# gusanagy/Hybrid-Diffusion-Underwater-Atmopheric-Image-Enhancement

Measured on AMD Instinct MI355X. Metric: denoising-steps/sec (256x256, T=1000), higher is better.
Workload: dtype f32 (tensors and accumulation fp32; every operand of the attention contractions as 2xfp16 pieces -- scores: a balance per product term, four terms at d_head 16 / three at d_head 32; P.V: three terms -- and of the 3x3 convs behind GroupNorm likewise (other 3x3 convs: 3xbf16 pieces), on the 16-bit MFM

## Files before the change

### hybrid-diffusion-underwater-atmopheric-image-enhancement_amd/_capi.py

```python
from __future__ import annotations

import ctypes as C
import os
import subprocess

_HERE = os.path.dirname(os.path.abspath(__file__))
LIB_PATH = os.environ.get("HDIFF_LIB", os.path.join(_HERE, "libhdiff.so"))
CSRC = os.path.join(_HERE, "csrc")
MAX_TAPS = 25

_lib = None


class LinearJob(C.Structure):
    _fields_ = [("w0", C.c_void_p), ("b0", C.c_void_p), ("w1", C.c_void_p), ("b1", C.c_void_p), ("y", C.c_void_p),
                ("n", C.c_int), ("first", C.c_int)]


class DdpmLoopDesc(C.Structure):
    _fields_ = [
        ("x", C.c_void_p), ("eps_c", C.c_void_p), ("eps_u", C.c_void_p), ("noise", C.c_void_p), ("x_next", C.c_void_p),
        ("coeff1", C.c_void_p), ("coeff2", C.c_void_p), ("sigma", C.c_void_p), ("step_ptr", C.c_void_p), ("T", C.c_int),
        ("w", C.c_double), ("seed", C.c_uint64), ("nan_flag", C.c_void_p), ("n", C.c_int64),
        ("x_dup0", C.c_void_p), ("x_dup1", C.c_void_p), ("t_next", C.c_void_p), ("t_count", C.c_int),
        ("done_counter", C.c_void_p),
    ]


class CfgDdimLoopDesc(C.Structure):
    _fields_ = [
        ("x", C.c_void_p), ("eps_c", C.c_void_p), ("eps_u", C.c_void_p), ("noise", C.c_void_p), ("x_next", C.c_void_p),
        ("tab", C.c_void_p), ("t_tab", C.c_void_p), ("step_ptr", C.c_void_p), ("nsteps", C.c_int), ("clip_x0", C.c_int),
        ("w", C.c_double), ("seed", C.c_uint64), ("nan_flag", C.c_void_p), ("n", C.c_int64),
        ("x_dup0", C.c_void_p), ("x_dup1", C.c_void_p), ("t_next", C.c_void_p), ("t_count", C.c_int),
        ("done_counter", C.c_void_p),
    ]


class CfgDpmppLoopDesc(C.Structure):
    _fields_ = [
        ("x", C.c_void_p), ("eps_c", C.c_void_p), ("eps_u", C.c_void_p), ("x_next", C.c_void_p), ("x0_prev", C.c_void_p),
        ("tab", C.c_void_p), ("t_tab", C.c_void_p), ("step_ptr", C.c_void_p), ("nsteps", C.c_int), ("clip_x0", C.c_int),
        ("w", C.c_double), ("nan_flag", C.c_void_p), ("n", C.c_int64),
        ("x_dup0", C.c_void_p), ("x_dup1", C.c_void_p), ("t_next", C.c_void_p), ("t_count", C.c_int),
        ("done_counter", C.c_void_p),
    ]


class ConvDesc(C.Structure):
    _fields_ = [
        ("x0", C.c_void_p), ("x1", C.c_void_p), ("C0", C.c_int), ("C1", C.c_int),
        ("B", C.c_int), ("H", C.c_int), ("W", C.c_int),
        ("wp", C.c_void_p), ("bias", C.c_void_p), ("Cout", C.c_int), ("CinPad", C.c_int), ("CoutPad", C.c_int),
        ("gn_scale", C.c_void_p), ("gn_shift", C.c_void_p), ("addvec", C.c_void_p), ("residual", C.c_void_p),
        ("out", C.c_void_p), ("OH", C.c_int), ("OW", C.c_int),
        ("VH", C.c_int), ("VW", C.c_int), ("in_stride", C.c_int),
        ("out_sy", C.c_int), ("out_oy", C.c_int), ("out_sx", C.c_int), ("out_ox", C.c_int),
        ("ntaps", C.c_int), ("tap_dy", C.c_int * MAX_TAPS), ("tap_dx", C.c_int * MAX_TAPS),
        ("splitk_ws", C.c_void_p), ("splitk_floats", C.c_int64), ("wp_x3", C.c_void_p),
        ("wp_h2", C.c_void_p), ("act_scale", C.c_void_p),
    ]


class ConvRange(C.Structure):
    _fields_ = [("absmax_out", C.c_void_p), ("absmax_in", C.c_void_p), ("wp_h2_taps", C.c_void_p),
                ("wp_h2_s2", C.c_void_p)]


class MsssimDesc(C.Structure):
    MAX_PAIRS, MAX_SCALES, MAX_WINDOW = 15, 5, 33
    _fields_ = [
        ("B", C.c_int), ("C", C.c_int), ("H", C.c_int), ("W", C.c_int), ("nscales", C.c_int), ("window", C.c_int),
        ("weights", C.POINTER(C.c_float)), ("npairs", C.c_int),
        ("pair_chan", C.c_int * 15), ("pair_scale", C.c_int * 15), ("pair_cs_pow", C.c_int * 15), ("pair_l_pow", C.c_int * 15),
        ("l1_scale", C.c_int), ("C1", C.c_float), ("C2", C.c_float), ("alpha", C.c_float), ("compensation", C.c_float),
        ("data_range", C.c_float), ("mean", C.c_int),
    ]


class WgradDesc(C.Structure):
    _fields_ = [
        ("x0", C.c_void_p), ("x1", C.c_void_p), ("C0", C.c_int), ("C1", C.c_int),
        ("B", C.c_int), ("H", C.c_int), ("W", C.c_int),
        ("gn_scale", C.c_void_p), ("gn_shift", C.c_void_p), ("dy", C.c_void_p),
        ("Cout", C.c_int), ("CinPad", C.c_int), ("CoutPad", C.c_int), ("OH", C.c_int), ("OW", C.c_int),
        ("VH", C.c_int), ("VW", C.c_int), ("in_stride", C.c_int),
        ("out_sy", C.c_int), ("out_oy", C.c_int), ("out_sx", C.c_int), ("out_ox", C.c_int),
        ("ntaps", C.c_int), ("tap_dy", C.c_int * MAX_TAPS), ("tap_dx", C.c_int * MAX_TAPS),
    ]


_PROTOS = {
    "hdiff_abi_version": (C.c_int, []),
    "hdiff_last_error": (C.c_char_p, []),
    "hdiff_device_count": (C.c_int, []),
    "hdiff_pack_conv_weight_x3": (C.c_int, [C.c_void_p, C.c_void_p, C.c_int, C.c_int, C.c_int, C.c_int, C.c_void_p]),
    "hdiff_pack_conv_weight_x3_taps": (C.c_int, [C.c_void_p, C.c_void_p, C.c_int, C.c_int, C.c_int, C.c_int, C.c_int, C.c_int,
                                                 C.POINTER(C.c_int), C.POINTER(C.c_int), C.c_int, C.c_void_p]),
    "hdiff_pack_conv_weight_h2_words": (C.c_int, [C.c_int, C.c_int, C.c_int, C.POINTER(C.c_int64)]),
    "hdiff_pack_conv_weight_h2": (C.c_int, [C.c_void_p, C.c_void_p, C.c_int, C.c_int, C.c_int, C.c_void_p]),
    "hdiff_gn_act_scale": (C.c_int, [C.c_void_p, C.c_void_p, C.c_int, C.c_int64, C.c_float, C.c_void_p, C.c_void_p]),
    "hdiff_set_contraction_mode": (C.c_int, [C.c_int]),
    "hdiff_get_contraction_mode": (C.c_int, []),
    "hdiff_pack_conv_weight": (C.c_int, [C.c_void_p, C.c_void_p, C.c_int, C.c_int, C.c_int, C.c_int, C.c_int, C.c_int,
                                         C.POINTER(C.c_int), C.POINTER(C.c_int), C.c_int, C.c_int, C.c_int, C.c_void_p]),
    "hdiff_conv2d_fwd": (C.c_int, [C.POINTER(ConvDesc), C.c_void_p]),
    "hdiff_conv2d_fwd_dropout": (C.c_int, [C.POINTER(ConvDesc), C.c_void_p, C.c_float, C.c_void_p]),
    "hdiff_conv2d_fwd_range": (C.c_int, [C.POINTER(ConvDesc), C.POINTER(ConvRange), C.c_void_p]),
    "hdiff_range_words_zero": (C.c_int, [C.c_void_p, C.c_int, C.c_void_p]),
    "hdiff_conv2d_fwd_route": (C.c_int, [C.POINTER(ConvDesc), C.POINTER(ConvRange), C.c_int, C.POINTER(C.c_int), C.POINTER(C.c_int)]),
    "hdiff_pack_conv_weight_h2_taps_words": (C.c_int, [C.c_int, C.c_int, C.c_int, C.c_int, C.POINTER(C.c_int64)]),
    "hdiff_pack_conv_weight_h2_taps": (C.c_int, [C.c_void_p, C.c_void_p, C.c_int, C.c_int, C.c_int, C.c_int, C.c_int, C.c_int,
                                                 C.POINTER(C.c_int), C.POINTER(C.c_int), C.c_int, C.c_void_p]),
    "hdiff_pack_conv_weight_h2_s2_words": (C.c_int, [C.c_int, C.c_int, C.c_int, C.POINTER(C.c_int64)]),
    "hdiff_pack_conv_weight_h2_s2": (C.c_int, [C.c_void_p, C.c_void_p, C.c_int, C.c_int, C.c_int, C.c_int, C.c_void_p]),
    "hdiff_conv2d_fwd_workspace": (C.c_int, [C.POINTER(ConvDesc), C.POINTER(C.c_int64)]),
    "hdiff_gn_stats": (C.c_int, [C.c_void_p, C.c_void_p, C.c_int, C.c_int, C.c_int, C.c_int, C.c_int, C.c_int, C.c_void_p,
                                 C.c_void_p]),
    "hdiff_gn_finalize": (C.c_int, [C.c_void_p, C.c_int, C.c_int, C.c_int, C.c_int, C.c_void_p, C.c_void_p, C.c_float,
                                    C.c_void_p, C.c_void_p, C.c_void_p, C.c_void_p, C.c_void_p]),
    "hdiff_gn_scale_shift": (C.c_int, [C.c_void_p, C.c_void_p, C.c_int, C.c_int, C.c_int, C.c_int, C.c_int, C.c_int, C.c_void_p,
                                       C.c_void_p, C.c_void_p, C.c_float, C.c_void_p, C.c_void_p, C.c_void_p]),
    "hdiff_gn_swish_apply": (C.c_int, [C.c_void_p, C.c_void_p, C.c_void_p, C.c_void_p, C.c_int, C.c_int, C.c_int,
                                       C.c_void_p]),
    "hdiff_mha_flash_fwd": (C.c_int, [C.c_void_p, C.c_void_p, C.c_void_p, C.c_int, C.c_int, C.c_int, C.c_int, C.c_void_p]),
    "hdiff_mha_flash_fwd_workspace": (C.c_int, [C.c_int, C.c_int, C.c_int, C.c_int, C.POINTER(C.c_int64)]),
    "hdiff_mha_flash_fwd_ws": (C.c_int, [C.c_void_p, C.c_void_p, C.c_void_p, C.c_int, C.c_int, C.c_int, C.c_int, C.c_void_p,
                                         C.c_int64, C.c_void_p]),
    "hdiff_mha_flash_fwd_route": (C.c_int, [C.c_int, C.c_int, C.c_int, C.c_int, C.c_int, C.c_int64] + [C.POINTER(C.c_int)] * 3),
    "hdiff_mha_wide_fwd": (C.c_int, [C.c_void_p, C.c_void_p, C.c_int, C.c_int, C.c_int, C.c_void_p]),
    "hdiff_mha_wide_bwd": (C.c_int, [C.c_void_p, C.c_void_p, C.c_void_p, C.c_void_p, C.c_int, C.c_int, C.c_int, C.c_void_p]),
    "hdiff_gn_affine_bwd": (C.c_int, [C.c_void_p, C.c_int, C.c_int, C.c_int, C.c_int, C.c_void_p, C.c_void_p, C.c_void_p, C.c_void_p,
                                      C.c_void_p, C.c_void_p, C.c_void_p, C.c_void_p, C.c_void_p, C.c_void_p]),
    "hdiff_gn_affine_apply": (C.c_int, [C.c_void_p, C.c_void_p, C.c_void_p, C.c_void_p, C.c_int, C.c_int, C.c_int,
                                        C.c_void_p]),
    "hdiff_mha_flash_bwd_workspace": (C.c_int, [C.c_int, C.c_int, C.c_int, C.c_int, C.POINTER(C.c_int64)]),
    "hdiff_mha_flash_bwd": (C.c_int, [C.c_void_p, C.c_void_p, C.c_void_p, C.c_void_p, C.c_void_p, C.c_void_p, C.c_void_p,
                                      C.c_int, C.c_int, C.c_int, C.c_int, C.c_void_p]),
    "hdiff_mha_flash_bwd_route": (C.c_int, [C.c_int, C.c_int, C.c_int, C.c_int] + [C.POINTER(C.c_int)] * 4),
    "hdiff_conv2d_wgrad_workspace": (C.c_int, [C.POINTER(WgradDesc), C.POINTER(C.c_int), C.POINTER(C.c_int64)]),
    "hdiff_conv2d_wgrad": (C.c_int, [C.POINTER(WgradDesc), C.c_void_p, C.c_int, C.c_void_p]),
    "hdiff_conv2d_wgrad_dropout": (C.c_int, [C.POINTER(WgradDesc), C.c_void_p, C.c_float, C.c_void_p, C.c_int, C.c_void_p]),
    "hdiff_conv2d_wgrad_route": (C.c_int, [C.POINTER(WgradDesc), C.c_int, C.POINTER(C.c_int)]),
    "hdiff_conv_wgrad_unpack": (C.c_int, [C.c_void_p, C.c_int, C.c_void_p, C.c_int, C.c_int, C.c_int, C.c_int, C.c_int, C.c_int,
                                          C.POINTER(C.c_int), C.POINTER(C.c_int), C.c_int, C.c_int, C.c_int, C.c_void_p]),
    "hdiff_gn_swish_bwd": (C.c_int, [C.c_void_p, C.c_void_p, C.c_int, C.c_int, C.c_int, C.c_int, C.c_int, C.c_void_p, C.c_void_p,
                                     C.c_void_p, C.c_void_p, C.c_void_p, C.c_void_p, C.c_void_p, C.c_void_p, C.c_void_p,
                                     C.c_void_p, C.c_void_p]),
    "hdiff_gn_swish_dropout_bwd": (C.c_int, [C.c_void_p, C.c_int, C.c_int, C.c_int, C.c_int, C.c_void_p, C.c_void_p, C.c_float,
                                             C.c_void_p, C.c_void_p, C.c_void_p, C.c_void_p, C.c_void_p, C.c_void_p, C.c_void_p,
                                             C.c_void_p, C.c_void_p]),
    "hdiff_bias_addvec_grad": (C.c_int, [C.c_void_p, C.c_int, C.c_int, C.c_int, C.c_void_p, C.c_void_p, C.c_void_p]),
    "hdiff_linear_rows_bwd": (C.c_int, [C.c_void_p, C.c_void_p, C.c_int, C.c_void_p, C.c_void_p, C.c_void_p, C.c_void_p,
                                        C.c_void_p, C.c_int, C.c_int, C.c_int, C.c_int, C.c_int, C.c_int, C.c_void_p]),
    "hdiff_sq_err_bwd": (C.c_int, [C.c_void_p, C.c_void_p, C.c_void_p, C.c_void_p, C.c_int64, C.c_void_p]),
    "hdiff_dropout_mask": (C.c_int, [C.c_void_p, C.c_int64, C.c_float, C.c_uint64, C.c_uint64, C.c_void_p]),
    "hdiff_dropout_keep_bits": (C.c_int, [C.c_void_p, C.c_int64, C.c_float, C.c_uint64, C.c_uint64, C.c_void_p]),
    "hdiff_mul": (C.c_int, [C.c_void_p, C.c_void_p, C.c_void_p, C.c_int64, C.c_void_p]),
    "hdiff_linear_rows": (C.c_int, [C.c_void_p, C.c_void_p, C.c_int, C.c_void_p, C.c_void_p, C.c_void_p, C.c_int, C.c_int,
                                    C.c_int, C.c_int, C.c_int, C.c_void_p]),
    "hdiff_linear_rows_multi": (C.c_int, [C.c_void_p, C.c_void_p, C.c_void_p, C.c_int, C.c_int, C.c_int, C.c_int, C.c_void_p]),
    "hdiff_q_sample": (C.c_int, [C.c_void_p, C.c_void_p, C.c_void_p, C.c_void_p, C.c_void_p, C.c_void_p, C.c_int, C.c_int,
                                 C.c_int, C.c_void_p]),
    "hdiff_sq_err": (C.c_int, [C.c_void_p, C.c_void_p, C.c_void_p, C.c_int64, C.c_void_p]),
    "hdiff_ddpm_step": (C.c_int, [C.c_void_p, C.c_void_p, C.c_void_p, C.c_void_p, C.c_void_p, C.c_void_p, C.c_void_p,
                                  C.c_void_p, C.c_void_p, C.c_int, C.c_double, C.c_uint64, C.c_void_p, C.c_int64, C.c_void_p]),
    "hdiff_ddpm_step_loop": (C.c_int, [C.c_void_p, C.c_void_p]),
    "hdiff_cfg_ddim_step": (C.c_int, [C.c_void_p, C.c_void_p, C.c_void_p, C.c_void_p, C.c_void_p, C.c_void_p, C.c_void_p, C.c_int,
                                      C.c_double, C.c_int, C.c_uint64, C.c_void_p, C.c_int64, C.c_void_p]),
    "hdiff_cfg_ddim_step_loop": (C.c_int, [C.c_void_p, C.c_void_p]),
    "hdiff_cfg_dpmpp_step": (C.c_int, [C.c_void_p, C.c_void_p, C.c_void_p, C.c_void_p, C.c_void_p, C.c_void_p, C.c_void_p, C.c_int,
                                       C.c_double, C.c_int, C.c_void_p, C.c_int64, C.c_void_p]),
    "hdiff_cfg_dpmpp_step_loop": (C.c_int, [C.c_void_p, C.c_void_p]),
    "hdiff_fill_t": (C.c_int, [C.c_void_p, C.c_void_p, C.c_int, C.c_void_p]),
    "hdiff_step_decrement": (C.c_int, [C.c_void_p, C.c_void_p]),
    "hdiff_ddim_step": (C.c_int, [C.c_void_p, C.c_void_p, C.c_void_p, C.c_void_p, C.c_void_p, C.c_int, C.c_void_p, C.c_int64,
                                  C.c_void_p]),
    "hdiff_fill_from_table": (C.c_int, [C.c_void_p, C.c_void_p, C.c_void_p, C.c_int, C.c_int, C.c_void_p]),
    "hdiff_tile_gather": (C.c_int, [C.c_void_p] * 4 + [C.c_int] * 10 + [C.c_void_p]),
    "hdiff_tile_ddim_step": (C.c_int, [C.c_void_p] * 12 + [C.c_int, C.c_void_p] + [C.c_int] * 8 + [C.c_void_p]),
    "hdiff_dpmpp_step": (C.c_int, [C.c_void_p] * 6 + [C.c_int, C.c_int, C.c_void_p, C.c_int64, C.c_void_p]),
    "hdiff_tile_dpmpp_step": (C.c_int, [C.c_void_p] * 13 + [C.c_int, C.c_int, C.c_void_p] + [C.c_int] * 8 + [C.c_void_p]),
    "hdiff_resize_nearest": (C.c_int, [C.c_void_p, C.c_void_p, C.c_int, C.c_int, C.c_int, C.c_int, C.c_int, C.c_void_p]),
    "hdiff_avgpool_global": (C.c_int, [C.c_void_p, C.c_void_p, C.c_int, C.c_int, C.c_void_p]),
    "hdiff_train_b_loss_workspace": (C.c_int, [C.c_int64, C.POINTER(C.c_int64)]),
    "hdiff_train_b_loss_fwd": (C.c_int, [C.c_void_p] * 7 + [C.c_int, C.c_int, C.c_int] + [C.c_void_p] * 5),
    "hdiff_train_b_loss_bwd": (C.c_int, [C.c_void_p] * 7 + [C.c_int, C.c_int, C.c_int] + [C.c_void_p] * 5),
    "hdiff_msssim_l1_workspace": (C.c_int, [C.POINTER(MsssimDesc), C.POINTER(C.c_int64), C.POINTER(C.c_int64)]),
    "hdiff_msssim_l1_fwd": (C.c_int, [C.POINTER(MsssimDesc)] + [C.c_void_p] * 6),
    "hdiff_msssim_l1_bwd": (C.c_int, [C.POINTER(MsssimDesc)] + [C.c_void_p] * 7),
    "hdiff_quality_workspace": (C.c_int, [C.c_int, C.c_int, C.c_int, C.POINTER(C.c_int64)]),
    "hdiff_psnr_ssim": (C.c_int, [C.c_void_p, C.c_void_p, C.c_int, C.c_int, C.c_int, C.c_void_p, C.c_void_p, C.c_void_p]),
    "hdiff_uiqm": (C.c_int, [C.c_void_p, C.c_int, C.c_int, C.c_int, C.c_void_p, C.c_void_p, C.c_void_p]),
    "hdiff_avgpool_global_bwd": (C.c_int, [C.c_void_p, C.c_void_p, C.c_int, C.c_int, C.c_void_p]),
    "hdiff_resize_nearest_bwd": (C.c_int, [C.c_void_p, C.c_void_p, C.c_int, C.c_int, C.c_int, C.c_int, C.c_int, C.c_void_p]),
    "hdiff_concat2": (C.c_int, [C.c_void_p, C.c_void_p, C.c_void_p, C.c_int, C.c_int64, C.c_int64, C.c_void_p]),
    "hdiff_clip": (C.c_int, [C.c_void_p, C.c_void_p, C.c_float, C.c_float, C.c_int64, C.c_void_p]),
    "hdiff_axpby": (C.c_int, [C.c_float, C.c_void_p, C.c_float, C.c_void_p, C.c_void_p, C.c_int64, C.c_void_p]),
    "hdiff_opt_chunk": (C.c_int, []),
    "hdiff_grad_norm_clip_coef": (C.c_int, [C.c_void_p, C.c_void_p, C.c_int, C.c_void_p, C.c_float, C.c_void_p, C.c_void_p]),
    "hdiff_adamw_step": (C.c_int, [C.c_void_p, C.c_void_p, C.c_int, C.c_void_p, C.c_double, C.c_double, C.c_double, C.c_double, C.c_double,
                                   C.c_int64, C.c_void_p]),
    "hdiff_randn": (C.c_int, [C.c_void_p, C.c_int64, C.c_uint64, C.c_uint64, C.c_void_p]),
    "hdiff_graph_begin": (C.c_int, [C.c_void_p]),
    "hdiff_graph_end": (C.c_int, [C.c_void_p, C.POINTER(C.c_void_p)]),
    "hdiff_graph_launch": (C.c_int, [C.c_void_p, C.c_void_p]),
    "hdiff_graph_destroy": (C.c_int, [C.c_void_p]),
    "hdiff_event_create": (C.c_int, [C.POINTER(C.c_void_p)]),
    "hdiff_event_record": (C.c_int, [C.c_void_p, C.c_void_p]),
    "hdiff_event_elapsed_ms": (C.c_int, [C.c_void_p, C.c_void_p, C.POINTER(C.c_float)]),
    "hdiff_event_destroy": (C.c_int, [C.c_void_p]),
}

EXPORTED_SYMBOLS = tuple(_PROTOS.keys())


def build(verbose: bool = False, clean: bool = False) -> str:
    if clean:
        subprocess.run(["make", "-C", CSRC, "clean"], capture_output=True, text=True, check=True)
    res = subprocess.run(["make", "-C", CSRC, "-j8"], capture_output=True, text=True)
    if verbose or res.returncode != 0:
        print(res.stdout[-4000:])
        print(res.stderr[-4000:])
    if res.returncode != 0 or not os.path.isfile(LIB_PATH):
        raise RuntimeError("building libhdiff.so failed")
    return LIB_PATH


MUTANT_PATH = os.path.join(CSRC, "build", "libhdiff_mutant.so")
MUTANT2_PATH = os.path.join(CSRC, "build", "libhdiff_mutant2.so")


def build_mutant(verbose: bool = False) -> str:
    res = subprocess.run(["make", "-C", CSRC, "-j4", "mutant", "mutant2"], capture_output=True, text=True)
    if verbose or res.returncode != 0:
        print(res.stdout[-4000:])
        print(res.stderr[-4000:])
    if res.returncode != 0 or not os.path.isfile(MUTANT_PATH) or not os.path.isfile(MUTANT2_PATH):
        raise RuntimeError("building libhdiff_mutant.so / libhdiff_mutant2.so failed")
    return MUTANT_PATH


def lib() -> C.CDLL:
    global _lib
    if _lib is None:
        if not os.path.isfile(LIB_PATH):
            raise RuntimeError(f"{LIB_PATH} is missing: run `python -c 'import __graft_entry__ as g; g.build()'` "
                               "(the HIP extension is required; there is no CPU fallback)")
        import torch
        hip_rt = os.path.join(os.path.dirname(torch.__file__), "lib", "libamdhip64.so")
        if os.path.isfile(hip_rt):
            C.CDLL(hip_rt, mode=C.RTLD_GLOBAL)
        l = C.CDLL(LIB_PATH)
        for name, (res, args) in _PROTOS.items():
            fn = getattr(l, name)
            fn.restype, fn.argtypes = res, args
        _lib = l
    return _lib


def check(rc: int, what: str = "") -> None:
    if rc != 0:
        msg = lib().hdiff_last_error().decode(errors="replace")
        raise RuntimeError(f"hdiff {what} failed (status {rc}): {msg}")
```

### hybrid-diffusion-underwater-atmopheric-image-enhancement_amd/csrc/attention.hip

```cpp
#include <stdlib.h>

#include <type_traits>

#include "common.h"
#include "device.h"

using namespace hdiff;

namespace {

constexpr int KT = 64;
constexpr int KROW = KT + 4;
constexpr int ATT_THREADS = 256;
constexpr float RESCALE_LIMIT = 1.8446744e19f;

__device__ __forceinline__ f32x2 pk_add(f32x2 a, f32x2 b) {
  f32x2 r;
  asm("v_pk_add_f32 %0, %1, %2" : "=v"(r) : "v"(a), "v"(b));
  return r;
}

template <int D, int NQ>
__global__ __launch_bounds__(ATT_THREADS) void mha_flash_fwd_kernel(const float* __restrict__ qkv, float* __restrict__ out,
                                                                    float* __restrict__ lse2, int C, int L, float qscale, int check) {
// ... 300 lines not shown
  f32x2 l_run[NQ];
#pragma unroll
  for (int qt = 0; qt < NQ; ++qt) {
    l_run[qt] = f32x2{0.f, 0.f};
    negm4[qt] = f32x4{0.f, 0.f, 0.f, 0.f};
#pragma unroll
    for (int mt = 0; mt < MT; ++mt) O[mt][qt] = f32x4{0.f, 0.f, 0.f, 0.f};
  }

  f32x4 P[4];
  auto rowsum = [&](int qt) {
    const f32x2 a = pk_add(__builtin_shufflevector(P[0], P[0], 0, 1), __builtin_shufflevector(P[0], P[0], 2, 3));
    const f32x2 b = pk_add(__builtin_shufflevector(P[1], P[1], 0, 1), __builtin_shufflevector(P[1], P[1], 2, 3));
    const f32x2 c = pk_add(__builtin_shufflevector(P[2], P[2], 0, 1), __builtin_shufflevector(P[2], P[2], 2, 3));
    const f32x2 d = pk_add(__builtin_shufflevector(P[3], P[3], 0, 1), __builtin_shufflevector(P[3], P[3], 2, 3));
    const f32x2 ab = pk_add(a, b), cd = pk_add(c, d);
    l_run[qt] = pk_add(l_run[qt], pk_add(ab, cd));
  };
  auto do_tile = [&](auto first_tag, int buf) {
    constexpr bool FIRST = decltype(first_tag)::value;
    float kf[4][KS];
    float vf[4][MT][4];
#pragma unroll
    for (int ks = 0; ks < 4; ++ks) {
#pragma unroll
      for (int s = 0; s < KS; ++s) kf[ks][s] = sK[buf][(4 * s + g) * KROW + ks * 16 + i16];
#pragma unroll
      for (int mt = 0; mt < MT; ++mt) {
        const float4 v4 = *reinterpret_cast<const float4*>(&sV[buf][(mt * 16 + i16) * KROW + ks * 16 + 4 * g]);
        vf[ks][mt][0] = v4.x; vf[ks][mt][1] = v4.y; vf[ks][mt][2] = v4.z; vf[ks][mt][3] = v4.w;
      }
    }
    f32x4 S[2][4];
    auto qk_mfma = [&](int qt, int i) {
      const int s = i >> 2, ks = i & 3;
      S[qt & 1][ks] = __builtin_amdgcn_mfma_f32_16x16x4f32(kf[ks][s], qf[qt][s], s == 0 ? negm4[qt] : S[qt & 1][ks], 0, 0, 0);
    };
    auto pv_mfma = [&](int qt, int i) {
      const int mt = i % MT, j = i / MT, ks = j >> 2, r = j & 3;
      O[mt][qt] = __builtin_amdgcn_mfma_f32_16x16x4f32(vf[ks][mt][r], P[ks][r], O[mt][qt], 0, 0, 0);
    };
    auto softmax = [&](int qt) {
      f32x4(&Sq)[4] = S[qt & 1];
      if (FIRST) {
        float tm = fmaxf(fmaxf(Sq[0][0], Sq[0][1]), fmaxf(Sq[0][2], Sq[0][3]));
#pragma unroll
        for (int ks = 1; ks < 4; ++ks) tm = fmaxf(tm, fmaxf(fmaxf(Sq[ks][0], Sq[ks][1]), fmaxf(Sq[ks][2], Sq[ks][3])));
        tm = fmaxf(tm, __shfl_xor(tm, 16, 64));
        tm = fmaxf(tm, __shfl_xor(tm, 32, 64));
        const float nm = -tm;
        negm4[qt] = f32x4{nm, nm, nm, nm};
#pragma unroll
        for (int ks = 0; ks < 4; ++ks) Sq[ks] += negm4[qt];
      }
      if (!FIRST || qt > 0) {
        __builtin_amdgcn_sched_barrier(0);
        rowsum((qt + NQ - 1) % NQ);
      }
#pragma unroll
      for (int ks = 0; ks < 4; ++ks)
        P[ks] = f32x4{__builtin_amdgcn_exp2f(Sq[ks][0]), __builtin_amdgcn_exp2f(Sq[ks][1]), __builtin_amdgcn_exp2f(Sq[ks][2]),
                      __builtin_amdgcn_exp2f(Sq[ks][3])};
      __builtin_amdgcn_sched_barrier(0);
    };
#pragma unroll
    for (int i = 0; i < N_QK; ++i) qk_mfma(0, i);
#pragma unroll
    for (int qt = 0; qt < NQ; ++qt) {
      softmax(qt);
      constexpr int LEAD = 3;
      static_assert(N_QK <= N_PV, "the QK^T chain is folded into the P.V slots");
      if (qt + 1 < NQ) {
#pragma unroll
        for (int i = 0; i < LEAD; ++i) qk_mfma(qt + 1, i);
      }
#pragma unroll
      for (int i = 0; i < N_PV; ++i) {
        if (i == N_PV - LEAD) __builtin_amdgcn_sched_barrier(0);
        pv_mfma(qt, i);
        if (qt + 1 < NQ && i + LEAD < N_QK) qk_mfma(qt + 1, i + LEAD);
      }
    }
  };

  stage_load(0);
  stage_store(0);
  __syncthreads();
  stage_load(ntiles > 1 ? 1 : 0);
  do_tile(std::true_type{}, 0);
  stage_store(1);
  __syncthreads();
  auto step = [&](int t, auto buf_tag) {
    constexpr int buf = decltype(buf_tag)::value;
    stage_load((t + 1 < ntiles) ? t + 1 : t);
    do_tile(std::false_type{}, buf);
    stage_store(buf ^ 1);
    __syncthreads();
  };
  int t = 1;
  for (; t + 1 < ntiles; t += 2) {
    step(t, std::integral_constant<int, 1>{});
    step(t + 1, std::integral_constant<int, 0>{});
  }
  if (t < ntiles) step(t, std::integral_constant<int, 1>{});
  rowsum(NQ - 1);

  float* obase = out + ((size_t)b * C + (size_t)head * D) * L;
#pragma unroll
  for (int qt = 0; qt < NQ; ++qt) {
    float lt = l_run[qt].x + l_run[qt].y;
    lt += __shfl_xor(lt, 16, 64);
    lt += __shfl_xor(lt, 32, 64);
    const bool bad = !(lt < OVERFLOW_LIMIT);
    const float inv = bad ? __builtin_nanf("") : 1.0f / lt;
    const int q = qblk0 + qt * 16 + i16;
    if (lse2 != nullptr && q < L && g == 0)
      lse2[((size_t)b * gridDim.y + head) * L + q] = bad ? __builtin_nanf("") : __builtin_amdgcn_logf(lt) - negm4[qt][0];
    if (q < L) {
#pragma unroll
      for (int mt = 0; mt < MT; ++mt)
#pragma unroll
        for (int r = 0; r < 4; ++r) {
          const int d = mt * 16 + 4 * g + r;
          if (d < D) obase[(size_t)d * L + q] = O[mt][qt][r] * inv;
        }
    }
  }
}

template <int D, int NQ>
void launch_v(const float* qkv, float* o, float* lse2, int B, int C, int heads, int L, float qscale, int check,
              hipStream_t stream) {
  dim3 grid(cdiv(L, 64 * NQ), heads, B);
  hipLaunchKernelGGL((mha_flash_fwd_kernel<D, NQ>), grid, dim3(ATT_THREADS), 0, stream, qkv, o, lse2, C, L, qscale, check);
}

struct MhaFwdRoute { int route, nq, check; };
MhaFwdRoute mha_fwd_route(int B, int C, int heads, int L, bool want_lse, int64_t ws_bytes, int mode) {
  const int D = C / heads;
  if (D >= 48 || L < 512) return {HDIFF_MHA_FWD_ROUTE_RUNNING_MAX, 1, 0};
  if (mode != HDIFF_CONTRACT_F32) {
    const int64_t need = mha_fwd_x3p_workspace(B, C, heads, L);
    const bool ws_ok = need != 0 && ws_bytes >= need;
    if (mode == HDIFF_CONTRACT_F16 && !want_lse && ws_ok) return {HDIFF_MHA_FWD_ROUTE_F16_SINGLE, 4, 1};
    if (ws_ok && D == 16) return {HDIFF_MHA_FWD_ROUTE_H2_PAIRS, 4, 1};
    if (ws_ok && D == 32) return {HDIFF_MHA_FWD_ROUTE_X3P_PAIRS, 4, 1};
    if (L % KT == 0 && (D == 16 || D == 32)) return {HDIFF_MHA_FWD_ROUTE_X3_TRIPLES, 4, 1};
  }
  if (L % KT == 0) return {HDIFF_MHA_FWD_ROUTE_FAST_F32, 4, 1};
  return {HDIFF_MHA_FWD_ROUTE_RUNNING_MAX, 4, 0};
}

template <int D>
void launch_d(const float* qkv, float* o, float* lse2, int B, int C, int heads, int L, void* ws, const MhaFwdRoute& rt,
              hipStream_t stream) {
  const float qscale = 1.4426950408889634f / sqrtf((float)D);
  static const bool skip_check = getenv("HDIFF_NO_CHECK_PASS") != nullptr;
  const bool tail = !skip_check || rt.route == HDIFF_MHA_FWD_ROUTE_RUNNING_MAX || rt.route == HDIFF_MHA_FWD_ROUTE_FAST_F32;
  if constexpr (D < 48) {
    switch (rt.route) {
      case HDIFF_MHA_FWD_ROUTE_F16_SINGLE: launch_mha_fwd_f16(qkv, o, B, C, heads, L, qscale, ws, stream); break;
      case HDIFF_MHA_FWD_ROUTE_H2_PAIRS: launch_mha_fwd_h2(qkv, o, lse2, B, C, heads, L, qscale, ws, stream); break;
      case HDIFF_MHA_FWD_ROUTE_X3P_PAIRS: launch_mha_fwd_x3p(qkv, o, lse2, B, C, heads, L, qscale, ws, stream); break;
      case HDIFF_MHA_FWD_ROUTE_X3_TRIPLES: launch_mha_fwd_x3(qkv, o, lse2, B, C, heads, L, qscale, stream); break;
      case HDIFF_MHA_FWD_ROUTE_FAST_F32:
        hipLaunchKernelGGL((mha_flash_fwd_fast_kernel<D, 4>), dim3(cdiv(L, 256), heads, B), dim3(ATT_THREADS), 0, stream, qkv, o, lse2, C, L, qscale);
        break;
      default: break;
    }
    if (tail && rt.nq == 4) launch_v<D, 4>(qkv, o, lse2, B, C, heads, L, qscale, rt.check, stream);
  }
  if (tail && rt.nq == 1) launch_v<D, 1>(qkv, o, lse2, B, C, heads, L, qscale, rt.check, stream);
}

}

static int mha_fwd_check_shape(int B, int C, int heads, int L) {
  HDIFF_CHECK_ARG(B > 0 && L > 0 && heads > 0 && C % heads == 0, "mha_flash_fwd: bad sizes B=%d C=%d heads=%d L=%d", B, C,
                  heads, L);
  HDIFF_CHECK_ARG(mha_head_dim_ok(C / heads), "mha_flash_fwd: head dim %d not in {4, 8, 12, 16, 24, 32, 48, 64}", C / heads);
  return HDIFF_OK;
}

static int mha_flash_fwd_any(const float* qkv, float* o, float* lse2, int B, int C, int heads, int L, void* ws,
                             int64_t ws_bytes, hipStream_t s) {
  HDIFF_CHECK_ARG(qkv && o, "mha_flash_fwd: null pointer");
  const int rc = mha_fwd_check_shape(B, C, heads, L);
  if (rc != HDIFF_OK) return rc;
  const MhaFwdRoute rt = mha_fwd_route(B, C, heads, L, lse2 != nullptr, ws_bytes, contraction_mode());
  (void)hipGetLastError();
  with_head_dim(C / heads, [&](auto d) { launch_d<decltype(d)::value>(qkv, o, lse2, B, C, heads, L, ws, rt, s); });
  HDIFF_CHECK_LAUNCH("mha_flash_fwd_kernel");
  return HDIFF_OK;
}

extern "C" int hdiff_mha_flash_fwd(const float* qkv, float* o, float* lse2, int B, int C, int heads, int L,
                                   hdiff_stream_t stream) {
  return mha_flash_fwd_any(qkv, o, lse2, B, C, heads, L, nullptr, 0, (hipStream_t)stream);
}

extern "C" int hdiff_mha_flash_fwd_workspace(int B, int C, int heads, int L, int64_t* bytes_out) {
  HDIFF_CHECK_ARG(bytes_out, "mha_flash_fwd_workspace: null pointer");
  HDIFF_CHECK_ARG(B > 0 && L > 0 && heads > 0 && C % heads == 0, "mha_flash_fwd_workspace: bad sizes B=%d C=%d heads=%d L=%d", B,
                  C, heads, L);
  *bytes_out = mha_fwd_x3p_workspace(B, C, heads, L);
  return HDIFF_OK;
}

extern "C" int hdiff_mha_flash_fwd_ws(const float* qkv, float* o, float* lse2, int B, int C, int heads, int L, void* ws,
                                      int64_t ws_bytes, hdiff_stream_t stream) {
  HDIFF_CHECK_ARG(ws_bytes >= 0 && (ws != nullptr || ws_bytes == 0), "mha_flash_fwd_ws: workspace pointer / size mismatch");
  return mha_flash_fwd_any(qkv, o, lse2, B, C, heads, L, ws, ws_bytes, (hipStream_t)stream);
}

extern "C" int hdiff_mha_flash_fwd_route(int B, int C, int heads, int L, int want_lse, int64_t ws_bytes, int* route_out,
                                         int* nq_out, int* check_out) {
  HDIFF_CHECK_ARG(route_out && nq_out && check_out, "mha_flash_fwd_route: null pointer");
  HDIFF_CHECK_ARG(ws_bytes >= 0, "mha_flash_fwd_ws: workspace pointer / size mismatch");
  const int rc = mha_fwd_check_shape(B, C, heads, L);
  if (rc != HDIFF_OK) return rc;
  const MhaFwdRoute rt = mha_fwd_route(B, C, heads, L, want_lse != 0, ws_bytes, contraction_mode());
  *route_out = rt.route;
  *nq_out = rt.nq;
  *check_out = rt.check;
  return HDIFF_OK;
}
```

### hybrid-diffusion-underwater-atmopheric-image-enhancement_amd/csrc/attention_h2.hip

```cpp
#include <stdlib.h>

#include <type_traits>

#include "common.h"
#include "device.h"

using namespace hdiff;

namespace {

constexpr int KT = 64;
constexpr int THREADS = 256;
#define H2_RARE_BEGIN "s_cmp_lg_u64 %[cond], 0\n\ts_cbranch_scc1 .Lh2r_%=\n.Lh2b_%=:\n\t.subsection 1\n.Lh2r_%=:\n\t"
#define H2_RARE_END "s_branch .Lh2b_%=\n\t.subsection 0"

__device__ __forceinline__ float h2_rare_delta(unsigned long long cond, const f32x4 (&S)[4], int bp16, int bp32) {
  float delta, t, u;
  asm volatile(H2_RARE_BEGIN
               "v_max3_f32 %[t], %[s0], %[s1], %[s2]\n\t"
               "v_max3_f32 %[u], %[s3], %[s4], %[s5]\n\t"
               "v_max3_f32 %[t], %[t], %[s6], %[s7]\n\t"
               "v_max3_f32 %[u], %[u], %[s8], %[s9]\n\t"
               "v_max3_f32 %[t], %[t], %[s10], %[s11]\n\t"
               "v_max3_f32 %[u], %[u], %[s12], %[s13]\n\t"
               "v_max3_f32 %[t], %[t], %[s14], %[s15]\n\t"
               "v_max_f32 %[t], %[t], %[u]\n\t"
               "s_nop 1\n\t"
               "ds_bpermute_b32 %[u], %[bp16], %[t]\n\t"
               "s_waitcnt lgkmcnt(0)\n\t"
               "v_max_f32 %[t], %[t], %[u]\n\t"
               "s_nop 1\n\t"
               "ds_bpermute_b32 %[u], %[bp32], %[t]\n\t"
               "s_waitcnt lgkmcnt(0)\n\t"
               "v_max_f32 %[t], %[t], %[u]\n\t"
               "v_subrev_f32 %[u], 8.0, %[t]\n\t"
               "v_ceil_f32 %[u], %[u]\n\t"
               "v_cmp_lt_f32 vcc, 0x41100000, %[t]\n\t"
               "v_cndmask_b32 %[d], 0, %[u], vcc\n\t"
               H2_RARE_END
               : [d] "=&v"(delta), [t] "=&v"(t), [u] "=&v"(u)
               : [cond] "s"(cond), [bp16] "v"(bp16), [bp32] "v"(bp32), [s0] "v"(S[0][0]), [s1] "v"(S[0][1]), [s2] "v"(S[0][2]),
                 [s3] "v"(S[0][3]), [s4] "v"(S[1][0]), [s5] "v"(S[1][1]), [s6] "v"(S[1][2]), [s7] "v"(S[1][3]), [s8] "v"(S[2][0]),
                 [s9] "v"(S[2][1]), [s10] "v"(S[2][2]), [s11] "v"(S[2][3]), [s12] "v"(S[3][0]), [s13] "v"(S[3][1]),
                 [s14] "v"(S[3][2]), [s15] "v"(S[3][3])
               : "vcc", "scc");
  return delta;
}

__device__ __forceinline__ void h2_rare_rescale(unsigned long long cond, float delta, f32x4& O, f32x4& negm, float& l, float& sum0,
                                                float& sum1) {
  float o0 = O[0], o1 = O[1], o2 = O[2], o3 = O[3], n0 = negm[0], n1 = negm[1], n2 = negm[2], n3 = negm[3], w;
  asm volatile(H2_RARE_BEGIN
               "v_cvt_i32_f32 %[w], %[d]\n\t"
               "v_sub_u32 %[w], 0, %[w]\n\t"
               "v_ldexp_f32 %[o0], %[o0], %[w]\n\t"
               "v_ldexp_f32 %[o1], %[o1], %[w]\n\t"
               "v_ldexp_f32 %[o2], %[o2], %[w]\n\t"
               "v_ldexp_f32 %[o3], %[o3], %[w]\n\t"
               "v_ldexp_f32 %[l], %[l], %[w]\n\t"
               "v_sub_f32 %[n0], %[n0], %[d]\n\t"
               "v_sub_f32 %[n1], %[n1], %[d]\n\t"
               "v_sub_f32 %[n2], %[n2], %[d]\n\t"
               "v_sub_f32 %[n3], %[n3], %[d]\n\t"
               "v_mov_b32 %[q0], 0\n\t"
               "v_mov_b32 %[q1], 0\n\t"
               H2_RARE_END
               : [o0] "+v"(o0), [o1] "+v"(o1), [o2] "+v"(o2), [o3] "+v"(o3), [n0] "+v"(n0), [n1] "+v"(n1), [n2] "+v"(n2),
                 [n3] "+v"(n3), [l] "+v"(l), [q0] "+v"(sum0), [q1] "+v"(sum1), [w] "=&v"(w)
               : [cond] "s"(cond), [d] "v"(delta)
               : "scc");
  O = f32x4{o0, o1, o2, o3};
  negm = f32x4{n0, n1, n2, n3};
}

__device__ __forceinline__ void h2_rare_exp_split(unsigned long long cond, float delta, float one, f32x4 S, unsigned& a0, unsigned& a1,
                                                  unsigned& r0, unsigned& r1, float& sum0, float& sum1) {
  float p0, p1, p2, p3, t0, t1;
  asm volatile(H2_RARE_BEGIN
               "v_sub_f32 %[p0], %[s0], %[d]\n\t"
               "v_sub_f32 %[p1], %[s1], %[d]\n\t"
               "v_sub_f32 %[p2], %[s2], %[d]\n\t"
               "v_sub_f32 %[p3], %[s3], %[d]\n\t"
               "v_exp_f32 %[p0], %[p0]\n\t"
               "v_exp_f32 %[p1], %[p1]\n\t"
               "v_exp_f32 %[p2], %[p2]\n\t"
               "v_exp_f32 %[p3], %[p3]\n\t"
               "s_nop 1\n\t"
               "v_cvt_pk_f16_f32 %[a0], %[p0], %[p1]\n\t"
               "v_cvt_pk_f16_f32 %[a1], %[p2], %[p3]\n\t"
               "v_add_f32 %[t0], %[p0], %[p2]\n\t"
               "v_add_f32 %[t1], %[p1], %[p3]\n\t"
               "v_fma_mixlo_f16 %[r0], %[p0], %[one], -%[a0] op_sel_hi:[0,0,1]\n\t"
               "v_fma_mixlo_f16 %[r1], %[p2], %[one], -%[a1] op_sel_hi:[0,0,1]\n\t"
               "v_add_f32 %[q0], %[q0], %[t0]\n\t"
               "v_add_f32 %[q1], %[q1], %[t1]\n\t"
               "v_fma_mixhi_f16 %[r0], %[p1], %[one], -%[a0] op_sel:[0,0,1] op_sel_hi:[0,0,1]\n\t"
               "v_fma_mixhi_f16 %[r1], %[p3], %[one], -%[a1] op_sel:[0,0,1] op_sel_hi:[0,0,1]\n\t"
               "s_nop 1\n\t"
               H2_RARE_END
               : [a0] "+v"(a0), [a1] "+v"(a1), [r0] "+v"(r0), [r1] "+v"(r1), [q0] "+v"(sum0), [q1] "+v"(sum1), [p0] "=&v"(p0),
                 [p1] "=&v"(p1), [p2] "=&v"(p2), [p3] "=&v"(p3), [t0] "=&v"(t0), [t1] "=&v"(t1)
               : [cond] "s"(cond), [d] "v"(delta), [one] "s"(one), [s0] "v"(S[0]), [s1] "v"(S[1]), [s2] "v"(S[2]), [s3] "v"(S[3])
               : "scc");
}


__global__ __launch_bounds__(THREADS) void qk_rowmax_kernel(const float* __restrict__ qkv, float* __restrict__ rowmax, int C, int L) {
  qkv_rowmax<2>(qkv, rowmax, C, L);
}

template <int D>
__global__ __launch_bounds__(THREADS) void qk_split_h2_kernel(const float* __restrict__ qkv, const float* __restrict__ rowmax,
                                                              __bf16* __restrict__ ws, int C, int L, float qscale, float one) {
  const int heads = C / D;
  const int which = blockIdx.y / heads, head = blockIdx.y - which * heads, b = blockIdx.z;
  const int l = blockIdx.x * THREADS + threadIdx.x;
  float mq = 0.f, mk = 0.f;
#pragma unroll
  for (int d = 0; d < D; ++d) {
    mq = fmaxf(mq, rowmax[(size_t)b * 2 * C + head * D + d]);
    mk = fmaxf(mk, rowmax[(size_t)b * 2 * C + C + head * D + d]);
  }
  const int a = balance_exp(__builtin_bit_cast(unsigned, mq), __builtin_bit_cast(unsigned, mk), qscale);
  const float sc = which == 0 ? qscale * __builtin_bit_cast(float, (unsigned)(127 - a) << 23) : __builtin_bit_cast(float, (unsigned)(127 + a) << 23);
  if (l >= L) return;
  const float* src = qkv + ((size_t)b * 3 * C + (size_t)which * C + (size_t)head * D) * L;
  const size_t piece = (size_t)L * D;
  __bf16* pair = ws + ((size_t)b * heads + head) * F_COUNT * piece;
  const float up = (float)(1 << PAIR_SHIFT) * one;
  unsigned h[4][D / 2];
#pragma unroll
  for (int j = 0; j < D / 2; ++j)
    pair4(src[(size_t)(2 * j) * L + l] * sc, src[(size_t)(2 * j + 1) * L + l] * sc, up, h[0][j], h[1][j], h[2][j], h[3][j]);
#pragma unroll
  for (int p = 0; p < 4; ++p) {
    if (which == 0 && (p == 1 || p == 3)) continue;
    const int slot = which == 0 ? F_Q + (p == 0 ? 0 : 1) : F_K + p;
    u32x4* o = reinterpret_cast<u32x4*>(pair + slot * piece + (size_t)l * D);
#pragma unroll
    for (int j = 0; j < D / 8; ++j) o[j] = u32x4{h[p][4 * j], h[p][4 * j + 1], h[p][4 * j + 2], h[p][4 * j + 3]};
  }
}

template <int D>
__global__ __launch_bounds__(THREADS) void v_split_h2_kernel(const float* __restrict__ qkv, __bf16* __restrict__ ws, int C, int L,
                                                             float one) {
  const int heads = C / D;
  const int row = blockIdx.x, head = row / D, d = row - head * D, b = blockIdx.y;
  const int tid = threadIdx.x;
  const float* src = qkv + ((size_t)b * 3 * C + 2 * (size_t)C + row) * L;
  const size_t piece = (size_t)L * D;
  __bf16* pair = ws + ((size_t)b * heads + head) * F_COUNT * piece;
  _Float16* dst = reinterpret_cast<_Float16*>(pair + F_V * piece) + (size_t)d * L;

  const float amax = row_absmax(src, L, tid);
  int e = (int)((__builtin_bit_cast(unsigned, amax) >> 23) & 0xffu) - 127;
  e = e < -100 ? -100 : (e > 127 ? 127 : e);
  const float scale = __builtin_bit_cast(float, (unsigned)(14 - e + 127) << 23);
  if (tid == 0) reinterpret_cast<float*>(pair + F_VINV * piece)[d] = __builtin_bit_cast(float, (unsigned)(e - 14 + 127) << 23);
  for (int i = tid; i < L / 4; i += THREADS) {
    const f32x4 v = *reinterpret_cast<const f32x4*>(src + 4 * (size_t)i);
    unsigned a0, a1, c0, c1;
    split2(v[0] * scale, v[1] * scale, one, a0, a1);
    split2(v[2] * scale, v[3] * scale, one, c0, c1);
    *reinterpret_cast<u32x2*>(dst + 4 * (size_t)i) = u32x2{a0, c0};
    *reinterpret_cast<u32x2*>(dst + piece + 4 * (size_t)i) = u32x2{a1, c1};
  }
}

template <int D, int NQ>
__global__ __launch_bounds__(THREADS, 2) void mha_flash_fwd_h2_kernel(const __bf16* __restrict__ ws, float* __restrict__ out,
                                                                      float* __restrict__ lse2, int C, int L, float one) {
  static_assert(D == 16, "head dim: two terms share one MFMA's 32 contraction slots");
  static_assert(NQ == 4, "the stage pipeline is written for four query tiles per wave");
  constexpr int NKP = 4;
  constexpr int NKS = 2;
  constexpr int NQK = NKS;
  constexpr int MT = D / 16;
  constexpr int KROWB = D * 2;
  constexpr int KPART = KT * KROWB;
  constexpr int VROWB = KT * 2 + 8;
  constexpr int VPART = D * VROWB;
  constexpr int QB = 64 * NQ;
  constexpr int VBASE = NKP * KPART;
  constexpr int BUFB = VBASE + 2 * VPART;
  __shared__ __attribute__((aligned(16))) unsigned char smem[2][BUFB];

  const int tid = threadIdx.x, lane = tid & 63, wave = tid >> 6;
  const int i16 = lane & 15, g = lane >> 4;
  const TileId tile = xcd_tile();
  const int head = tile.head, b = tile.b;
  const int qblk0 = tile.x * QB + wave * (16 * NQ);
  const int ntiles = L / KT;

  const int doff = 8 * (g & 1);
  const bool hi = g >> 1;

  const size_t piece_n = (size_t)L * D;
  const __bf16* wsq = ws + ((size_t)b * gridDim.y + head) * F_COUNT * piece_n;
  u32x4 qop[NQ][NQK];
  {
    const unsigned dn2 = PAIR_DOWN2;
#pragma unroll
    for (int qt = 0; qt < NQ; ++qt) {
      const int q = qblk0 + qt * 16 + i16;
      const u32x4 q0 = *reinterpret_cast<const u32x4*>(wsq + (size_t)q * D + doff);
      const u32x4 q1s = *reinterpret_cast<const u32x4*>(wsq + piece_n + (size_t)q * D + doff);
      const u32x4 sel = hi ? q1s : q0;
      unsigned dnw[4];
#pragma unroll
      for (int w = 0; w < 4; ++w) asm("v_pk_mul_f16 %0, %1, %2" : "=v"(dnw[w]) : "v"(sel[w]), "v"(dn2));
      qop[qt][0] = sel;
      qop[qt][1] = u32x4{dnw[0], dnw[1], dnw[2], dnw[3]};
    }
  }
  int kaddr[NKS];
#pragma unroll
  for (int ks = 0; ks < NKS; ++ks) kaddr[ks] = (2 * ks + (hi ? 1 : 0)) * KPART + i16 * KROWB + doff * 2;
  const int vaddr = i16 * VROWB + 8 * g;

  static_assert(2 * D * 8 == THREADS, "staging geometry: one V chunk per thread");
  static_assert(KPART == 2048 && THREADS == 256, "LDS-DMA geometry: eight 1 KiB runs, two per wave");
  const unsigned char* gsrc;
  int lds_off;
  u32x4 stage;
  {
    const __bf16* vsp = wsq + F_V * piece_n;
    const int p = tid / (D * 8), rem = tid - p * (D * 8);
    const int d = rem >> 3, seg = rem & 7;
    gsrc = reinterpret_cast<const unsigned char*>(vsp + p * piece_n + (size_t)d * L) + seg * 16;
    lds_off = VBASE + p * VPART + d * VROWB + seg * 16;
  }
  const unsigned lds0 = (unsigned)(size_t)(lds_byte*)&smem[0][0];
  const unsigned char* kdma = reinterpret_cast<const unsigned char*>(wsq + F_K * piece_n);
  auto dma_k = [&](int t, int buf) {
    const int ws_ = __builtin_amdgcn_readfirstlane(wave);
    const unsigned char* src = kdma + (size_t)ws_ * (piece_n * 2) + (size_t)t * KPART;
    const unsigned dst = __builtin_amdgcn_readfirstlane(lds0 + buf * BUFB + ws_ * KPART);
    dma_1k(src, lane * 16, dst);
    dma_1k(src + 1024, lane * 16, dst + 1024);
  };
  auto stage_load = [&](int t) { stage = *reinterpret_cast<const u32x4*>(gsrc + (size_t)t * (KT * 2)); };
  auto stage_store = [&](int buf) {
    unsigned char* dst = &smem[buf][lds_off];
    *reinterpret_cast<u32x2*>(dst) = u32x2{stage[0], stage[1]};
    *reinterpret_cast<u32x2*>(dst + 8) = u32x2{stage[2], stage[3]};
  };

  f32x4 O[MT][NQ];
  f32x4 negm4[NQ];
  float l_run[NQ];
  const int bp16 = (lane ^ 16) * 4, bp32 = (lane ^ 32) * 4;
#pragma unroll
  for (int qt = 0; qt < NQ; ++qt) {
    l_run[qt] = 0.f;
    negm4[qt] = f32x4{0.f, 0.f, 0.f, 0.f};
#pragma unroll
    for (int mt = 0; mt < MT; ++mt) O[mt][qt] = f32x4{0.f, 0.f, 0.f, 0.f};
  }

  u32x4 vop[2][MT][2];
  u32x4 kop[4][NKS];
  f32x4 S[2][4];
  u32x4 pop[2][2][2];
  auto load_v = [&](int buf) {
    const unsigned char* vb = smem[buf] + VBASE;
#pragma unroll
    for (int p = 0; p < 2; ++p)
#pragma unroll
      for (int mt = 0; mt < MT; ++mt)
#pragma unroll
        for (int c = 0; c < 2; ++c) {
          const unsigned char* src = vb + p * VPART + mt * 16 * VROWB + 64 * c + vaddr;
          const u32x2 lo = *reinterpret_cast<const u32x2*>(src);
          const u32x2 hi2 = *reinterpret_cast<const u32x2*>(src + 32);
          vop[p][mt][c] = u32x4{lo[0], lo[1], hi2[0], hi2[1]};
        }
  };
  auto load_k = [&](int buf) {
    const unsigned char* kb = smem[buf];
#pragma unroll
    for (int kt = 0; kt < 4; ++kt)
#pragma unroll
      for (int ks = 0; ks < NKS; ++ks) kop[kt][ks] = *reinterpret_cast<const u32x4*>(kb + kaddr[ks] + kt * 16 * KROWB);
  };
  auto qk_mfma = [&](int qt, int par, int n, int rollk = -1) {
    const int j = n >> 2, kt = n & 3;
    u32x4 qb = qop[qt][j];
    if ((HDIFF_MUTANT & 4) && j == 1)
#pragma unroll
      for (int w = 0; w < 4; ++w) qb[w] &= 0xffe0ffe0u;
    S[par][kt] = mfma_f16(kop[kt][j], qb, j == 0 ? negm4[qt] : S[par][kt]);
    if (rollk >= 0) kop[kt][j] = *reinterpret_cast<const u32x4*>(smem[rollk] + kaddr[j] + kt * 16 * KROWB);
  };
  constexpr int NPV = 6 * MT;
  auto pv_mfma = [&](int qt, int par, int n) {
    const int c = n / (3 * MT), r = n - c * 3 * MT, mt = r / 3, term = r - mt * 3;
    const int pv_v = term == 0 ? 1 : 0, pv_p = term == 1 ? 1 : 0;
    u32x4 pb = pop[par][pv_p][c];
    if ((HDIFF_MUTANT & 8) && pv_p == 1)
#pragma unroll
      for (int w = 0; w < 4; ++w) pb[w] &= 0xffe0ffe0u;
    O[mt][qt] = mfma_f16(vop[pv_v][mt][c], pb, O[mt][qt]);
  };
  auto exp_split = [&](const f32x4 (&Sq)[4], u32x4 (&pp)[2][2], float& sum0, float& sum1) {
#pragma unroll
    for (int kt = 0; kt < 4; ++kt) {
      const float p0 = __builtin_amdgcn_exp2f(Sq[kt][0]), p1 = __builtin_amdgcn_exp2f(Sq[kt][1]);
      const float p2 = __builtin_amdgcn_exp2f(Sq[kt][2]), p3 = __builtin_amdgcn_exp2f(Sq[kt][3]);
      sum0 = (kt == 0) ? p0 + p2 : sum0 + (p0 + p2);
      sum1 = (kt == 0) ? p1 + p3 : sum1 + (p1 + p3);
      const int c = kt >> 1, o = (kt & 1) * 2;
      unsigned a0, a1, c0, c1;
      split2(p0, p1, one, a0, a1);
      split2(p2, p3, one, c0, c1);
      pp[0][c][o] = a0; pp[1][c][o] = a1;
      pp[0][c][o + 1] = c0; pp[1][c][o + 1] = c1;
    }
  };
  auto stage_max = [&](int par) {
    float mx = fmaxf(fmaxf(S[par][0][0], S[par][0][1]), fmaxf(S[par][0][2], S[par][0][3]));
#pragma unroll
    for (int kt = 1; kt < 4; ++kt) mx = fmaxf(mx, fmaxf(fmaxf(S[par][kt][0], S[par][kt][1]), fmaxf(S[par][kt][2], S[par][kt][3])));
    mx = fmaxf(mx, __shfl_xor(mx, 16, 64));
    return fmaxf(mx, __shfl_xor(mx, 32, 64));
  };
  auto stage_fn = [&](auto qt_tag, auto first_tag, auto pend_tag, int rollk = -1) {
    constexpr int QT = decltype(qt_tag)::value;
    constexpr bool FIRST = decltype(first_tag)::value;
    constexpr bool PEND = decltype(pend_tag)::value;
    constexpr int par = QT & 1;
    constexpr int qk_q = (QT + 1) % NQ, pv_q = (QT + NQ - 1) % NQ;
    constexpr int NQKM = 4 * NQK, NM = NQKM + (PEND ? NPV : 0);
    float sum0, sum1;
    if constexpr (FIRST) {
#pragma unroll
      for (int n = 0; n < NQKM; ++n) qk_mfma(qk_q, par ^ 1, n, rollk);
      if constexpr (PEND)
#pragma unroll
        for (int n = 0; n < NPV; ++n) pv_mfma(pv_q, par ^ 1, n);
      const float nm = P_SHIFT - stage_max(par);
      negm4[QT] = f32x4{nm, nm, nm, nm};
#pragma unroll
      for (int kt = 0; kt < 4; ++kt) S[par][kt] += negm4[QT];
      exp_split(S[par], pop[par], sum0, sum1);
    } else {
      float pe[4][4], ad[4][2];
      unsigned u[4][2];
      _Float16 rl[4][2];
      unsigned r2[4][2];
      auto vstep = [&](int n) {
        const int kt = n / 14, r = n - kt * 14;
        if (r < 4) pe[kt][r] = __builtin_amdgcn_exp2f(S[par][kt][r]);
        else if (r < 6) {
          const f16x2 p = {(_Float16)pe[kt][2 * (r - 4)], (_Float16)pe[kt][2 * (r - 4) + 1]};
          unsigned w = __builtin_bit_cast(unsigned, p);
          asm("" : "+v"(w));
          u[kt][r - 4] = w;
        } else if (r < 8) ad[kt][r - 6] = pe[kt][r - 6] + pe[kt][r - 6 + 2];
        else if (r < 10) rl[kt][r - 8] = (_Float16)__builtin_fmaf(pe[kt][2 * (r - 8)], one, -(float)__builtin_bit_cast(f16x2, u[kt][r - 8])[0]);
        else if (r < 12) {
          const f16x2 pr = {rl[kt][r - 10],
                            (_Float16)__builtin_fmaf(pe[kt][2 * (r - 10) + 1], one, -(float)__builtin_bit_cast(f16x2, u[kt][r - 10])[1])};
          unsigned w = __builtin_bit_cast(unsigned, pr);
          asm("" : "+v"(w));
          r2[kt][r - 10] = w;
        } else if (r == 12) sum0 = (kt == 0) ? ad[kt][0] : sum0 + ad[kt][0];
        else sum1 = (kt == 0) ? ad[kt][1] : sum1 + ad[kt][1];
      };
      constexpr int NV = 56;
#pragma unroll
      for (int i = 0; i < NM; ++i) {
        if constexpr (PEND) {
          const int npv = (i + 1) * NPV / NM, ppv = i * NPV / NM;
          if (npv != ppv) pv_mfma(pv_q, par ^ 1, ppv);
          else qk_mfma(qk_q, par ^ 1, i - ppv, rollk);
        } else qk_mfma(qk_q, par ^ 1, i, rollk);
#pragma unroll
        for (int n = NV * i / NM; n < NV * (i + 1) / NM; ++n) vstep(n);
        __builtin_amdgcn_sched_barrier(0);
      }
      const unsigned long long cond = __builtin_amdgcn_ballot_w64(sum0 + sum1 >= P_TRIP);
      const float delta = h2_rare_delta(cond, S[par], bp16, bp32);
      h2_rare_rescale(cond, delta, O[0][QT], negm4[QT], l_run[QT], sum0, sum1);
#pragma unroll
      for (int kt = 0; kt < 4; ++kt)
        h2_rare_exp_split(cond, delta, one, S[par][kt], u[kt][0], u[kt][1], r2[kt][0], r2[kt][1], sum0, sum1);
#pragma unroll
      for (int kt = 0; kt < 4; ++kt) {
        const int c = kt >> 1, o = (kt & 1) * 2;
        pop[par][0][c][o] = u[kt][0]; pop[par][1][c][o] = r2[kt][0];
        pop[par][0][c][o + 1] = u[kt][1]; pop[par][1][c][o + 1] = r2[kt][1];
      }
    }
    l_run[QT] += sum0 + sum1;
  };

  auto tile_fn = [&](auto first_tag, int t) {
    constexpr bool FIRST = decltype(first_tag)::value;
    using Pend = std::integral_constant<bool, !FIRST>;
    const int buf = t & 1;
    if constexpr (FIRST) load_v(buf);
    stage_fn(std::integral_constant<int, 0>{}, first_tag, Pend{});
    if constexpr (!FIRST) load_v(buf);
    stage_fn(std::integral_constant<int, 1>{}, first_tag, std::true_type{});
    stage_store(buf ^ 1);
    asm volatile("s_waitcnt vmcnt(0)" ::: "memory");
    __syncthreads();
    stage_load((t + 2 < ntiles) ? t + 2 : ntiles - 1);
    dma_k((t + 2 < ntiles) ? t + 2 : ntiles - 1, buf);
    stage_fn(std::integral_constant<int, 2>{}, first_tag, std::true_type{}, buf ^ 1);
    stage_fn(std::integral_constant<int, 3>{}, first_tag, std::true_type{});
  };

  stage_load(0);
  dma_k(0, 0);
  stage_store(0);
  asm volatile("s_waitcnt vmcnt(0)" ::: "memory");
  __syncthreads();
  stage_load(ntiles > 1 ? 1 : 0);
  dma_k(ntiles > 1 ? 1 : 0, 1);
  load_k(0);
#pragma unroll
  for (int n = 0; n < 4 * NQK; ++n) qk_mfma(0, 0, n);
  tile_fn(std::true_type{}, 0);
  for (int t = 1; t < ntiles; ++t) tile_fn(std::false_type{}, t);
#pragma unroll
  for (int n = 0; n < NPV; ++n) pv_mfma(NQ - 1, 1, n);

  float* obase = out + ((size_t)b * C + (size_t)head * D) * L;
  const float* vinv = reinterpret_cast<const float*>(wsq + F_VINV * piece_n);
#pragma unroll
  for (int qt = 0; qt < NQ; ++qt) {
    float lt = l_run[qt];
    lt += __shfl_xor(lt, 16, 64);
    lt += __shfl_xor(lt, 32, 64);
    const bool bad = !(lt < OVERFLOW_LIMIT);
    const float inv = bad ? __builtin_nanf("") : 1.0f / lt;
    const int q = qblk0 + qt * 16 + i16;
    if (lse2 != nullptr && g == 0)
      lse2[((size_t)b * gridDim.y + head) * L + q] = bad ? __builtin_nanf("") : __builtin_amdgcn_logf(lt) - negm4[qt][0];
#pragma unroll
    for (int mt = 0; mt < MT; ++mt)
#pragma unroll
      for (int r = 0; r < 4; ++r)
        obase[(size_t)(mt * 16 + 4 * g + r) * L + q] = (O[mt][qt][r] * inv) * vinv[mt * 16 + 4 * g + r];
  }
}

}

namespace hdiff {
void launch_v_split_h2(const float* qkv, void* ws, int B, int C, int heads, int L, hipStream_t stream) {
  if (C / heads == 16) hipLaunchKernelGGL((v_split_h2_kernel<16>), dim3(C, B), dim3(THREADS), 0, stream, qkv, (__bf16*)ws, C, L, 1.0f);
  else hipLaunchKernelGGL((v_split_h2_kernel<32>), dim3(C, B), dim3(THREADS), 0, stream, qkv, (__bf16*)ws, C, L, 1.0f);
}

int64_t mha_fwd_h2_tail_bytes(int B, int C) { return ((int64_t)B * 2 * C * 4 + 255) / 256 * 256; }

void launch_qk_split_h2(const float* qkv, void* ws, int B, int C, int heads, int L, float qscale, hipStream_t stream) {
  float* rowmax = reinterpret_cast<float*>(reinterpret_cast<unsigned char*>(ws) + mha_fwd_x3p_workspace(B, C, heads, L) - mha_fwd_h2_tail_bytes(B, C));
  hipLaunchKernelGGL(qk_rowmax_kernel, dim3(2 * C, B), dim3(THREADS), 0, stream, qkv, rowmax, C, L);
  dim3 grid(cdiv(L, 256), 2 * heads, B);
  if (C / heads == 16) hipLaunchKernelGGL((qk_split_h2_kernel<16>), grid, dim3(THREADS), 0, stream, qkv, rowmax, (__bf16*)ws, C, L, qscale, 1.0f);
  else hipLaunchKernelGGL((qk_split_h2_kernel<32>), grid, dim3(THREADS), 0, stream, qkv, rowmax, (__bf16*)ws, C, L, qscale, 1.0f);
}

void launch_mha_fwd_h2(const float* qkv, float* o, float* lse2, int B, int C, int heads, int L, float qscale, void* ws,
                       hipStream_t stream) {
  launch_qk_split_h2(qkv, ws, B, C, heads, L, qscale, stream);
  launch_v_split_h2(qkv, ws, B, C, heads, L, stream);
  hipLaunchKernelGGL((mha_flash_fwd_h2_kernel<16, 4>), dim3(L / 256, heads, B), dim3(THREADS), 0, stream, (const __bf16*)ws, o, lse2,
                     C, L, 1.0f);
}

}
```

### hybrid-diffusion-underwater-atmopheric-image-enhancement_amd/csrc/attention_x3p.hip

```cpp
#include <stdlib.h>

#include "common.h"
#include "device.h"

using namespace hdiff;

namespace {

constexpr int D = 32;
constexpr int KT = 64;
constexpr int THREADS = 256;
constexpr int NQT = 3;

__global__ __launch_bounds__(THREADS, 2) void mha_flash_fwd_x3p_kernel(const __bf16* __restrict__ ws, float* __restrict__ out,
                                                                      float* __restrict__ lse2, int C, int L, float one) {
  constexpr int KS = D / 16;
  constexpr int KROWB = D * 2 + 16;
  constexpr int KPART = KT * KROWB;
  constexpr int VROWB = KT * 2 + 8;
  constexpr int VPART = D * VROWB;
  constexpr int NKC = NQT * KT * D / 8;
  constexpr int NVC = 2 * D * 8;
  constexpr int NLD = (NKC + NVC) / THREADS;
  static_assert((NKC + NVC) % THREADS == 0, "staging geometry");
// ... 92 lines not shown
#pragma unroll
      for (int s = 0; s < KS; ++s) kop[p][s] = *reinterpret_cast<const u32x4*>(kbuf + p * KPART + 32 * s);
  };
  auto load_v = [&](int buf, int kb, u32x4 (&vop)[2][2]) {
    const unsigned char* vbuf = smem[buf] + VBASE + kb * 64;
#pragma unroll
    for (int ab = 0; ab < 2; ++ab)
#pragma unroll
      for (int p = 0; p < 2; ++p) {
        const unsigned char* src = vbuf + vaddr[p] + 32 * ab;
        const u32x2 lo = *reinterpret_cast<const u32x2*>(src);
        const u32x2 hi2 = *reinterpret_cast<const u32x2*>(src + 16);
        vop[ab][p] = u32x4{lo[0], lo[1], hi2[0], hi2[1]};
      }
  };
  auto qk = [&](const u32x4 (&kop)[NQT][KS], int G, f32x16 c) {
    f32x16 S = c;
#pragma unroll
    for (int term = 0; term < NQT; ++term)
#pragma unroll
      for (int s = 0; s < KS; ++s) {
        u32x4 qb = qop[G][term][s];
        if ((HDIFF_MUTANT & 2) && term == 1)
#pragma unroll
          for (int w = 0; w < 4; ++w) qb[w] &= 0xffe0ffe0u;
        S = mfma_f16(kop[term][s], qb, S);
      }
    return S;
  };
  auto exp_pairs = [&](const f32x16& S, u32x4 (&pop)[2][2], float& sum0, float& sum1) {
    sum0 = 0.f; sum1 = 0.f;
#pragma unroll
    for (int j = 0; j < 4; ++j) {
      const float p0 = __builtin_amdgcn_exp2f(S[4 * j]), p1 = __builtin_amdgcn_exp2f(S[4 * j + 1]);
      const float p2 = __builtin_amdgcn_exp2f(S[4 * j + 2]), p3 = __builtin_amdgcn_exp2f(S[4 * j + 3]);
      sum0 += p0 + p2;
      sum1 += p1 + p3;
      unsigned a0, a1, c0, c1;
      split2(p0, p1, one, a0, a1);
      split2(p2, p3, one, c0, c1);
      const int ab = j >> 1, o = (j & 1) * 2;
      pop[ab][0][o] = a0; pop[ab][1][o] = a1;
      pop[ab][0][o + 1] = c0; pop[ab][1][o + 1] = c1;
    }
  };
  auto softmax_pairs = [&](f32x16& S, int G, u32x4 (&pop)[2][2]) {
    float sum0, sum1;
    exp_pairs(S, pop, sum0, sum1);
    if (__builtin_amdgcn_ballot_w64(sum0 + sum1 >= P_TRIP) != 0ull) {
      float mx = fmaxf(fmaxf(S[0], S[1]), fmaxf(S[2], S[3]));
#pragma unroll
      for (int j = 1; j < 4; ++j) mx = fmaxf(mx, fmaxf(fmaxf(S[4 * j], S[4 * j + 1]), fmaxf(S[4 * j + 2], S[4 * j + 3])));
      mx = fmaxf(mx, __shfl_xor(mx, 32, 64));
      const float delta = (mx > P_SHIFT + 1.0f) ? __builtin_ceilf(mx - P_SHIFT) : 0.f;
      const int e = -(int)delta;
#pragma unroll
      for (int r = 0; r < 16; ++r) O[G][r] = __builtin_ldexpf(O[G][r], e);
      l_run[G][0] = __builtin_ldexpf(l_run[G][0], e);
      l_run[G][1] = __builtin_ldexpf(l_run[G][1], e);
      negm2[G] -= delta;
#pragma unroll
      for (int r = 0; r < 16; ++r) S[r] -= delta;
      exp_pairs(S, pop, sum0, sum1);
    }
    l_run[G][0] += sum0;
    l_run[G][1] += sum1;
  };
  auto pv = [&](const u32x4 (&vop)[2][2], const u32x4 (&pop)[2][2], int G) {
#pragma unroll
    for (int ab = 0; ab < 2; ++ab) {
      O[G] = mfma_f16(vop[ab][1], pop[ab][0], O[G]);
      O[G] = mfma_f16(vop[ab][0], pop[ab][1], O[G]);
      O[G] = mfma_f16(vop[ab][0], pop[ab][0], O[G]);
    }
  };

  stage_load(0);
  stage_store(0);
  __syncthreads();
  stage_load(ntiles > 1 ? 1 : 0);
  {
    u32x4 K0[NQT][KS];
    load_k(0, 0, K0);
    const f32x16 s0 = qk(K0, 0, negm16), s1 = qk(K0, 1, negm16);
    float t0 = s0[0], t1 = s1[0];
#pragma unroll
    for (int r = 1; r < 16; ++r) { t0 = fmaxf(t0, s0[r]); t1 = fmaxf(t1, s1[r]); }
    negm2[0] = P_SHIFT - fmaxf(t0, __shfl_xor(t0, 32, 64));
    negm2[1] = P_SHIFT - fmaxf(t1, __shfl_xor(t1, 32, 64));
  }
  auto block = [&](int buf, int kb) {
    u32x4 kop[NQT][KS], vop[2][2];
    load_k(buf, kb, kop);
    load_v(buf, kb, vop);
    f32x16 S2[2];
#pragma unroll
    for (int G = 0; G < 2; ++G) {
      float nm = negm2[G];
      asm volatile("" : "+v"(nm));
#pragma unroll
      for (int r = 0; r < 16; ++r) negm16[r] = nm;
      S2[G] = qk(kop, G, negm16);
    }
#pragma unroll
    for (int G = 0; G < 2; ++G) {
      u32x4 pop[2][2];
      softmax_pairs(S2[G], G, pop);
      pv(vop, pop, G);
    }
  };
  block(0, 0);
  block(0, 1);
  stage_store(1);
  __syncthreads();
  for (int t = 1; t < ntiles; ++t) {
    const int buf = t & 1;
    stage_load((t + 1 < ntiles) ? t + 1 : t);
    block(buf, 0);
    block(buf, 1);
    stage_store(buf ^ 1);
    __syncthreads();
  }

  float* obase = out + ((size_t)b * C + (size_t)head * D) * L;
  const float* vinv = reinterpret_cast<const float*>(qs + 8 * piece);
#pragma unroll
  for (int G = 0; G < 2; ++G) {
    float lt = l_run[G][0] + l_run[G][1];
    lt += __shfl_xor(lt, 32, 64);
    const bool bad = !(lt < OVERFLOW_LIMIT);
    const float inv = bad ? __builtin_nanf("") : 1.0f / lt;
    const int q = qblk0 + 32 * G + l31;
    if (lse2 != nullptr && h == 0)
      lse2[((size_t)b * heads + head) * L + q] = bad ? __builtin_nanf("") : __builtin_amdgcn_logf(lt) - negm2[G];
#pragma unroll
    for (int r = 0; r < 16; ++r) {
      const int d = 8 * (r >> 2) + 4 * h + (r & 3);
      obase[(size_t)d * L + q] = (O[G][r] * inv) * vinv[d];
    }
  }
}

}

namespace hdiff {

int64_t mha_fwd_x3p_workspace(int B, int C, int heads, int L) {
  const int Dh = C / heads;
  if ((Dh != 16 && Dh != 32) || L % 256 != 0 || L < 512) return 0;
  return (int64_t)B * C * L * F_COUNT * 2 + mha_fwd_h2_tail_bytes(B, C);
}

void launch_mha_fwd_x3p(const float* qkv, float* o, float* lse2, int B, int C, int heads, int L, float qscale, void* ws,
                        hipStream_t stream) {
  launch_qk_split_h2(qkv, ws, B, C, heads, L, qscale, stream);
  launch_v_split_h2(qkv, ws, B, C, heads, L, stream);
  hipLaunchKernelGGL(mha_flash_fwd_x3p_kernel, dim3(L / 256, heads, B), dim3(THREADS), 0, stream, (const __bf16*)ws, o, lse2, C, L, 1.0f);
}

}
```

### hybrid-diffusion-underwater-atmopheric-image-enhancement_amd/csrc/common.h

```cpp
#pragma once
#include <hip/hip_runtime.h>
#include <stdint.h>
#include <stdio.h>
#include <string.h>

#include <type_traits>

#include "../../include/hdiff.h"

namespace hdiff {

void set_error(const char* fmt, ...);

#define HDIFF_CHECK_ARG(cond, ...)            \
  do {                                        \
    if (!(cond)) {                            \
      hdiff::set_error(__VA_ARGS__);          \
      return HDIFF_ERR_INVALID;               \
    }                                         \
  } while (0)

#define HDIFF_CHECK_LAUNCH(what)                                                   \
  do {                                                                             \
    hipError_t e__ = hipGetLastError();                                            \
    if (e__ != hipSuccess) {                                                       \
      hdiff::set_error("%s: %s", what, hipGetErrorString(e__));                    \
      return HDIFF_ERR_LAUNCH;                                                     \
    }                                                                              \
  } while (0)

static inline int cdiv(int a, int b) { return (a + b - 1) / b; }

static inline int grid_floor_2k(int64_t n, int per_thread = 1) {
  int64_t blocks = (n / per_thread + 255) / 256;
  if (blocks < 1) blocks = 1;
  if (blocks > 2048) blocks = 2048;
  return (int)blocks;
}
static inline int grid_ceil_8k(int64_t n, int per_thread = 1) {
  int64_t blocks = (n + (int64_t)256 * per_thread - 1) / ((int64_t)256 * per_thread);
  if (blocks > 256 * 32) blocks = 256 * 32;
  if (blocks < 1) blocks = 1;
  return (int)blocks;
}

static inline bool first_use_on_device(uint64_t& mask) {
  int dev = 0;
  if (hipGetDevice(&dev) != hipSuccess || dev < 0 || dev >= 64) return true;
  const uint64_t bit = 1ull << dev;
  if (mask & bit) return false;
  mask |= bit;
  return true;
}

bool wgrad3x3_applicable(const hdiff_conv_wgrad_desc* d);
int wgrad3x3_nsplit(const hdiff_conv_wgrad_desc* d);
int launch_wgrad3x3(const hdiff_conv_wgrad_desc* d, float* dwp, int nsplit, hipStream_t stream, const unsigned* keep_bits = nullptr,
                    float inv_keep = 1.0f);
bool wgrad1x1_applicable(const hdiff_conv_wgrad_desc* d);
int wgrad1x1_nsplit(const hdiff_conv_wgrad_desc* d);
int launch_wgrad1x1(const hdiff_conv_wgrad_desc* d, float* dwp, int nsplit, hipStream_t stream);

int contraction_mode();
inline bool split_operands_on() { return contraction_mode() != HDIFF_CONTRACT_F32; }

static inline bool mha_head_dim_ok(int D) { return D == 4 || D == 8 || D == 12 || D == 16 || D == 24 || D == 32 || D == 48 || D == 64; }
template <class F>
static inline void with_head_dim(int D, F&& f) {
  switch (D) {
    case 4: return f(std::integral_constant<int, 4>{});
    case 8: return f(std::integral_constant<int, 8>{});
    case 12: return f(std::integral_constant<int, 12>{});
    case 16: return f(std::integral_constant<int, 16>{});
    case 24: return f(std::integral_constant<int, 24>{});
    case 32: return f(std::integral_constant<int, 32>{});
    case 48: return f(std::integral_constant<int, 48>{});
    case 64: return f(std::integral_constant<int, 64>{});
  }
}

struct KeyRanges { int per, nsplit; };
static inline KeyRanges key_ranges(int nkb_total, int want) {
  if (want > nkb_total) want = nkb_total;
  if (want < 1) want = 1;
  const int per = cdiv(nkb_total, want);
  return {per, cdiv(nkb_total, per)};
}
long long mha_bwd_slab_cap_bytes();
bool mha_bwd_x3_shape_ok(int B, int C, int heads, int L);
KeyRanges mha_bwd_h2_key_ranges(int B, int heads, int L, int D);
int64_t mha_bwd_x3_workspace_floats(int B, int C, int heads, int L);
bool mha_bwd_h2_lds_granted();
void launch_mha_bwd_h2(const float* qkv, const float* d_o, const float* lse2, const float* delta, float* dqkv, float* ws, int B,
                       int C, int heads, int L, KeyRanges g, hipStream_t stream);
int64_t mha_fwd_x3p_workspace(int B, int C, int heads, int L);
int64_t mha_fwd_h2_tail_bytes(int B, int C);
void launch_mha_fwd_x3p(const float* qkv, float* o, float* lse2, int B, int C, int heads, int L, float qscale, void* ws, hipStream_t stream);
void launch_mha_fwd_h2(const float* qkv, float* o, float* lse2, int B, int C, int heads, int L, float qscale, void* ws, hipStream_t stream);
void launch_qk_split_h2(const float* qkv, void* ws, int B, int C, int heads, int L, float qscale, hipStream_t stream);
void launch_v_split_h2(const float* qkv, void* ws, int B, int C, int heads, int L, hipStream_t stream);
void launch_mha_fwd_x3(const float* qkv, float* o, float* lse2, int B, int C, int heads, int L, float qscale, hipStream_t stream);
void launch_mha_fwd_f16(const float* qkv, float* o, int B, int C, int heads, int L, float qscale, void* ws, hipStream_t stream);

}
```

### hybrid-diffusion-underwater-atmopheric-image-enhancement_amd/csrc/conv1x1_x3.hip

```cpp
#include <stdlib.h>

#include "common.h"
#include "conv_x3.h"
#include "device.h"

using namespace hdiff;

namespace {

constexpr int THREADS = 256;

__device__ constexpr int TERM_W[6] = {2, 1, 0, 1, 0, 0};
__device__ constexpr int TERM_X[6] = {0, 1, 2, 0, 1, 0};

template <bool WLDS>
__global__ __launch_bounds__(THREADS, 3) void conv1x1_x3_kernel(const Conv1x1X3K p) {
  constexpr int MT = 2, WN = 2;
  __shared__ __attribute__((aligned(16))) u32x4 sW[WLDS ? 2 : 1][WLDS ? 3 * 64 * 2 : 1];
  const int tid = threadIdx.x, lane = tid & 63, wave = tid >> 6;
  const int l31 = lane & 31, h = lane >> 5;
  int cob = blockIdx.x, tile_id = blockIdx.y;
  if ((gridDim.y & 7u) == 0u && gridDim.x > 1u) {
    const unsigned lin = blockIdx.x + gridDim.x * blockIdx.y, per = 8u * gridDim.x;
    const unsigned grp = lin / per, r = lin - grp * per;
    tile_id = (int)(grp * 8u + (r & 7u));
    cob = (int)(r >> 3);
  }
  const int co0 = cob * 64;
  const long px0 = ((long)tile_id * 4 + __builtin_amdgcn_readfirstlane(wave)) * 64;
  const int b = blockIdx.z;
  const int C1 = p.Cin - p.C0;
  const unsigned hw = (unsigned)p.HW;
  const float* x0b = p.x0 + (size_t)b * p.C0 * p.HW + px0;
  const float* x1b = p.x1 ? p.x1 + (size_t)b * C1 * p.HW + px0 - (size_t)p.C0 * p.HW : x0b;
  const unsigned* wlane = p.wp3 + ((size_t)(co0 + l31) * 8 + h * 4);
  const size_t w_piece = (size_t)p.CoutPad * 8, w_chunk = 3 * w_piece;

  f32x16 acc[MT][WN];
#pragma unroll
  for (int mt = 0; mt < MT; ++mt)
#pragma unroll
    for (int nt = 0; nt < WN; ++nt)
#pragma unroll
      for (int r = 0; r < 16; ++r) acc[mt][nt][r] = 0.f;

  constexpr int XD = 1;
  const int nchunks = p.Cin / 16;
  f32x2 xr[XD + 1][8];
  u32x4 wr[2][MT][3];
  auto load_x = [&](f32x2 (&x)[8], int c) {
    c = min(c, nchunks - 1);
    const float* xb = (16 * c < p.C0) ? x0b : x1b;
    const unsigned k0 = (unsigned)(16 * c + 8 * h);
#pragma unroll
    for (int j = 0; j < 8; ++j) x[j] = *reinterpret_cast<const f32x2*>(xb + (size_t)((k0 + j) * hw + 2u * l31));
  };
  auto load_w = [&](u32x4 (&w)[MT][3], int c) {
    const unsigned* wb = wlane + (size_t)min(c, nchunks - 1) * w_chunk;
#pragma unroll
    for (int mt = 0; mt < MT; ++mt)
#pragma unroll
      for (int pc = 0; pc < 3; ++pc) w[mt][pc] = *reinterpret_cast<const u32x4*>(wb + pc * w_piece + (size_t)mt * 32 * 8);
  };
  auto mma = [&](const f32x2 (&x)[8], const u32x4 (&w)[MT][3]) {
    u32x4 xp[WN][3];
#pragma unroll
    for (int nt = 0; nt < WN; ++nt)
#pragma unroll
      for (int j = 0; j < 4; ++j) {
        unsigned h0, h1, h2;
        split3(x[2 * j][nt], x[2 * j + 1][nt], h0, h1, h2);
        xp[nt][0][j] = h0; xp[nt][1][j] = h1; xp[nt][2][j] = h2;
      }
#pragma unroll
    for (int t = 0; t < 6; ++t) {
      if ((HDIFF_MUTANT & 1) && TERM_W[t] == 0 && TERM_X[t] == 2) continue;
#pragma unroll
      for (int mt = 0; mt < MT; ++mt)
#pragma unroll
        for (int nt = 0; nt < WN; ++nt) acc[mt][nt] = mfma_bf16(w[mt][TERM_W[t]], xp[nt][TERM_X[t]], acc[mt][nt]);
    }
  };

  if constexpr (WLDS) {
    const unsigned* wsrc[2];
    int wdst[2];
#pragma unroll
    for (int i = 0; i < 2; ++i) {
      int u = i * THREADS + tid;
      if (u >= 384) u -= 128;
      const int pc = u >> 7, rem = u & 127;
      wsrc[i] = p.wp3 + (size_t)pc * w_piece + (size_t)(co0 + (rem >> 1)) * 8 + (rem & 1) * 4;
      wdst[i] = u;
    }
    u32x4 wst[2];
    auto wload = [&](int c) {
      const size_t off = (size_t)min(c, nchunks - 1) * w_chunk;
#pragma unroll
      for (int i = 0; i < 2; ++i) wst[i] = *reinterpret_cast<const u32x4*>(wsrc[i] + off);
    };
    auto wstore = [&](int buf) {
#pragma unroll
      for (int i = 0; i < 2; ++i) sW[buf][wdst[i]] = wst[i];
    };
    auto wread = [&](u32x4 (&w)[MT][3], int buf) {
#pragma unroll
      for (int mt = 0; mt < MT; ++mt)
#pragma unroll
        for (int pc = 0; pc < 3; ++pc) w[mt][pc] = sW[buf][(pc * 64 + 32 * mt + l31) * 2 + h];
    };
    wload(0);
    load_x(xr[0], 0);
    wstore(0);
    __syncthreads();
    for (int c = 0; c < nchunks; c += 2) {
#pragma unroll
      for (int i = 0; i < 2; ++i) {
        if (c + i < nchunks) {
          wload(c + i + 1);
          load_x(xr[(i + 1) & 1], c + i + 1);
          wread(wr[0], i);
          mma(xr[i], wr[0]);
          wstore((i + 1) & 1);
          asm volatile("s_waitcnt lgkmcnt(0)\n\ts_barrier" ::: "memory");
        }
      }
    }
  } else {
#pragma unroll
    for (int i = 0; i < XD; ++i) load_x(xr[i], i);
    load_w(wr[0], 0);
    for (int c = 0; c < nchunks; c += XD + 1) {
#pragma unroll
      for (int i = 0; i < XD + 1; ++i) {
        if (c + i < nchunks) {
          load_x(xr[(i + XD) % (XD + 1)], c + i + XD);
          load_w(wr[(i + 1) & 1], c + i + 1);
          mma(xr[i], wr[i & 1]);
        }
      }
    }
  }

  const size_t blk = ((size_t)b * p.Cout) * p.HW + px0;
  const bool full = co0 + 64 <= p.Cout;
  const bool track = p.absmax_out != nullptr;
  unsigned amax = 0u;
#pragma unroll
  for (int mt = 0; mt < MT; ++mt) {
#pragma unroll
    for (int r0 = 0; r0 < 16; r0 += 8) {
      f32x2 res[8];
      float add[8];
      bool ok[8];
#pragma unroll
      for (int j = 0; j < 8; ++j) {
        const int r = r0 + j;
        const int co = co0 + 32 * mt + (r & 3) + 8 * (r >> 2) + 4 * h;
        ok[j] = full || co < p.Cout;
        const int cc = ok[j] ? co : 0;
        float a = 0.f;
        if (p.bias) a += p.bias[cc];
        if (p.addvec) a += p.addvec[(size_t)b * p.Cout + cc];
        add[j] = a;
        if (p.residual) res[j] = *reinterpret_cast<const f32x2*>(p.residual + blk + (size_t)cc * p.HW + 2u * l31);
      }
#pragma unroll
      for (int j = 0; j < 8; ++j) {
        const int r = r0 + j;
        const int co = co0 + 32 * mt + (r & 3) + 8 * (r >> 2) + 4 * h;
        f32x2 v = {acc[mt][0][r], acc[mt][1][r]};
        v += add[j];
        if (p.residual) v += res[j];
        if (ok[j]) *reinterpret_cast<f32x2*>(p.out + blk + (size_t)co * p.HW + 2u * l31) = v;
        if (track && ok[j]) {
          const unsigned v0 = __builtin_bit_cast(unsigned, v[0]) & 0x7fffffffu, v1 = __builtin_bit_cast(unsigned, v[1]) & 0x7fffffffu;
          const unsigned vm = v0 > v1 ? v0 : v1;
          amax = vm > amax ? vm : amax;
        }
      }
    }
  }
  if (track) {
#pragma unroll
    for (int o = 32; o > 0; o >>= 1) {
      const unsigned other = (unsigned)__shfl_xor((int)amax, o, 64);
      amax = other > amax ? other : amax;
    }
    if (lane == 0) atomicMax(&p.absmax_out[b], amax);
  }
}

}

namespace hdiff {

void launch_conv1x1_x3(const Conv1x1X3K& k, int B, hipStream_t stream) {
  dim3 grid(cdiv(k.Cout, 64), (unsigned)(k.HW / 256), B);
  hipLaunchKernelGGL(conv1x1_x3_kernel<true>, grid, dim3(THREADS), 0, stream, k);
}

}
```

### hybrid-diffusion-underwater-atmopheric-image-enhancement_amd/csrc/conv_igemm.hip

```cpp
#include <stdlib.h>

#include "common.h"
#include "conv_x3.h"
#include "device.h"

using namespace hdiff;

namespace {

constexpr int BM = 64;
constexpr int NTHREADS = 256;

struct ConvK {
  const float* x0;
  const float* x1;
  int C0, C1, Cin, H, W;
  const float* wp;
  int CinPad, CoutPad, Cout;
  const float* bias;
  const float* gn_scale;
  const float* gn_shift;
  const float* addvec;
  const float* residual;
  float* out;
// ... 406 lines not shown
  static uint64_t attr_mask = 0;
  if (first_use_on_device(attr_mask)) {
    (void)hipFuncSetAttribute(reinterpret_cast<const void*>(&conv_igemm_kernel<WN, CK, NXS, NWS, SPEC, TWOM, DROP>),
                              hipFuncAttributeMaxDynamicSharedMemorySize, 160 * 1024);
  }
  hipLaunchKernelGGL((conv_igemm_kernel<WN, CK, NXS, NWS, SPEC, TWOM, DROP>), grid, dim3(NTHREADS), lds_bytes, stream, k);
}

template <int WN, int CK, int NXS, int NWS, int SPEC>
int launch(const ConvK& k, int B, size_t lds_bytes, hipStream_t stream) {
  const int BN = 128 * WN;
  const int TW = 1 << k.tw_log2;
  const int tiles_y = cdiv(k.VH, BN / TW);
  dim3 grid(k.tiles_x * tiles_y, cdiv(k.Cout, BM), B * k.ksplit);
  (void)hipGetLastError();
  if (k.keep_bits != nullptr) {
    if (k.Cout > 32) launch_t<WN, CK, NXS, NWS, SPEC, true, true>(k, grid, lds_bytes, stream);
    else launch_t<WN, CK, NXS, NWS, SPEC, false, true>(k, grid, lds_bytes, stream);
  } else if (k.Cout > 32) launch_t<WN, CK, NXS, NWS, SPEC, true>(k, grid, lds_bytes, stream);
  else launch_t<WN, CK, NXS, NWS, SPEC, false>(k, grid, lds_bytes, stream);
  if (k.ksplit > 1) {
    const size_t n = (size_t)B * k.Cout * k.VH * k.VW;
    const int blocks = (int)((n + 255) / 256 < 2048 ? (n + 255) / 256 : 2048);
    hipLaunchKernelGGL(conv_splitk_reduce_kernel, dim3(blocks), dim3(256), 0, stream, k);
  }
  HDIFF_CHECK_LAUNCH("conv_igemm_kernel");
  return HDIFF_OK;
}

}

extern "C" int hdiff_pack_conv_weight(const float* w, float* wp, int mode, int Cout, int Cin, int KH, int KW, int ntaps,
                                      const int* tap_ky, const int* tap_kx, int CinPad, int CoutPad, int accumulate,
                                      hdiff_stream_t stream) {
  HDIFF_CHECK_ARG(w && wp && tap_ky && tap_kx, "pack_conv_weight: null pointer");
  HDIFF_CHECK_ARG(ntaps >= 1 && ntaps <= HDIFF_MAX_TAPS, "pack_conv_weight: ntaps %d out of range", ntaps);
  HDIFF_CHECK_ARG(CinPad >= Cin && CinPad % 8 == 0 && CoutPad >= Cout && CoutPad % 64 == 0,
                  "pack_conv_weight: CinPad %% 8 / CoutPad %% 64 violated (%d, %d)", CinPad, CoutPad);
  PackK p{};
  p.mode = mode; p.Cout = Cout; p.Cin = Cin; p.KH = KH; p.KW = KW; p.ntaps = ntaps;
  p.CinPad = CinPad; p.CoutPad = CoutPad; p.accumulate = accumulate;
  for (int t = 0; t < ntaps; ++t) {
    HDIFF_CHECK_ARG(tap_ky[t] < KH && tap_kx[t] < KW, "pack_conv_weight: tap %d outside the kernel", t);
    p.ky[t] = tap_ky[t];
    p.kx[t] = tap_kx[t];
  }
  const size_t n = (size_t)ntaps * CinPad * CoutPad;
  const int blocks = (int)((n + 255) / 256 < 4096 ? (n + 255) / 256 : 4096);
  (void)hipGetLastError();
  hipLaunchKernelGGL(pack_conv_weight_kernel, dim3(blocks), dim3(256), 0, (hipStream_t)stream, w, wp, p);
  HDIFF_CHECK_LAUNCH("pack_conv_weight_kernel");
  return HDIFF_OK;
}

namespace {

struct ConvCfg {
  ConvK k;
  int WN, CK;
  size_t lds;
  int64_t splitk_floats;
};

int configure(const hdiff_conv_desc* d, ConvCfg& c) {
  HDIFF_CHECK_ARG(d && d->x0 && d->wp && d->out, "conv2d_fwd: null pointer");
  HDIFF_CHECK_ARG(d->C1 == 0 || d->x1, "conv2d_fwd: C1 > 0 without x1");
  HDIFF_CHECK_ARG(d->ntaps >= 1 && d->ntaps <= HDIFF_MAX_TAPS, "conv2d_fwd: ntaps %d out of range", d->ntaps);
  HDIFF_CHECK_ARG(d->CinPad >= d->C0 + d->C1 && d->CinPad % 8 == 0 && d->CoutPad >= d->Cout && d->CoutPad % 64 == 0,
                  "conv2d_fwd: padded channel counts invalid (Cin %d CinPad %d Cout %d CoutPad %d)", d->C0 + d->C1,
                  d->CinPad, d->Cout, d->CoutPad);
  HDIFF_CHECK_ARG(d->B > 0 && d->H > 0 && d->W > 0 && d->VH > 0 && d->VW > 0 && d->in_stride >= 1 && d->in_stride <= 2,
                  "conv2d_fwd: bad geometry");
  HDIFF_CHECK_ARG((d->VH - 1) * d->out_sy + d->out_oy < d->OH && (d->VW - 1) * d->out_sx + d->out_ox < d->OW,
                  "conv2d_fwd: virtual grid maps outside the output tensor");
  HDIFF_CHECK_ARG((d->gn_scale == nullptr) == (d->gn_shift == nullptr), "conv2d_fwd: gn_scale/gn_shift must come together");
  HDIFF_CHECK_ARG((long)d->OH * d->OW < (1L << 25) && (long)d->VH * d->VW < (1L << 25),
                  "conv2d_fwd: planes of 2^25 pixels or more are not supported (32-bit element offsets inside a channel block)");

  ConvK& k = c.k;
  k = ConvK{};
  k.x0 = d->x0; k.x1 = d->x1; k.C0 = d->C0; k.C1 = d->C1; k.Cin = d->C0 + d->C1; k.H = d->H; k.W = d->W;
  k.wp = d->wp; k.CinPad = d->CinPad; k.CoutPad = d->CoutPad; k.Cout = d->Cout;
  k.bias = d->bias; k.gn_scale = d->gn_scale; k.gn_shift = d->gn_shift; k.addvec = d->addvec; k.residual = d->residual;
  k.out = d->out; k.OH = d->OH; k.OW = d->OW; k.VH = d->VH; k.VW = d->VW; k.in_stride = d->in_stride;
  k.out_sy = d->out_sy; k.out_oy = d->out_oy; k.out_sx = d->out_sx; k.out_ox = d->out_ox; k.ntaps = d->ntaps;
  k.B = d->B;

  int dy_min = d->tap_dy[0], dy_max = d->tap_dy[0], dx_min = d->tap_dx[0], dx_max = d->tap_dx[0];
  for (int t = 1; t < d->ntaps; ++t) {
    dy_min = d->tap_dy[t] < dy_min ? d->tap_dy[t] : dy_min;
    dy_max = d->tap_dy[t] > dy_max ? d->tap_dy[t] : dy_max;
    dx_min = d->tap_dx[t] < dx_min ? d->tap_dx[t] : dx_min;
    dx_max = d->tap_dx[t] > dx_max ? d->tap_dx[t] : dx_max;
  }
  k.dy_min = dy_min; k.dx_min = dx_min;

  c.WN = ((long)d->VH * d->VW >= 1024) ? 2 : 1;
  const int BN = 128 * c.WN;
  int twl = ceil_log2(d->VW);
  if (twl > 5) twl = 5;
  k.tw_log2 = twl;
  const int TW = 1 << twl;
  k.TH = BN / TW;
  k.tiles_x = cdiv(d->VW, TW);
  k.rows = k.TH < d->VH ? k.TH : d->VH;
  k.PH = (k.rows - 1) * d->in_stride + (dy_max - dy_min + 1);
  k.PW = (TW - 1) * d->in_stride + (dx_max - dx_min + 1);
  k.PWp = k.PW | 1;
  k.PLANE = k.PH * k.PWp;
  for (int t = 0; t < d->ntaps; ++t) k.tap_off[t] = (d->tap_dy[t] - dy_min) * k.PWp + (d->tap_dx[t] - dx_min);

  const int Cin = d->C0 + d->C1;
  auto slots_x = [&](int ck) { return cdiv(ck * k.PH * k.PW, NTHREADS); };
  auto slots_w = [&](int ck) { return cdiv(d->ntaps * ck * (BM / 4), NTHREADS); };
  auto lds_for = [&](int ck) {
    const int xfl = (ck * k.PLANE + 3) & ~3;
    return (size_t)(xfl + d->ntaps * ck * BM + 2 * Cin + 2 * BM) * sizeof(float);
  };
  c.CK = 0;
  if (slots_x(8) <= 12 && slots_w(8) <= 5 && lds_for(8) <= 64 * 1024 && (d->C1 == 0 || d->C0 % 8 == 0)) c.CK = 8;
  else if (slots_x(4) <= 20 && slots_w(4) <= 7 && lds_for(4) <= 96 * 1024 && (d->C1 == 0 || d->C0 % 4 == 0)) c.CK = 4;
  HDIFF_CHECK_ARG(c.CK != 0, "conv2d_fwd: no kernel configuration fits (taps %d, patch %dx%d, C0 %d)", d->ntaps, k.PH, k.PW,
                  d->C0);
  c.lds = lds_for(c.CK);
  k.XFLOATS = (c.CK * k.PLANE + 3) & ~3;
  k.WFLOATS = d->ntaps * c.CK * BM;
  k.nx = slots_x(c.CK);
  k.nw = slots_w(c.CK);

  const int chunks = d->CinPad / c.CK;
  const long blocks = (long)k.tiles_x * cdiv(d->VH, k.TH) * cdiv(d->Cout, BM) * d->B;
  int ksplit = 1;
  if (blocks < 192 && chunks >= 8) {
    ksplit = (int)((512 + blocks - 1) / blocks);
    if (ksplit > chunks / 2) ksplit = chunks / 2;
    if (ksplit > 32) ksplit = 32;
  }
  k.chunks_per_split = cdiv(chunks, ksplit);
  k.ksplit = cdiv(chunks, k.chunks_per_split);
  c.splitk_floats = (k.ksplit > 1) ? (int64_t)k.ksplit * d->B * d->Cout * d->VH * d->VW : 0;
  return HDIFF_OK;
}

}

namespace {

struct ConvRoute {
  int route;
  const hdiff_conv_range* range;
  const unsigned* pair_pack;
  int pair_taps;
  bool absmax_tail;
};

bool s2_5x5_geometry(const hdiff_conv_desc* d, bool identity) {
  if (d->ntaps != 25 || d->in_stride != 2 || d->gn_scale != nullptr || d->residual != nullptr) return false;
  if (!identity || d->VH != d->OH || d->VW != d->OW) return false;
  if (d->VH != (d->H - 1) / 2 + 1 || d->VW != (d->W - 1) / 2 + 1) return false;
  for (int t = 0; t < 25; ++t)
    if (d->tap_dy[t] != t / 5 - 2 || d->tap_dx[t] != t % 5 - 2) return false;
  return (long)d->H * d->W < (1L << 25);
}

bool x3_geometry(const hdiff_conv_desc* d, bool same) {
  if ((d->ntaps != 9 && d->ntaps != 6 && d->ntaps != 4) || d->in_stride != 1) return false;
  if (d->VH != d->H || d->VW != d->W) return false;
  const bool phase = d->out_sy == 2 && d->out_sx == 2 && (d->out_oy == 0 || d->out_oy == 1) && (d->out_ox == 0 || d->out_ox == 1) &&
                     d->OH == 2 * d->H && d->OW == 2 * d->W && d->residual == nullptr;
  if (!same && !phase) return false;
  unsigned seen = 0;
  for (int t = 0; t < d->ntaps; ++t) {
    if (d->tap_dy[t] < -1 || d->tap_dy[t] > 1 || d->tap_dx[t] < -1 || d->tap_dx[t] > 1) return false;
    const unsigned bit = 1u << ((d->tap_dy[t] + 1) * 3 + (d->tap_dx[t] + 1));
    if (seen & bit) return false;
    seen |= bit;
  }
  if (same)
    for (int t = 0; t < 9; ++t)
      if (d->ntaps != 9 || d->tap_dy[t] != t / 3 - 1 || d->tap_dx[t] != t % 3 - 1) return false;
  return true;
}

bool direct_1x1_geometry(const hdiff_conv_desc* d, bool same) {
  return d->ntaps == 1 && d->tap_dy[0] == 0 && d->tap_dx[0] == 0 && d->in_stride == 1 && d->gn_scale == nullptr && same &&
         d->VH == d->H && d->VW == d->W && (long)d->B * d->H * d->W >= 32768 && ((long)d->H * d->W) % 128 == 0 &&
         d->C0 % 2 == 0 && (long)(d->C0 + d->C1) * d->H * d->W < (1L << 30) && d->CinPad * d->CoutPad < (1 << 30);
}

ConvRoute conv_route(const hdiff_conv_desc* d, const hdiff_conv_range* r, bool dropout) {
  const bool split = hdiff::split_operands_on();
  if (!split || dropout) r = nullptr;
  auto take = [&](int route, const void* pack = nullptr, int taps = 0) {
    const bool tail = r != nullptr && r->absmax_out != nullptr && (route == HDIFF_CONV_ROUTE_IGEMM || route == HDIFF_CONV_ROUTE_DIRECT_1X1);
    return ConvRoute{route, r, (const unsigned*)pack, taps, tail};
  };
  const bool identity = d->out_sy == 1 && d->out_oy == 0 && d->out_sx == 1 && d->out_ox == 0;
  const bool same = identity && d->OH == d->H && d->OW == d->W;
  const bool word = r != nullptr && r->absmax_in != nullptr && d->gn_scale == nullptr;
  const int Cin = d->C0 + d->C1;
  const bool ch16 = Cin % 16 == 0 && (d->C1 == 0 || d->C0 % 16 == 0);
  const bool x3_fills = split && ch16 && Cin <= 4096 && (long)cdiv(d->VW, 32) * cdiv(d->VH, 8) * cdiv(d->Cout, 64) * d->B >= 192;

  if (x3_fills && word && r->wp_h2_s2 != nullptr && s2_5x5_geometry(d, identity)) return take(HDIFF_CONV_ROUTE_S2_PAIRS_WORD, r->wp_h2_s2, 25);
  if (x3_fills && x3_geometry(d, same)) {
    if (same && d->wp_h2 != nullptr && d->act_scale != nullptr) return take(HDIFF_CONV_ROUTE_X3_PAIRS_GN, d->wp_h2, 9);
    const void* by_word = !word ? nullptr : same ? d->wp_h2 : r->wp_h2_taps;
    if (by_word != nullptr) return take(HDIFF_CONV_ROUTE_X3_PAIRS_WORD, by_word, d->ntaps);
    if (d->wp_x3 != nullptr) return take(HDIFF_CONV_ROUTE_X3_TRIPLES);
  }
  if (direct_1x1_geometry(d, same)) {
    if (d->wp_x3 != nullptr && split && ch16 && ((long)d->H * d->W) % 256 == 0 && d->CoutPad % 64 == 0) return take(HDIFF_CONV_ROUTE_X3_1X1);
    return take(HDIFF_CONV_ROUTE_DIRECT_1X1);
  }
  return take(HDIFF_CONV_ROUTE_IGEMM);
}

}

extern "C" int hdiff_conv2d_fwd_workspace(const hdiff_conv_desc* d, int64_t* floats_out) {
  HDIFF_CHECK_ARG(floats_out, "conv2d_fwd_workspace: null pointer");
  ConvCfg c;
  const int rc = configure(d, c);
  if (rc != HDIFF_OK) return rc;
  *floats_out = conv_route(d, nullptr, false).route == HDIFF_CONV_ROUTE_IGEMM ? c.splitk_floats : 0;
  return HDIFF_OK;
}

namespace {
hdiff::ConvX3K x3_args(const hdiff_conv_desc* d, const ConvRoute& rt) {
  hdiff::ConvX3K q{};
  q.x0 = d->x0; q.x1 = d->x1; q.C0 = d->C0; q.C1 = d->C1; q.Cin = d->C0 + d->C1; q.H = d->VH; q.W = d->VW;
  q.wp3 = (const unsigned*)d->wp_x3; q.CoutPad = d->CoutPad; q.Cout = d->Cout; q.out = d->out; q.tiles_x = cdiv(d->VW, 32);
  q.OH = d->OH; q.OW = d->OW; q.out_sy = d->out_sy; q.out_oy = d->out_oy; q.out_sx = d->out_sx; q.out_ox = d->out_ox;
  q.in_s = d->in_stride; q.IH = d->H; q.IW = d->W;
  if (rt.pair_pack != nullptr) {
    q.wp3 = rt.pair_pack;
    q.w_scale = reinterpret_cast<const float*>(rt.pair_pack + (size_t)(q.Cin / 16) * rt.pair_taps * 2 * d->CoutPad * 8);
    q.one = 1.0f;
    if (rt.route == HDIFF_CONV_ROUTE_X3_PAIRS_GN) q.act_scale = d->act_scale;
    else q.absmax_in = rt.range->absmax_in;
  }
  return q;
}
}

static int conv2d_fwd_launch(const hdiff_conv_desc* d, ConvCfg& c, const ConvRoute& rt, const unsigned* keep_bits, float inv_keep,
                             hipStream_t s) {
  unsigned* const absmax_out = rt.range != nullptr ? rt.range->absmax_out : nullptr;
  (void)hipGetLastError();
  switch (rt.route) {
    case HDIFF_CONV_ROUTE_S2_PAIRS_WORD: {
      hdiff::ConvX3K q = x3_args(d, rt);
      const size_t per_tap = (size_t)(q.Cin / 16) * 2 * d->CoutPad * 8;
      size_t taps_before = 0;
      for (int g = 0; g < 4; ++g) {
        int ky[9], kx[9];
        q.in_oy = g >> 1; q.in_ox = g & 1;
        q.ntaps = hdiff::s2_plane_taps(q.in_oy, q.in_ox, ky, kx);
        for (int t = 0; t < q.ntaps; ++t) q.tap_off[t] = (((ky[t] - 2 - q.in_oy) / 2 + 1) * 34 + ((kx[t] - 2 - q.in_ox) / 2 + 1)) * 4;
        q.wp3 = rt.pair_pack + taps_before * per_tap;
        q.bias = g == 3 ? d->bias : nullptr;
        q.addvec = g == 3 ? d->addvec : nullptr;
        q.residual = g == 0 ? nullptr : d->out;
        q.residual_first = g != 0;
        q.absmax_out = g == 3 ? absmax_out : nullptr;
        hdiff::launch_conv3x3_x3(q, d->B, s);
        HDIFF_CHECK_LAUNCH("conv3x3_x3_kernel");
        taps_before += q.ntaps;
      }
      return HDIFF_OK;
    }
    case HDIFF_CONV_ROUTE_X3_TRIPLES:
    case HDIFF_CONV_ROUTE_X3_PAIRS_GN:
    case HDIFF_CONV_ROUTE_X3_PAIRS_WORD: {
      hdiff::ConvX3K q = x3_args(d, rt);
      q.absmax_out = absmax_out;
      q.bias = d->bias; q.gn_scale = d->gn_scale; q.gn_shift = d->gn_shift; q.addvec = d->addvec; q.residual = d->residual;
      q.ntaps = d->ntaps;
      for (int t = 0; t < d->ntaps; ++t) q.tap_off[t] = ((d->tap_dy[t] + 1) * 34 + (d->tap_dx[t] + 1)) * 4;
      q.keep_bits = keep_bits; q.inv_keep = inv_keep;
      hdiff::launch_conv3x3_x3(q, d->B, s);
      HDIFF_CHECK_LAUNCH("conv3x3_x3_kernel");
      return HDIFF_OK;
    }
    case HDIFF_CONV_ROUTE_X3_1X1: {
      const hdiff::Conv1x1X3K q{d->x0, d->x1, d->C0, d->C0 + d->C1, (long)d->H * d->W, (const unsigned*)d->wp_x3, d->CoutPad, d->Cout,
                                d->bias, d->addvec, d->residual, d->out, absmax_out};
      hdiff::launch_conv1x1_x3(q, d->B, s);
      HDIFF_CHECK_LAUNCH("conv1x1_x3_kernel");
      return HDIFF_OK;
    }
    case HDIFF_CONV_ROUTE_DIRECT_1X1: {
      const hdiff::Conv1x1K q{d->x0, d->x1, d->C0, d->C0 + d->C1, (long)d->H * d->W, d->wp, d->CoutPad, d->Cout, d->bias, d->addvec,
                              d->residual, d->out};
      hdiff::launch_conv1x1_direct(q, d->B, s);
      HDIFF_CHECK_LAUNCH("conv1x1_direct_kernel");
      return HDIFF_OK;
    }
    default: break;
  }
  ConvK& k = c.k;
  k.keep_bits = keep_bits;
  k.inv_keep = inv_keep;
  if (k.ksplit > 1 && d->splitk_ws != nullptr && d->splitk_floats >= c.splitk_floats) {
    k.partial = d->splitk_ws;
  } else {
    k.ksplit = 1;
    k.chunks_per_split = d->CinPad / c.CK;
    k.partial = nullptr;
  }
  bool spec = c.WN == 2 && c.CK == 8 && d->ntaps == 9 && d->in_stride == 1 && k.tw_log2 == 5 && k.PWp == 35 && k.PLANE == 350;
  for (int t = 0; spec && t < 9; ++t) spec = k.tap_off[t] == (t / 3) * 35 + (t % 3);
  const long long hw = (long long)d->H * d->W;
  if (4 * hw * (d->C0 > d->C1 ? d->C0 : d->C1) >= (1ll << 31)) spec = false;
  if (spec) return launch<2, 8, 12, 5, 1>(k, d->B, c.lds, s);
  if (c.WN == 2 && c.CK == 8) return launch<2, 8, 12, 5, 0>(k, d->B, c.lds, s);
  if (c.WN == 2 && c.CK == 4) return launch<2, 4, 20, 7, 0>(k, d->B, c.lds, s);
  if (c.WN == 1 && c.CK == 8) return launch<1, 8, 12, 5, 0>(k, d->B, c.lds, s);
  return launch<1, 4, 20, 7, 0>(k, d->B, c.lds, s);
}

namespace {
struct OutAbsmaxK {
  const float* out;
  unsigned* words;
  int Cout, VH, VW, OH, OW, sy, oy, sx, ox;
};
__global__ __launch_bounds__(256) void conv_out_absmax_kernel(const OutAbsmaxK q) {
  const int b = blockIdx.y;
  const long plane = (long)q.VH * q.VW, n = plane * q.Cout;
  const float* base = q.out + (size_t)b * q.Cout * q.OH * q.OW;
  unsigned m = 0u;
  for (long i = (long)blockIdx.x * blockDim.x + threadIdx.x; i < n; i += (long)gridDim.x * blockDim.x) {
    const long co = i / plane, pix = i - co * plane;
    const int vy = (int)(pix / q.VW), vx = (int)(pix - (long)vy * q.VW);
    const float v = base[((size_t)co * q.OH + (size_t)(vy * q.sy + q.oy)) * q.OW + (size_t)(vx * q.sx + q.ox)];
    const unsigned vb = __builtin_bit_cast(unsigned, v) & 0x7fffffffu;
    m = vb > m ? vb : m;
  }
#pragma unroll
  for (int o = 32; o > 0; o >>= 1) {
    const unsigned other = (unsigned)__shfl_xor((int)m, o, 64);
    m = other > m ? other : m;
  }
  if ((threadIdx.x & 63) == 0) atomicMax(&q.words[b], m);
}
}

static int check_range(const hdiff_conv_desc* d, const hdiff_conv_range* r) {
  HDIFF_CHECK_ARG(d && r, "conv2d_fwd_range: null pointer");
  HDIFF_CHECK_ARG(((uintptr_t)r->absmax_out & 3u) == 0 && ((uintptr_t)r->absmax_in & 3u) == 0,
                  "conv2d_fwd_range: absmax_out / absmax_in are not aligned to 32-bit words");
  HDIFF_CHECK_ARG(r->absmax_in == nullptr || (const void*)r->absmax_in != (const void*)r->absmax_out,
                  "conv2d_fwd_range: absmax_in and absmax_out are the same words (a launch cannot read the range it is writing)");
  HDIFF_CHECK_ARG(r->absmax_in == nullptr || d->gn_scale == nullptr,
                  "conv2d_fwd_range: absmax_in describes x0 / x1 as stored, not the output of the GroupNorm + Swish prologue "
                  "(use act_scale)");
  HDIFF_CHECK_ARG(r->wp_h2_taps == nullptr || r->absmax_in != nullptr, "conv2d_fwd_range: wp_h2_taps without absmax_in (the pair form needs the range)");
  HDIFF_CHECK_ARG(r->wp_h2_taps == nullptr || (d->ntaps >= 1 && d->ntaps <= 9),
                  "conv2d_fwd_range: wp_h2_taps holds a tap list of at most 9 taps (ntaps %d)", d->ntaps);
  HDIFF_CHECK_ARG(r->wp_h2_s2 == nullptr || r->absmax_in != nullptr, "conv2d_fwd_range: wp_h2_s2 without absmax_in (the pair form needs the range)");
  HDIFF_CHECK_ARG(r->wp_h2_s2 == nullptr || (d->ntaps == 25 && d->in_stride == 2),
                  "conv2d_fwd_range: wp_h2_s2 is the pack of a 25-tap stride-2 conv (ntaps %d, in_stride %d)", d->ntaps, d->in_stride);
  return HDIFF_OK;
}

static int check_dropout(const hdiff_conv_desc* d) {
  HDIFF_CHECK_ARG(d->x1 == nullptr && d->C1 == 0, "conv2d_fwd_dropout: a concat input (x1) is not supported");
  HDIFF_CHECK_ARG(d->gn_scale != nullptr && d->gn_shift != nullptr, "conv2d_fwd_dropout: needs the GroupNorm + Swish prologue (gn_scale / gn_shift)");
  bool plain = d->ntaps == 9 && d->in_stride == 1 && d->VH == d->H && d->VW == d->W && d->OH == d->H && d->OW == d->W &&
               d->out_sy == 1 && d->out_oy == 0 && d->out_sx == 1 && d->out_ox == 0;
  for (int t = 0; plain && t < 9; ++t) plain = d->tap_dy[t] == t / 3 - 1 && d->tap_dx[t] == t % 3 - 1;
  HDIFF_CHECK_ARG(plain, "conv2d_fwd_dropout: not a plain 3x3 / stride-1 / pad-1 convolution (nine taps in row-major order, output grid = input grid)");
  HDIFF_CHECK_ARG(d->C0 > 0 && d->C0 % 8 == 0, "conv2d_fwd_dropout: C0 = %d is not a multiple of 8", d->C0);
  HDIFF_CHECK_ARG(d->B > 0 && d->H > 0 && d->W > 0 && (long long)d->B * d->C0 * d->H * d->W < (1ll << 31),
                  "conv2d_fwd_dropout: inputs of 2^31 elements or more are not supported (32-bit bit indices)");
  return HDIFF_OK;
}

static int conv2d_fwd(const hdiff_conv_desc* d, const hdiff_conv_range* r, const unsigned* keep_bits, float inv_keep,
                      hdiff_stream_t stream) {
  ConvCfg c;
  int rc = configure(d, c);
  if (rc != HDIFF_OK) return rc;
  const ConvRoute rt = conv_route(d, r, keep_bits != nullptr);
  rc = conv2d_fwd_launch(d, c, rt, keep_bits, inv_keep, (hipStream_t)stream);
  if (rc != HDIFF_OK || !rt.absmax_tail) return rc;
  const OutAbsmaxK q{d->out, rt.range->absmax_out, d->Cout, d->VH, d->VW, d->OH, d->OW, d->out_sy, d->out_oy, d->out_sx, d->out_ox};
  const long n = (long)d->Cout * d->VH * d->VW;
  const int blocks = (int)((n + 1023) / 1024 < 256 ? (n + 1023) / 1024 : 256);
  hipLaunchKernelGGL(conv_out_absmax_kernel, dim3(blocks, d->B), dim3(256), 0, (hipStream_t)stream, q);
  HDIFF_CHECK_LAUNCH("conv_out_absmax_kernel");
  return HDIFF_OK;
}

extern "C" int hdiff_conv2d_fwd(const hdiff_conv_desc* d, hdiff_stream_t stream) { return conv2d_fwd(d, nullptr, nullptr, 1.0f, stream); }

extern "C" int hdiff_conv2d_fwd_range(const hdiff_conv_desc* d, const hdiff_conv_range* r, hdiff_stream_t stream) {
  const int rc = check_range(d, r);
  return rc != HDIFF_OK ? rc : conv2d_fwd(d, r, nullptr, 1.0f, stream);
}

extern "C" int hdiff_conv2d_fwd_dropout(const hdiff_conv_desc* d, const uint32_t* keep_bits, float inv_keep, hdiff_stream_t stream) {
  HDIFF_CHECK_ARG(d && keep_bits, "conv2d_fwd_dropout: null pointer");
  HDIFF_CHECK_ARG(inv_keep >= 1.0f && inv_keep <= 3.0e38f, "conv2d_fwd_dropout: inv_keep = %g is not a finite 1 / keep with keep in (0, 1]",
                  (double)inv_keep);
  const int rc = check_dropout(d);
  return rc != HDIFF_OK ? rc : conv2d_fwd(d, nullptr, keep_bits, inv_keep, stream);
}

extern "C" int hdiff_conv2d_fwd_route(const hdiff_conv_desc* d, const hdiff_conv_range* r, int dropout, int* route_out,
                                      int* absmax_tail_out) {
  HDIFF_CHECK_ARG(d && route_out && absmax_tail_out, "conv2d_fwd_route: null pointer");
  HDIFF_CHECK_ARG(!(dropout && r), "conv2d_fwd_route: the dropout form takes no range struct");
  ConvCfg c;
  int rc = r != nullptr ? check_range(d, r) : dropout ? check_dropout(d) : HDIFF_OK;
  if (rc == HDIFF_OK) rc = configure(d, c);
  if (rc != HDIFF_OK) return rc;
  const ConvRoute rt = conv_route(d, r, dropout != 0);
  *route_out = rt.route;
  *absmax_tail_out = rt.absmax_tail;
  return HDIFF_OK;
}

namespace {
__global__ void range_words_zero_kernel(unsigned* __restrict__ words, int n) {
  for (int i = blockIdx.x * blockDim.x + threadIdx.x; i < n; i += gridDim.x * blockDim.x) words[i] = 0u;
}
}

extern "C" int hdiff_range_words_zero(uint32_t* words, int n, hdiff_stream_t stream) {
  HDIFF_CHECK_ARG(words && n > 0, "range_words_zero: null pointer or n = %d", n);
  (void)hipGetLastError();
  hipLaunchKernelGGL(range_words_zero_kernel, dim3(n < 4096 ? (n + 255) / 256 : 16), dim3(256), 0, (hipStream_t)stream, words, n);
  HDIFF_CHECK_LAUNCH("range_words_zero_kernel");
  return HDIFF_OK;
}
```

### hybrid-diffusion-underwater-atmopheric-image-enhancement_amd/csrc/conv_x3.h

```cpp
#pragma once
#include <hip/hip_runtime.h>

namespace hdiff {

struct ConvX3K {
  const float* x0;
  const float* x1;
  int C0, C1, Cin, H, W;
  const unsigned* wp3;
  int CoutPad, Cout;
  const float* bias;
  const float* gn_scale;
  const float* gn_shift;
  const float* addvec;
  const float* residual;
  float* out;
  int tiles_x;
  int ntaps;
  int tap_off[9];
  int OH, OW, out_sy, out_oy, out_sx, out_ox;
  const float* act_scale;
  const float* w_scale;
  float one;
  const unsigned* keep_bits;
  float inv_keep;
  unsigned* absmax_out;
  const unsigned* absmax_in;
  int in_s, in_oy, in_ox, IH, IW;
  int residual_first;
};
void launch_conv3x3_x3(const ConvX3K& k, int B, hipStream_t stream);
int s2_plane_taps(int oy, int ox, int* ky, int* kx);

struct Conv1x1X3K {
  const float* x0;
  const float* x1;
  int C0, Cin;
  long HW;
  const unsigned* wp3;
  int CoutPad, Cout;
  const float* bias;
  const float* addvec;
  const float* residual;
  float* out;
  unsigned* absmax_out;
};
void launch_conv1x1_x3(const Conv1x1X3K& k, int B, hipStream_t stream);

struct Conv1x1K {
  const float* x0;
  const float* x1;
  int C0, Cin;
  long HW;
  const float* wp;
  int CoutPad, Cout;
  const float* bias;
  const float* addvec;
  const float* residual;
  float* out;
};
void launch_conv1x1_direct(const Conv1x1K& k, int B, hipStream_t stream);

}
```

### hybrid-diffusion-underwater-atmopheric-image-enhancement_amd/engine.py

```python
from __future__ import annotations

import ctypes as C
from dataclasses import dataclass
from typing import Callable, Dict, List, Optional, Sequence, Tuple

import torch

from . import _capi

GN_GROUPS = 32
GN_EPS = 1e-5
NUM_HEADS = 8
FLASH_MAX_HEAD = 64


RESERVE_SPLIT_WORKSPACE = True


def _ptr(t: Optional[torch.Tensor]) -> Optional[int]:
    return None if t is None else t.data_ptr()


def _pad(v: int, m: int) -> int:
    return (v + m - 1) // m * m
# ... 53 lines not shown
            t.kx.append(kx)
    return t


PLAIN_3X3 = "plain 3x3"
PLAIN_3X3_T = "plain 3x3 transposed"
TAPS_3X3 = "3x3-neighbourhood tap list"
ONE_TAP = "one tap"
S2_5X5 = "row-major 5x5"
OTHER = "other"


class PackedConv:

    def __init__(self, device, cout: int, cin: int, taps: TapSet):
        self.cout, self.cin, self.taps = cout, cin, taps
        self.cin_pad, self.cout_pad = _pad(cin, 8), _pad(cout, 64)
        self.ntaps = len(taps.dy)
        self.wp = torch.empty(self.ntaps * self.cin_pad * self.cout_pad, dtype=torch.float32, device=device)
        self.sources: List[Tuple[torch.Tensor, int, int, int, List[int], List[int], int]] = []
        row_major_5x5 = self.ntaps == 25 and all(dy == t // 5 - 2 and dx == t % 5 - 2 for t, (dy, dx) in enumerate(zip(taps.dy, taps.dx)))
        self.kind = S2_5X5 if row_major_5x5 and cin % 16 == 0 else OTHER
        self.wp3: Optional[torch.Tensor] = None
        self._x3_src: Optional[torch.Tensor] = None
        self._x3_layout: Optional[Tuple[int, int, int]] = None
        self.wp2: Optional[torch.Tensor] = None
        self.act_scale: Optional[torch.Tensor] = None
        self._gn: Optional[Tuple[torch.Tensor, torch.Tensor, int, float]] = None

    def _pair_buffer(self, size_query: str, *args) -> torch.Tensor:
        words = C.c_int64(0)
        _capi.check(getattr(_capi.lib(), size_query)(self.cout, self.cin, self.cout_pad, *args, C.byref(words)),
                    size_query[len("hdiff_"):])
        return torch.empty(words.value, dtype=torch.int32, device=self.wp.device)

    def launch_ptrs(self, act_range: Optional[Tuple[torch.Tensor, torch.Tensor, int, float]], has_absmax_in: bool, in_stride: int,
                    out_map: Tuple[int, int, int, int]) -> Tuple[Optional[int], ...]:
        same = in_stride == 1 and out_map == (1, 0, 1, 0)
        wp_h2 = act_scale = wp_h2_taps = wp_h2_s2 = None
        if act_range is not None and self.kind == PLAIN_3X3:
            if same:
                self._serve_gn(*act_range)
            wp_h2, act_scale = _ptr(self.wp2), _ptr(self.act_scale)
        if has_absmax_in and in_stride == 1 and self.kind in (TAPS_3X3, ONE_TAP):
            if self.wp2 is None and self.kind == TAPS_3X3:
                self.wp2 = self._pair_buffer("hdiff_pack_conv_weight_h2_taps_words", self.ntaps)
            wp_h2_taps = _ptr(self.wp2)
        elif has_absmax_in and same and self.kind == PLAIN_3X3:
            if self._gn is not None:
                raise RuntimeError("PackedConv.enable_h2_words: this pack already stages activations behind a GroupNorm")
            if self.wp2 is None:
                self.wp2 = self._pair_buffer("hdiff_pack_conv_weight_h2_words")
            wp_h2 = _ptr(self.wp2)
        elif has_absmax_in and in_stride == 2 and self.kind == S2_5X5:
            if self.wp2 is None:
                self.wp2 = self._pair_buffer("hdiff_pack_conv_weight_h2_s2_words")
            wp_h2_s2 = _ptr(self.wp2)
        return _ptr(self.wp3), wp_h2, act_scale, wp_h2_taps, wp_h2_s2

    def _serve_gn(self, gamma: torch.Tensor, beta: torch.Tensor, group_elems: int, gain: float = 1.0) -> None:
        gn = (gamma, beta, int(group_elems), float(gain))
        ident = lambda g: (g[0].data_ptr(), g[1].data_ptr(), g[2], g[3])
        if self.wp2 is None:
            self.wp2 = self._pair_buffer("hdiff_pack_conv_weight_h2_words")
            self.act_scale = torch.empty(2, dtype=torch.float32, device=self.wp.device)
            self._gn = gn
        elif self._gn is None:
            raise RuntimeError("PackedConv.enable_h2: this pack already serves a conv that takes its range from a word")
        elif ident(self._gn) != ident(gn):
            raise RuntimeError("PackedConv.enable_h2: this pack already stages activations for another GroupNorm / gain; "
                               "use one PackedConv per (convolution, GroupNorm) pair")

    def enable_x3(self, w: torch.Tensor, transposed: bool = False) -> None:
        if self.ntaps == 9 and self.cin % 16 == 0 and tuple(w.shape[2:]) == (3, 3):
            self.wp3 = torch.empty((self.cin // 16) * 9 * 3 * self.cout_pad * 8, dtype=torch.int32, device=self.wp.device)
            self._x3_src = w
            self.kind = PLAIN_3X3_T if transposed else PLAIN_3X3

    def enable_x3_taps(self, w: torch.Tensor, mode: int) -> None:
        if self.ntaps in (1, 4, 6, 9) and self.cin % 16 == 0 and all(-1 <= v <= 1 for v in self.taps.dy + self.taps.dx):
            self.wp3 = torch.empty((self.cin // 16) * self.ntaps * 3 * self.cout_pad * 8, dtype=torch.int32, device=self.wp.device)
            self._x3_src = w
            self._x3_layout = (int(mode), int(w.shape[2]), int(w.shape[3]))
            self.kind = ONE_TAP if self.ntaps == 1 else TAPS_3X3

    def add_source(self, w: torch.Tensor, mode: int, ky: Sequence[int], kx: Sequence[int], accumulate: int) -> None:
        kh, kw = int(w.shape[2]), int(w.shape[3])
        self.sources.append((w, mode, kh, kw, list(ky), list(kx), accumulate))

    def pack(self, stream: int) -> None:
        lib = _capi.lib()
        taps = lambda ky, kx: ((C.c_int * self.ntaps)(*ky), (C.c_int * self.ntaps)(*kx))
        for w, mode, kh, kw, ky, kx, acc in self.sources:
            require_gpu_tensor(w, "conv weight")
            _capi.check(lib.hdiff_pack_conv_weight(w.data_ptr(), self.wp.data_ptr(), mode, self.cout, self.cin, kh, kw,
                                                   self.ntaps, *taps(ky, kx), self.cin_pad, self.cout_pad, acc, stream),
                        "pack_conv_weight")
        if self.kind in (TAPS_3X3, ONE_TAP):
            mode, kh, kw = self._x3_layout
            tail = (mode, self.cout, self.cin, kh, kw, self.ntaps, *taps(self.taps.ky, self.taps.kx), self.cout_pad, stream)
            _capi.check(lib.hdiff_pack_conv_weight_x3_taps(self._x3_src.data_ptr(), self.wp3.data_ptr(), *tail), "pack_conv_weight_x3_taps")
            if self.wp2 is not None:
                _capi.check(lib.hdiff_pack_conv_weight_h2_taps(self._x3_src.data_ptr(), self.wp2.data_ptr(), *tail), "pack_conv_weight_h2_taps")
        elif self.kind in (PLAIN_3X3, PLAIN_3X3_T):
            _capi.check(lib.hdiff_pack_conv_weight_x3(self._x3_src.data_ptr(), self.wp3.data_ptr(), self.cout, self.cin,
                                                      self.cout_pad, int(self.kind == PLAIN_3X3_T), stream), "pack_conv_weight_x3")
            if self.wp2 is not None:
                _capi.check(lib.hdiff_pack_conv_weight_h2(self._x3_src.data_ptr(), self.wp2.data_ptr(), self.cout, self.cin,
                                                          self.cout_pad, stream), "pack_conv_weight_h2")
            if self._gn is not None:
                gamma, beta, group_elems, gain = self._gn
                _capi.check(lib.hdiff_gn_act_scale(gamma.data_ptr(), beta.data_ptr(), int(gamma.numel()), C.c_int64(group_elems),
                                                   C.c_float(gain), self.act_scale.data_ptr(), stream), "gn_act_scale")
        elif self.wp2 is not None:
            _capi.check(lib.hdiff_pack_conv_weight_h2_s2(self.wp.data_ptr(), self.wp2.data_ptr(), self.cout, self.cin, self.cin_pad,
                                                         self.cout_pad, stream), "pack_conv_weight_h2_s2")


class Plan:

    def __init__(self, device: torch.device):
        self.device = torch.device(device)
        if self.device.type != "cuda":
            raise RuntimeError("hdiff: plans run on an MI355X device only (no CPU fallback)")
        self.lib = _capi.lib()
        self.ops: List[Tuple[str, Callable, tuple]] = []
        self.packs: List[PackedConv] = []
        self._gn_src: Dict[int, Tuple[torch.Tensor, torch.Tensor, int, float]] = {}
        self._pool: Dict[int, List[torch.Tensor]] = {}
        self._all: List[torch.Tensor] = []
        self._keep: List[object] = []
        self.graph = C.c_void_p(None)
        self._graph_stream: Optional[torch.cuda.Stream] = None
        self.flops = 0.0
        self._vec_jobs: List[tuple] = []
        self._words: Optional[torch.Tensor] = None
        self._words_used = 0

    def buf(self, *shape: int, dtype=torch.float32) -> torch.Tensor:
        n = 1
        for s in shape:
            n *= int(s)
        key = n * (8 if dtype == torch.int64 else 4)
        free = self._pool.get(key)
        if free:
            base = free.pop()
        else:
            base = torch.empty(key // 4, dtype=torch.float32, device=self.device)
            self._all.append(base)
        t = base.view(dtype)[:n].view(*shape) if dtype != torch.float32 else base[:n].view(*shape)
        t._hdiff_base = base
        return t

    RANGE_WORDS = 4096

    def range_words(self, B: int) -> torch.Tensor:
        if self._words is None:
            self._words = torch.zeros(self.RANGE_WORDS, dtype=torch.int32, device=self.device)
            self.call("hdiff_range_words_zero", self._words.data_ptr(), self.RANGE_WORDS)
        if self._words_used + B > self.RANGE_WORDS:
            raise RuntimeError(f"hdiff: a plan holds at most {self.RANGE_WORDS} range words")
        w = self._words[self._words_used:self._words_used + B]
        self._words_used += B
        return w

    def free(self, t: torch.Tensor) -> None:
        base = getattr(t, "_hdiff_base", None)
        if base is not None:
            self._pool.setdefault(base.numel() * 4, []).append(base)

    def bytes_allocated(self) -> int:
        return sum(b.numel() * 4 for b in self._all)

    def call(self, name: str, *args) -> None:
        self.ops.append((name, getattr(self.lib, name), args))

    def keep(self, obj) -> None:
        self._keep.append(obj)

    def run(self, stream: Optional[int] = None) -> None:
        assert not self._vec_jobs, "flush_block_vecs() was not called for this plan"
        with torch.cuda.device(self.device):
            s = torch.cuda.current_stream(self.device).cuda_stream if stream is None else stream
            for name, fn, args in self.ops:
                rc = fn(*args, s)
                if rc != 0:
                    _capi.check(rc, name)

    def pack_weights(self, stream: Optional[int] = None) -> None:
        with torch.cuda.device(self.device):
            s = torch.cuda.current_stream(self.device).cuda_stream if stream is None else stream
            for p in self.packs:
                p.pack(s)

    def capture(self) -> None:
        if self.graph.value:
            return
        with torch.cuda.device(self.device):
            torch.cuda.synchronize(self.device)
            self._graph_stream = torch.cuda.Stream(self.device)
            s = self._graph_stream.cuda_stream
            _capi.check(self.lib.hdiff_graph_begin(s), "graph_begin")
            try:
                self.run(s)
            finally:
                rc = self.lib.hdiff_graph_end(s, C.byref(self.graph))
            _capi.check(rc, "graph_end")

    def replay(self, stream: Optional[int] = None) -> None:
        with torch.cuda.device(self.device):
            s = torch.cuda.current_stream(self.device).cuda_stream if stream is None else stream
            _capi.check(self.lib.hdiff_graph_launch(self.graph, s), "graph_launch")

    def __del__(self):
        try:
            if self.graph.value:
                self.lib.hdiff_graph_destroy(self.graph)
        except Exception:
            pass

    def conv(self, x0: torch.Tensor, x1: Optional[torch.Tensor], pk: PackedConv, bias: Optional[torch.Tensor],
             out: torch.Tensor, *, B: int, H: int, W: int, VH: int, VW: int, in_stride: int = 1,
             out_map: Tuple[int, int, int, int] = (1, 0, 1, 0), gn: Optional[Tuple[torch.Tensor, torch.Tensor]] = None,
             addvec: Optional[torch.Tensor] = None, residual: Optional[torch.Tensor] = None,
             act_range: Optional[Tuple[torch.Tensor, torch.Tensor, int, float]] = None,
             dropout: Optional[Tuple[torch.Tensor, float]] = None,
             absmax_out: Optional[torch.Tensor] = None, absmax_in: Optional[torch.Tensor] = None) -> None:
        d = _capi.ConvDesc()
        C0 = int(x0.shape[1])
        C1 = int(x1.shape[1]) if x1 is not None else 0
        assert C0 + C1 == pk.cin, (C0, C1, pk.cin)
        d.x0, d.x1, d.C0, d.C1 = _ptr(x0), _ptr(x1), C0, C1
        d.B, d.H, d.W = B, H, W
        d.wp, d.bias = pk.wp.data_ptr(), _ptr(bias)
        d.Cout, d.CinPad, d.CoutPad = pk.cout, pk.cin_pad, pk.cout_pad
        d.gn_scale, d.gn_shift = (_ptr(gn[0]), _ptr(gn[1])) if gn is not None else (None, None)
        d.addvec, d.residual, d.out = _ptr(addvec), _ptr(residual), out.data_ptr()
        d.OH, d.OW = int(out.shape[2]), int(out.shape[3])
        d.VH, d.VW, d.in_stride = VH, VW, in_stride
        d.out_sy, d.out_oy, d.out_sx, d.out_ox = out_map
        d.ntaps = pk.ntaps
        if act_range is None and gn is not None:
            act_range = self._gn_src.get(id(gn[0]))
        assert (absmax_out is None and absmax_in is None) or (dropout is None and (absmax_in is None or gn is None))
        d.wp_x3, d.wp_h2, d.act_scale, wp_h2_taps, wp_h2_s2 = pk.launch_ptrs(act_range, absmax_in is not None, in_stride, out_map)
        r = None
        if absmax_out is not None or absmax_in is not None:
            r = _capi.ConvRange()
            r.absmax_out, r.absmax_in, r.wp_h2_taps, r.wp_h2_s2 = _ptr(absmax_out), _ptr(absmax_in), wp_h2_taps, wp_h2_s2
        for i in range(pk.ntaps):
            d.tap_dy[i], d.tap_dx[i] = pk.taps.dy[i], pk.taps.dx[i]
        need = C.c_int64(0)
        _capi.check(self.lib.hdiff_conv2d_fwd_workspace(C.byref(d), C.byref(need)), "conv2d_fwd_workspace")
        ws = None
        if need.value > 0:
            ws = self.buf(need.value)
            d.splitk_ws, d.splitk_floats = ws.data_ptr(), need.value
        self.keep((d, x0, x1, pk, bias, out, gn, addvec, residual, ws, dropout, r, absmax_out, absmax_in))
        self.flops += 2.0 * pk.ntaps * pk.cin * pk.cout * VH * VW * B
        if dropout is not None:
            self.call("hdiff_conv2d_fwd_dropout", C.byref(d), dropout[0].data_ptr(), C.c_float(dropout[1]))
        elif r is not None:
            self.call("hdiff_conv2d_fwd_range", C.byref(d), C.byref(r))
        else:
            self.call("hdiff_conv2d_fwd", C.byref(d))
        if ws is not None:
            self.free(ws)

    def attention_workspace(self, B: int, Cc: int, heads: int, L: int) -> Optional[torch.Tensor]:
        if not RESERVE_SPLIT_WORKSPACE:
            return None
        need = C.c_int64(0)
        _capi.check(self.lib.hdiff_mha_flash_fwd_workspace(B, Cc, heads, L, C.byref(need)), "mha_flash_fwd_workspace")
        return self.buf((need.value + 3) // 4) if need.value > 0 else None

    def flash_attention(self, qkv: torch.Tensor, o: torch.Tensor, B: int, Cc: int, heads: int, L: int) -> None:
        ws = self.attention_workspace(B, Cc, heads, L)
        self.call("hdiff_mha_flash_fwd_ws", qkv.data_ptr(), o.data_ptr(), None, B, Cc, heads, L, _ptr(ws),
                  C.c_int64(0 if ws is None else ws.numel() * 4))
        self.keep(ws)
        if ws is not None:
            self.free(ws)

    def gn_scale_shift(self, x0: torch.Tensor, x1: Optional[torch.Tensor], gamma: torch.Tensor, beta: torch.Tensor,
                       B: int, HW: int) -> Tuple[torch.Tensor, torch.Tensor]:
        C0 = int(x0.shape[1])
        C1 = int(x1.shape[1]) if x1 is not None else 0
        Ct = C0 + C1
        if Ct % GN_GROUPS != 0:
            raise RuntimeError(f"Expected number of channels in input to be divisible by num_groups, got {Ct}")
        nsplit = max(1, min(32, HW // 4096))
        ws = self.buf(B * GN_GROUPS * nsplit * 3)
        scale, shift = self.buf(B, Ct), self.buf(B, Ct)
        self.call("hdiff_gn_scale_shift", _ptr(x0), _ptr(x1), C0, C1, B, HW, GN_GROUPS, nsplit, ws.data_ptr(),
                  gamma.data_ptr(), beta.data_ptr(), C.c_float(GN_EPS), scale.data_ptr(), shift.data_ptr())
        self.keep((x0, x1, gamma, beta, ws))
        self.free(ws)
        self._gn_src[id(scale)] = (gamma, beta, (Ct // GN_GROUPS) * HW, 1.0)
        return scale, shift

    def block_vec(self, temb: torch.Tensor, cemb: Optional[torch.Tensor], P: Dict[str, torch.Tensor], p: str, B: int,
                  cout: int) -> torch.Tensor:
        vec = torch.empty(B, cout, dtype=torch.float32, device=self.device)
        wc = P[f"{p}.cond_proj.1.weight"] if cemb is not None else None
        bc = P[f"{p}.cond_proj.1.bias"] if cemb is not None else None
        self._vec_jobs.append((P[f"{p}.temb_proj.1.weight"], P[f"{p}.temb_proj.1.bias"], wc, bc, vec))
        return vec

    def flush_block_vecs(self, pos: int, temb: torch.Tensor, cemb: Optional[torch.Tensor], B: int) -> None:
        if not self._vec_jobs:
            return
        jobs = (_capi.LinearJob * len(self._vec_jobs))()
        first = 0
        for j, (wt, bt, wc, bc, vec) in enumerate(self._vec_jobs):
            jobs[j].w0, jobs[j].b0, jobs[j].w1, jobs[j].b1 = wt.data_ptr(), bt.data_ptr(), _ptr(wc), _ptr(bc)
            jobs[j].y, jobs[j].n, jobs[j].first = vec.data_ptr(), int(wt.shape[0]), first
            first += int(wt.shape[0])
        raw = bytes(jobs)
        table = torch.frombuffer(bytearray(raw), dtype=torch.uint8).to(self.device)
        K = int(self._vec_jobs[0][0].shape[1])
        if int(temb.shape[1]) != K or (cemb is not None and int(cemb.shape[1]) != K):
            raise RuntimeError(f"block projections: embedding width {tuple(temb.shape)} / "
                               f"{None if cemb is None else tuple(cemb.shape)} does not match the weights' {K}")
        for wt, _, wc, _, _ in self._vec_jobs:
            if int(wt.shape[1]) != K or (wc is not None and int(wc.shape[1]) != K):
                raise RuntimeError("block projections: temb_proj / cond_proj weights of different input widths in one model")
        self.keep((table, temb, cemb, list(self._vec_jobs)))
        self.ops.insert(pos, ("hdiff_linear_rows_multi", getattr(self.lib, "hdiff_linear_rows_multi"),
                              (temb.data_ptr(), _ptr(cemb), table.data_ptr(), len(self._vec_jobs), first, B, K)))
        self._vec_jobs = []

    def linear(self, x: torch.Tensor, idx: Optional[torch.Tensor], W: torch.Tensor, bias: Optional[torch.Tensor],
               y: torch.Tensor, B: int, swish_input: bool, accumulate: bool) -> None:
        N, K = int(W.shape[0]), int(W.shape[1])
        self.keep((x, idx, W, bias, y))
        n_rows = int(x.shape[0]) if idx is not None else 0
        self.call("hdiff_linear_rows", x.data_ptr(), _ptr(idx), n_rows, W.data_ptr(), _ptr(bias), y.data_ptr(), B, K, N,
                  int(swish_input), int(accumulate))


@dataclass
class UNetShape:
    T: int
    num_labels: int
    ch: int
    ch_mult: Tuple[int, ...]
    num_res_blocks: int


def _new_pack(plan: Plan, cout: int, cin: int, taps: TapSet) -> PackedConv:
    pk = PackedConv(plan.device, cout, cin, taps)
    plan.packs.append(pk)
    return pk


def _std_pack(plan: Plan, w: torch.Tensor, k: int, pad: int) -> PackedConv:
    taps = conv_taps(k, pad)
    pk = _new_pack(plan, int(w.shape[0]), int(w.shape[1]), taps)
    pk.add_source(w, 0, taps.ky, taps.kx, 0)
    if k == 3 and pad == 1:
        pk.enable_x3(w)
    elif k == 1 and pad == 0:
        pk.enable_x3_taps(w, 0)
    return pk


def emit_embed_mlp(plan: Plan, P: Dict[str, torch.Tensor], prefix: str, idx: torch.Tensor, B: int) -> torch.Tensor:
    w1, b1, w2, b2 = P[f"{prefix}.1.weight"], P[f"{prefix}.1.bias"], P[f"{prefix}.3.weight"], P[f"{prefix}.3.bias"]
    h = plan.buf(B, int(w1.shape[0]))
    out = plan.buf(B, int(w2.shape[0]))
    plan.linear(P[f"{prefix}.0.weight"], idx, w1, b1, h, B, swish_input=False, accumulate=False)
    plan.linear(h, None, w2, b2, out, B, swish_input=True, accumulate=False)
    plan.free(h)
    return out


def emit_mha(plan: Plan, P: Dict[str, torch.Tensor], p: str, h: torch.Tensor, B: int, Cc: int, H: int, W: int,
             absmax_out: Optional[torch.Tensor] = None) -> torch.Tensor:
    if Cc % NUM_HEADS != 0:
        raise AssertionError("embed_dim must be divisible by num_heads")
    w_in = P[f"{p}.attn.in_proj_weight"].view(3 * Cc, Cc, 1, 1)
    w_out = P[f"{p}.attn.out_proj.weight"].view(Cc, Cc, 1, 1)
    pk_in, pk_out = _std_pack(plan, w_in, 1, 0), _std_pack(plan, w_out, 1, 0)
    qkv = plan.buf(B, 3 * Cc, H, W)
    plan.conv(h, None, pk_in, P[f"{p}.attn.in_proj_bias"], qkv, B=B, H=H, W=W, VH=H, VW=W)
    o = plan.buf(B, Cc, H, W)
    plan.flash_attention(qkv, o, B, Cc, NUM_HEADS, H * W)
    plan.flops += 4.0 * (H * W) ** 2 * Cc * B
    plan.keep((qkv, o))
    plan.free(qkv)
    y = plan.buf(B, Cc, H, W)
    plan.conv(o, None, pk_out, P[f"{p}.attn.out_proj.bias"], y, B=B, H=H, W=W, VH=H, VW=W, absmax_out=absmax_out)
    plan.free(o)
    return y


def emit_attn_block(plan: Plan, P: Dict[str, torch.Tensor], p: str, x: torch.Tensor, B: int, Cc: int, H: int, W: int) -> torch.Tensor:
    L = H * W
    scale, shift = plan.gn_scale_shift(x, None, P[f"{p}.group_norm.weight"], P[f"{p}.group_norm.bias"], B, L)
    hn = plan.buf(B, Cc, H, W)
    plan.call("hdiff_gn_affine_apply", x.data_ptr(), scale.data_ptr(), shift.data_ptr(), hn.data_ptr(), B, Cc, L)
    plan.keep((x, scale, shift, hn))
    plan.free(scale); plan.free(shift)
    w_qkv = torch.cat([P[f"{p}.proj_q.weight"], P[f"{p}.proj_k.weight"], P[f"{p}.proj_v.weight"]], dim=0).detach().contiguous()
    b_qkv = torch.cat([P[f"{p}.proj_q.bias"], P[f"{p}.proj_k.bias"], P[f"{p}.proj_v.bias"]], dim=0).detach().contiguous()
    plan.keep((w_qkv, b_qkv))
    pk_in = _std_pack(plan, w_qkv, 1, 0)
    qkv = plan.buf(B, 3 * Cc, H, W)
    plan.conv(hn, None, pk_in, b_qkv, qkv, B=B, H=H, W=W, VH=H, VW=W)
    plan.free(hn)
    o = plan.buf(B, Cc, H, W)
    if Cc <= FLASH_MAX_HEAD:
        plan.flash_attention(qkv, o, B, Cc, 1, L)
    else:
        plan.call("hdiff_mha_wide_fwd", qkv.data_ptr(), o.data_ptr(), B, Cc, L)
    plan.flops += 4.0 * L * L * Cc * B
    plan.keep((qkv, o))
    plan.free(qkv)
    pk_out = _std_pack(plan, P[f"{p}.proj.weight"], 1, 0)
    y = plan.buf(B, Cc, H, W)
    plan.conv(o, None, pk_out, P[f"{p}.proj.bias"], y, B=B, H=H, W=W, VH=H, VW=W, residual=x)
    plan.free(o)
    return y


def emit_resblock(plan: Plan, P: Dict[str, torch.Tensor], p: str, xa: torch.Tensor, xb: Optional[torch.Tensor],
                  temb: torch.Tensor, cemb: Optional[torch.Tensor], cout: int, B: int, H: int, W: int, attn: bool,
                  absmax_out: Optional[torch.Tensor] = None) -> torch.Tensor:
    sc1 = plan.gn_scale_shift(xa, xb, P[f"{p}.block1.0.weight"], P[f"{p}.block1.0.bias"], B, H * W)
    vec = plan.block_vec(temb, cemb, P, p, B, cout)
    pk1 = _std_pack(plan, P[f"{p}.block1.2.weight"], 3, 1)
    h1 = plan.buf(B, cout, H, W)
    plan.conv(xa, xb, pk1, P[f"{p}.block1.2.bias"], h1, B=B, H=H, W=W, VH=H, VW=W, gn=sc1, addvec=vec)
    plan.free(sc1[0]); plan.free(sc1[1])

    sc2 = plan.gn_scale_shift(h1, None, P[f"{p}.block2.0.weight"], P[f"{p}.block2.0.bias"], B, H * W)
    if f"{p}.shortcut.weight" in P:
        pks = _std_pack(plan, P[f"{p}.shortcut.weight"], 1, 0)
        res = plan.buf(B, cout, H, W)
        plan.conv(xa, xb, pks, P[f"{p}.shortcut.bias"], res, B=B, H=H, W=W, VH=H, VW=W)
        res_owned = True
    else:
        assert xb is None
        res, res_owned = xa, False
    pk2 = _std_pack(plan, P[f"{p}.block2.3.weight"], 3, 1)
    h2 = plan.buf(B, cout, H, W)
    plan.conv(h1, None, pk2, P[f"{p}.block2.3.bias"], h2, B=B, H=H, W=W, VH=H, VW=W, gn=sc2, residual=res,
              absmax_out=None if attn else absmax_out)
    plan.free(sc2[0]); plan.free(sc2[1]); plan.free(h1)
    if res_owned:
        plan.free(res)
    if attn:
        y = emit_mha(plan, P, p, h2, B, cout, H, W, absmax_out=absmax_out)
        plan.free(h2)
        return y
    return h2


def emit_downsample(plan: Plan, P: Dict[str, torch.Tensor], p: str, x: torch.Tensor, B: int, Cc: int, H: int, W: int,
                    x_absmax: Optional[torch.Tensor] = None) -> torch.Tensor:
    taps = conv_taps(5, 2)
    pk = _new_pack(plan, Cc, Cc, taps)
    pk.add_source(P[f"{p}.c2.weight"], 0, taps.ky, taps.kx, 0)
    ky3 = [ky - 1 if (1 <= ky <= 3 and 1 <= kx <= 3) else -1 for ky, kx in zip(taps.ky, taps.kx)]
    kx3 = [kx - 1 if (1 <= ky <= 3 and 1 <= kx <= 3) else 0 for ky, kx in zip(taps.ky, taps.kx)]
    pk.add_source(P[f"{p}.c1.weight"], 0, ky3, kx3, 1)
    OH, OW = (H - 1) // 2 + 1, (W - 1) // 2 + 1
    bias = plan.buf(Cc)
    plan.call("hdiff_axpby", C.c_float(1.0), P[f"{p}.c1.bias"].data_ptr(), C.c_float(1.0), P[f"{p}.c2.bias"].data_ptr(),
              bias.data_ptr(), Cc)
    plan.keep((P[f"{p}.c1.bias"], P[f"{p}.c2.bias"]))
    y = plan.buf(B, Cc, OH, OW)
    plan.conv(x, None, pk, bias, y, B=B, H=H, W=W, VH=OH, VW=OW, in_stride=2, absmax_in=x_absmax)
    plan.free(bias)
    return y


def emit_upsample(plan: Plan, P: Dict[str, torch.Tensor], p: str, x: torch.Tensor, B: int, Cc: int, H: int, W: int,
                  x_absmax: Optional[torch.Tensor] = None) -> torch.Tensor:
    wt = P[f"{p}.t.weight"]
    u = plan.buf(B, Cc, 2 * H, 2 * W)
    u_absmax = plan.range_words(B)
    for py in (0, 1):
        for px in (0, 1):
            taps = tconv_phase_taps(py, px)
            pk = _new_pack(plan, Cc, Cc, taps)
            pk.add_source(wt, 1, taps.ky, taps.kx, 0)
            pk.enable_x3_taps(wt, 1)
            plan.conv(x, None, pk, P[f"{p}.t.bias"], u, B=B, H=H, W=W, VH=H, VW=W, out_map=(2, py, 2, px),
                      absmax_out=u_absmax, absmax_in=x_absmax)
    pkc = _std_pack(plan, P[f"{p}.c.weight"], 3, 1)
    y = plan.buf(B, Cc, 2 * H, 2 * W)
    plan.conv(u, None, pkc, P[f"{p}.c.bias"], y, B=B, H=2 * H, W=2 * W, VH=2 * H, VW=2 * W, absmax_in=u_absmax)
    plan.free(u)
    return y


class UNetPlan:

    def __init__(self, P: Dict[str, torch.Tensor], shape: UNetShape, B: int, H: int, W: int, device):
        if H % (2 ** (len(shape.ch_mult) - 1)) or W % (2 ** (len(shape.ch_mult) - 1)):
            raise RuntimeError(f"Sizes of tensors must match: H, W = {H}, {W} not divisible by "
                               f"{2 ** (len(shape.ch_mult) - 1)}")
        plan = Plan(device)
        self.plan, self.B, self.H, self.W = plan, B, H, W
        self.x = plan.buf(B, 3, H, W)
        self.t = plan.buf(B, dtype=torch.int64)
        self.labels = plan.buf(B, dtype=torch.int64)
        ch = shape.ch
        temb = emit_embed_mlp(plan, P, "time_embedding.timembedding", self.t, B)
        cemb = emit_embed_mlp(plan, P, "cond_embedding.condEmbedding", self.labels, B)
        vec_pos = len(plan.ops)

        pk_head = _std_pack(plan, P["head.weight"], 3, 1)
        h = plan.buf(B, ch, H, W)
        plan.conv(self.x, None, pk_head, P["head.bias"], h, B=B, H=H, W=W, VH=H, VW=W)
        hs: List[Tuple[torch.Tensor, int, int, int]] = [(h, ch, H, W)]
        now, cH, cW = ch, H, W
        n_down = 0
        for i, mult in enumerate(shape.ch_mult):
            out = ch * mult
            h_absmax = None
            for j in range(shape.num_res_blocks):
                if i != len(shape.ch_mult) - 1 and j == shape.num_res_blocks - 1:
                    h_absmax = plan.range_words(B)
                h = emit_resblock(plan, P, f"downblocks.{n_down}", h, None, temb, cemb, out, B, cH, cW, attn=True,
                                  absmax_out=h_absmax)
                n_down += 1
                now = out
                hs.append((h, now, cH, cW))
            if i != len(shape.ch_mult) - 1:
                h = emit_downsample(plan, P, f"downblocks.{n_down}", h, B, now, cH, cW, x_absmax=h_absmax)
                n_down += 1
                cH, cW = (cH - 1) // 2 + 1, (cW - 1) // 2 + 1
                hs.append((h, now, cH, cW))
        hm = emit_resblock(plan, P, "middleblocks.0", h, None, temb, cemb, now, B, cH, cW, attn=True)
        h = emit_resblock(plan, P, "middleblocks.1", hm, None, temb, cemb, now, B, cH, cW, attn=False)
        plan.free(hm)
        n_up = 0
        for i, mult in reversed(list(enumerate(shape.ch_mult))):
# ... 144 lines not shown
```

### include/hdiff.h

```cpp
#ifndef HDIFF_H_
#define HDIFF_H_

#include <stdint.h>

#ifdef __cplusplus
extern "C" {
#endif

typedef void* hdiff_stream_t;

enum hdiff_status {
  HDIFF_OK = 0,
  HDIFF_ERR_INVALID = -1,
  HDIFF_ERR_LAUNCH = -2,
  HDIFF_ERR_NO_DEVICE = -3
};

int hdiff_abi_version(void);
const char* hdiff_last_error(void);
int hdiff_device_count(void);
enum { HDIFF_CONTRACT_F32 = 0, HDIFF_CONTRACT_BF16X3 = 1, HDIFF_CONTRACT_F16 = 2 };
int hdiff_set_contraction_mode(int mode);
int hdiff_get_contraction_mode(void);


#define HDIFF_MAX_TAPS 25

int hdiff_pack_conv_weight(const float* w, float* wp, int mode, int Cout, int Cin, int KH, int KW, int ntaps,
                           const int* tap_ky, const int* tap_kx, int CinPad, int CoutPad, int accumulate,
                           hdiff_stream_t stream);

int hdiff_pack_conv_weight_x3(const float* w, void* wp3, int Cout, int Cin, int CoutPad, int transposed,
                              hdiff_stream_t stream);
int hdiff_pack_conv_weight_x3_taps(const float* w, void* wp3, int mode, int Cout, int Cin, int KH, int KW, int ntaps,
                                   const int* tap_ky, const int* tap_kx, int CoutPad, hdiff_stream_t stream);
int hdiff_pack_conv_weight_h2_words(int Cout, int Cin, int CoutPad, int64_t* words_out);
int hdiff_pack_conv_weight_h2(const float* w, void* wp2, int Cout, int Cin, int CoutPad, hdiff_stream_t stream);
int hdiff_pack_conv_weight_h2_taps_words(int Cout, int Cin, int CoutPad, int ntaps, int64_t* words_out);
int hdiff_pack_conv_weight_h2_taps(const float* w, void* wp2, int mode, int Cout, int Cin, int KH, int KW, int ntaps,
                                   const int* tap_ky, const int* tap_kx, int CoutPad, hdiff_stream_t stream);
int hdiff_pack_conv_weight_h2_s2_words(int Cout, int Cin, int CoutPad, int64_t* words_out);
int hdiff_pack_conv_weight_h2_s2(const float* wp, void* wp2, int Cout, int Cin, int CinPad, int CoutPad, hdiff_stream_t stream);
int hdiff_gn_act_scale(const float* gamma, const float* beta, int C, int64_t group_elems, float gain, float* out2,
                       hdiff_stream_t stream);

typedef struct hdiff_conv_desc {
  const float* x0;
  const float* x1;
  int C0, C1;
  int B, H, W;
  const float* wp;
  const float* bias;
  int Cout, CinPad, CoutPad;
  const float* gn_scale;
  const float* gn_shift;
  const float* addvec;
  const float* residual;
  float* out;
  int OH, OW;
  int VH, VW;
  int in_stride;
  int out_sy, out_oy, out_sx, out_ox;
  int ntaps;
  int tap_dy[HDIFF_MAX_TAPS];
  int tap_dx[HDIFF_MAX_TAPS];
  float* splitk_ws;
  int64_t splitk_floats;
  const void* wp_x3;
  const void* wp_h2;
  const float* act_scale;
} hdiff_conv_desc;

int hdiff_conv2d_fwd_workspace(const hdiff_conv_desc* d, int64_t* floats_out);
int hdiff_conv2d_fwd(const hdiff_conv_desc* d, hdiff_stream_t stream);
int hdiff_conv2d_fwd_dropout(const hdiff_conv_desc* d, const uint32_t* keep_bits, float inv_keep, hdiff_stream_t stream);

typedef struct hdiff_conv_range {
  uint32_t* absmax_out;
  const uint32_t* absmax_in;
  const void* wp_h2_taps;
  const void* wp_h2_s2;
} hdiff_conv_range;
int hdiff_conv2d_fwd_range(const hdiff_conv_desc* d, const hdiff_conv_range* r, hdiff_stream_t stream);
int hdiff_range_words_zero(uint32_t* words, int n, hdiff_stream_t stream);

enum {
  HDIFF_CONV_ROUTE_IGEMM = 0,
  HDIFF_CONV_ROUTE_DIRECT_1X1 = 1,
  HDIFF_CONV_ROUTE_X3_1X1 = 2,
  HDIFF_CONV_ROUTE_X3_TRIPLES = 3,
  HDIFF_CONV_ROUTE_X3_PAIRS_GN = 4,
  HDIFF_CONV_ROUTE_X3_PAIRS_WORD = 5,
  HDIFF_CONV_ROUTE_S2_PAIRS_WORD = 6
};
int hdiff_conv2d_fwd_route(const hdiff_conv_desc* d, const hdiff_conv_range* r, int dropout, int* route_out, int* absmax_tail_out);

typedef struct hdiff_conv_wgrad_desc {
  const float* x0;
  const float* x1;
  int C0, C1;
  int B, H, W;
  const float* gn_scale;
  const float* gn_shift;
  const float* dy;
  int Cout, CinPad, CoutPad;
  int OH, OW;
  int VH, VW;
  int in_stride;
  int out_sy, out_oy, out_sx, out_ox;
  int ntaps;
  int tap_dy[HDIFF_MAX_TAPS];
  int tap_dx[HDIFF_MAX_TAPS];
} hdiff_conv_wgrad_desc;
int hdiff_conv2d_wgrad_workspace(const hdiff_conv_wgrad_desc* d, int* nsplit_out, int64_t* floats_out);
int hdiff_conv2d_wgrad(const hdiff_conv_wgrad_desc* d, float* dwp, int nsplit, hdiff_stream_t stream);
int hdiff_conv2d_wgrad_dropout(const hdiff_conv_wgrad_desc* d, const uint32_t* keep_bits, float inv_keep, float* dwp, int nsplit,
                               hdiff_stream_t stream);
enum {
  HDIFF_WGRAD_ROUTE_FAST_1X1 = 0,
  HDIFF_WGRAD_ROUTE_FAST_3X3 = 1,
  HDIFF_WGRAD_ROUTE_GENERIC = 2,
  HDIFF_WGRAD_ROUTE_GENERIC_ROWS1 = 3,
  HDIFF_WGRAD_ROUTE_GENERIC_ROWS2 = 4
};
int hdiff_conv2d_wgrad_route(const hdiff_conv_wgrad_desc* d, int dropout, int* route_out);
int hdiff_conv_wgrad_unpack(const float* dwp, int nsplit, float* dw, int mode, int Cout, int Cin, int KH, int KW, int ntaps,
                            const int* tap_ky, const int* tap_kx, int CinPad, int CoutPad, int accumulate,
                            hdiff_stream_t stream);

int hdiff_gn_stats(const float* x0, const float* x1, int C0, int C1, int B, int HW, int G, int nsplit, float* ws,
                   hdiff_stream_t stream);
int hdiff_gn_finalize(const float* ws, int B, int C, int G, int nsplit, const float* gamma, const float* beta, float eps,
                      float* scale, float* shift, float* mean_out , float* rstd_out ,
                      hdiff_stream_t stream);
int hdiff_gn_scale_shift(const float* x0, const float* x1, int C0, int C1, int B, int HW, int G, int nsplit, float* ws,
                         const float* gamma, const float* beta, float eps, float* scale, float* shift,
                         hdiff_stream_t stream);
int hdiff_gn_swish_bwd(const float* x0, const float* x1, int C0, int C1, int B, int HW, int G, const float* dA,
                       const float* mean, const float* rstd, const float* gamma, const float* beta, float* ws, float* dx0,
                       float* dx1, float* dgamma, float* dbeta, hdiff_stream_t stream);
int hdiff_gn_swish_dropout_bwd(const float* x, int C, int B, int HW, int G, const float* dA, const uint32_t* keep_bits,
                               float inv_keep, const float* mean, const float* rstd, const float* gamma, const float* beta,
                               float* ws, float* dx, float* dgamma, float* dbeta, hdiff_stream_t stream);
int hdiff_gn_affine_bwd(const float* x, int C, int B, int HW, int G, const float* dY, const float* mean, const float* rstd,
                        const float* gamma, const float* beta, float* ws, float* dx, float* dgamma, float* dbeta,
                        hdiff_stream_t stream);
int hdiff_bias_addvec_grad(const float* dy, int B, int C, int HW, float* dvec, float* dbias, hdiff_stream_t stream);
int hdiff_gn_affine_apply(const float* x, const float* scale, const float* shift, float* y, int B, int C, int HW,
                          hdiff_stream_t stream);
int hdiff_gn_swish_apply(const float* x, const float* scale, const float* shift, float* y, int B, int C, int HW,
                         hdiff_stream_t stream);

int hdiff_mha_flash_fwd(const float* qkv, float* o, float* lse2 , int B, int C, int heads, int L,
                        hdiff_stream_t stream);
int hdiff_mha_flash_fwd_workspace(int B, int C, int heads, int L, int64_t* bytes_out);
int hdiff_mha_flash_fwd_ws(const float* qkv, float* o, float* lse2 , int B, int C, int heads, int L,
                           void* ws, int64_t ws_bytes, hdiff_stream_t stream);
enum {
  HDIFF_MHA_FWD_ROUTE_RUNNING_MAX = 0,
  HDIFF_MHA_FWD_ROUTE_FAST_F32 = 1,
  HDIFF_MHA_FWD_ROUTE_X3_TRIPLES = 2,
  HDIFF_MHA_FWD_ROUTE_H2_PAIRS = 3,
  HDIFF_MHA_FWD_ROUTE_X3P_PAIRS = 4,
  HDIFF_MHA_FWD_ROUTE_F16_SINGLE = 5
};
int hdiff_mha_flash_fwd_route(int B, int C, int heads, int L, int want_lse, int64_t ws_bytes, int* route_out, int* nq_out,
                              int* check_out);
int hdiff_mha_wide_fwd(const float* qkv, float* o, int B, int C, int L, hdiff_stream_t stream);
int hdiff_mha_wide_bwd(const float* qkv, const float* d_o, float* dqkv, float* ws, int B, int C, int L, hdiff_stream_t stream);
int hdiff_mha_flash_bwd_workspace(int B, int C, int heads, int L, int64_t* n_floats);
int hdiff_mha_flash_bwd(const float* qkv, const float* o, const float* d_o, const float* lse2, float* delta, float* dqkv,
                        float* ws, int B, int C, int heads, int L, hdiff_stream_t stream);
enum {
  HDIFF_MHA_BWD_ROUTE_FUSED_F32 = 0,
  HDIFF_MHA_BWD_ROUTE_H2_PAIRS = 1
};
int hdiff_mha_flash_bwd_route(int B, int C, int heads, int L, int* route_out, int* nk_out, int* aligned_out, int* nsplit_out);

int hdiff_linear_rows(const float* x, const int64_t* idx, int n_rows, const float* W, const float* bias, float* y, int B,
                      int K, int N, int swish_input, int accumulate, hdiff_stream_t stream);
typedef struct hdiff_linear_job {
  const float* w0; const float* b0; const float* w1; const float* b1; float* y;
  int n; int first;
} hdiff_linear_job;
int hdiff_linear_rows_multi(const float* x0 , const float* x1 , const hdiff_linear_job* jobs,
                            int njobs, int total_n, int B, int K, hdiff_stream_t stream);

int hdiff_linear_rows_bwd(const float* x, const int64_t* idx, int n_rows, const float* W, const float* dy, float* dx,
                          float* dW, float* db, int B, int K, int N, int swish_input, int accumulate, int pad_row,
                          hdiff_stream_t stream);

int hdiff_q_sample(const float* x0, const float* noise, const int64_t* t, const float* sqrt_ab, const float* sqrt_1mab,
                   float* xt, int B, int per_sample, int T, hdiff_stream_t stream);
int hdiff_sq_err(const float* a, const float* b, float* out, int64_t n, hdiff_stream_t stream);
int hdiff_sq_err_bwd(const float* a, const float* b, const float* dloss, float* da, int64_t n, hdiff_stream_t stream);
int hdiff_ddpm_step(const float* x, const float* eps_c, const float* eps_u, const float* noise, float* x_next,
                    const float* coeff1, const float* coeff2, const float* sigma, const int32_t* step_ptr,
                    int T , double w,
                    uint64_t seed, int32_t* nan_flag, int64_t n, hdiff_stream_t stream);
typedef struct hdiff_ddpm_loop_desc {
  const float* x; const float* eps_c; const float* eps_u;
  const float* noise;
  float* x_next;
  const float* coeff1; const float* coeff2; const float* sigma;
  int32_t* step_ptr;
  int T;
  double w;
  uint64_t seed;
  int32_t* nan_flag;
  int64_t n;
  float* x_dup0; float* x_dup1;
  int64_t* t_next; int t_count;
  uint32_t* done_counter;
} hdiff_ddpm_loop_desc;
int hdiff_ddpm_step_loop(const hdiff_ddpm_loop_desc* d, hdiff_stream_t stream);
int hdiff_cfg_ddim_step(const float* x, const float* eps_c, const float* eps_u, const float* noise, float* x_next,
                        const float* tab , const int32_t* step_ptr, int nsteps, double w, int clip_x0,
                        uint64_t seed, int32_t* nan_flag, int64_t n, hdiff_stream_t stream);
typedef struct hdiff_cfg_ddim_loop_desc {
  const float* x; const float* eps_c; const float* eps_u;
  const float* noise;
  float* x_next;
  const float* tab;
  const int64_t* t_tab;
  int32_t* step_ptr;
  int nsteps;
  int clip_x0;
  double w;
  uint64_t seed;
  int32_t* nan_flag;
  int64_t n;
  float* x_dup0; float* x_dup1;
  int64_t* t_next; int t_count;
  uint32_t* done_counter;
} hdiff_cfg_ddim_loop_desc;
int hdiff_cfg_ddim_step_loop(const hdiff_cfg_ddim_loop_desc* d, hdiff_stream_t stream);
int hdiff_cfg_dpmpp_step(const float* x, const float* eps_c, const float* eps_u, float* x_next, float* x0_prev,
// ... 104 lines not shown
```

Before: 3.031.

## Compute QKV per-head maxima in projection conv and fuse Q/K/V split kernels

The QKV input projection conv now records per-head Q/K absolute maxima and per-channel V maxima, either inside the epilogue or through a follow-up max kernel. Attention then uses these precomputed maxima in a single fused qkv_split kernel, replacing the separate row-max pass, qk split and v split launches. This saves rereading the QKV tensor and several launches per attention block. In exchange it adds atomic max traffic in the conv, and the range-word pool grows to hold the maxima.

After: 3.038 (median of 6 runs). About the same (+0.2%).

```diff
diff --git a/hybrid-diffusion-underwater-atmopheric-image-enhancement_amd/_capi.py b/hybrid-diffusion-underwater-atmopheric-image-enhancement_amd/_capi.py
--- a/hybrid-diffusion-underwater-atmopheric-image-enhancement_amd/_capi.py
+++ b/hybrid-diffusion-underwater-atmopheric-image-enhancement_amd/_capi.py
@@ -65,6 +65,10 @@
 class ConvRange(C.Structure):
     _fields_ = [("absmax_out", C.c_void_p), ("absmax_in", C.c_void_p), ("wp_h2_taps", C.c_void_p),
                 ("wp_h2_s2", C.c_void_p)]
+
+
+class QkvMax(C.Structure):
+    _fields_ = [("qk_max", C.c_void_p), ("v_max", C.c_void_p), ("heads", C.c_int)]
 
 
 class MsssimDesc(C.Structure):
@@ -107,6 +111,7 @@
     "hdiff_conv2d_fwd": (C.c_int, [C.POINTER(ConvDesc), C.c_void_p]),
     "hdiff_conv2d_fwd_dropout": (C.c_int, [C.POINTER(ConvDesc), C.c_void_p, C.c_float, C.c_void_p]),
     "hdiff_conv2d_fwd_range": (C.c_int, [C.POINTER(ConvDesc), C.POINTER(ConvRange), C.c_void_p]),
+    "hdiff_conv2d_fwd_qkv": (C.c_int, [C.POINTER(ConvDesc), C.POINTER(ConvRange), C.POINTER(QkvMax), C.c_void_p]),
     "hdiff_range_words_zero": (C.c_int, [C.c_void_p, C.c_int, C.c_void_p]),
     "hdiff_conv2d_fwd_route": (C.c_int, [C.POINTER(ConvDesc), C.POINTER(ConvRange), C.c_int, C.POINTER(C.c_int), C.POINTER(C.c_int)]),
     "hdiff_pack_conv_weight_h2_taps_words": (C.c_int, [C.c_int, C.c_int, C.c_int, C.c_int, C.POINTER(C.c_int64)]),
@@ -127,6 +132,8 @@
     "hdiff_mha_flash_fwd_workspace": (C.c_int, [C.c_int, C.c_int, C.c_int, C.c_int, C.POINTER(C.c_int64)]),
     "hdiff_mha_flash_fwd_ws": (C.c_int, [C.c_void_p, C.c_void_p, C.c_void_p, C.c_int, C.c_int, C.c_int, C.c_int, C.c_void_p,
                                          C.c_int64, C.c_void_p]),
+    "hdiff_mha_flash_fwd_ws_max": (C.c_int, [C.c_void_p, C.c_void_p, C.c_void_p, C.c_int, C.c_int, C.c_int, C.c_int, C.c_void_p,
+                                             C.c_int64, C.c_void_p, C.c_void_p, C.c_void_p]),
     "hdiff_mha_flash_fwd_route": (C.c_int, [C.c_int, C.c_int, C.c_int, C.c_int, C.c_int, C.c_int64] + [C.POINTER(C.c_int)] * 3),
     "hdiff_mha_wide_fwd": (C.c_int, [C.c_void_p, C.c_void_p, C.c_int, C.c_int, C.c_int, C.c_void_p]),
     "hdiff_mha_wide_bwd": (C.c_int, [C.c_void_p, C.c_void_p, C.c_void_p, C.c_void_p, C.c_int, C.c_int, C.c_int, C.c_void_p]),
diff --git a/hybrid-diffusion-underwater-atmopheric-image-enhancement_amd/csrc/attention.hip b/hybrid-diffusion-underwater-atmopheric-image-enhancement_amd/csrc/attention.hip
--- a/hybrid-diffusion-underwater-atmopheric-image-enhancement_amd/csrc/attention.hip
+++ b/hybrid-diffusion-underwater-atmopheric-image-enhancement_amd/csrc/attention.hip
@@ -476,16 +476,16 @@
 }
 
 template <int D>
-void launch_d(const float* qkv, float* o, float* lse2, int B, int C, int heads, int L, void* ws, const MhaFwdRoute& rt,
-              hipStream_t stream) {
+void launch_d(const float* qkv, float* o, float* lse2, int B, int C, int heads, int L, void* ws, const MhaQkvMax& qm,
+              const MhaFwdRoute& rt, hipStream_t stream) {
   const float qscale = 1.4426950408889634f / sqrtf((float)D);
   static const bool skip_check = getenv("HDIFF_NO_CHECK_PASS") != nullptr;
   const bool tail = !skip_check || rt.route == HDIFF_MHA_FWD_ROUTE_RUNNING_MAX || rt.route == HDIFF_MHA_FWD_ROUTE_FAST_F32;
   if constexpr (D < 48) {
     switch (rt.route) {
       case HDIFF_MHA_FWD_ROUTE_F16_SINGLE: launch_mha_fwd_f16(qkv, o, B, C, heads, L, qscale, ws, stream); break;
-      case HDIFF_MHA_FWD_ROUTE_H2_PAIRS: launch_mha_fwd_h2(qkv, o, lse2, B, C, heads, L, qscale, ws, stream); break;
-      case HDIFF_MHA_FWD_ROUTE_X3P_PAIRS: launch_mha_fwd_x3p(qkv, o, lse2, B, C, heads, L, qscale, ws, stream); break;
+      case HDIFF_MHA_FWD_ROUTE_H2_PAIRS: launch_mha_fwd_h2(qkv, o, lse2, B, C, heads, L, qscale, ws, qm, stream); break;
+      case HDIFF_MHA_FWD_ROUTE_X3P_PAIRS: launch_mha_fwd_x3p(qkv, o, lse2, B, C, heads, L, qscale, ws, qm, stream); break;
       case HDIFF_MHA_FWD_ROUTE_X3_TRIPLES: launch_mha_fwd_x3(qkv, o, lse2, B, C, heads, L, qscale, stream); break;
       case HDIFF_MHA_FWD_ROUTE_FAST_F32:
         hipLaunchKernelGGL((mha_flash_fwd_fast_kernel<D, 4>), dim3(cdiv(L, 256), heads, B), dim3(ATT_THREADS), 0, stream, qkv, o, lse2, C, L, qscale);
@@ -507,20 +507,20 @@
 }
 
 static int mha_flash_fwd_any(const float* qkv, float* o, float* lse2, int B, int C, int heads, int L, void* ws,
-                             int64_t ws_bytes, hipStream_t s) {
+                             int64_t ws_bytes, const MhaQkvMax& qm, hipStream_t s) {
   HDIFF_CHECK_ARG(qkv && o, "mha_flash_fwd: null pointer");
   const int rc = mha_fwd_check_shape(B, C, heads, L);
   if (rc != HDIFF_OK) return rc;
   const MhaFwdRoute rt = mha_fwd_route(B, C, heads, L, lse2 != nullptr, ws_bytes, contraction_mode());
   (void)hipGetLastError();
-  with_head_dim(C / heads, [&](auto d) { launch_d<decltype(d)::value>(qkv, o, lse2, B, C, heads, L, ws, rt, s); });
+  with_head_dim(C / heads, [&](auto d) { launch_d<decltype(d)::value>(qkv, o, lse2, B, C, heads, L, ws, qm, rt, s); });
   HDIFF_CHECK_LAUNCH("mha_flash_fwd_kernel");
   return HDIFF_OK;
 }
 
 extern "C" int hdiff_mha_flash_fwd(const float* qkv, float* o, float* lse2, int B, int C, int heads, int L,
                                    hdiff_stream_t stream) {
-  return mha_flash_fwd_any(qkv, o, lse2, B, C, heads, L, nullptr, 0, (hipStream_t)stream);
+  return mha_flash_fwd_any(qkv, o, lse2, B, C, heads, L, nullptr, 0, MhaQkvMax{nullptr, nullptr}, (hipStream_t)stream);
 }
 
 extern "C" int hdiff_mha_flash_fwd_workspace(int B, int C, int heads, int L, int64_t* bytes_out) {
@@ -534,7 +534,15 @@
 extern "C" int hdiff_mha_flash_fwd_ws(const float* qkv, float* o, float* lse2, int B, int C, int heads, int L, void* ws,
                                       int64_t ws_bytes, hdiff_stream_t stream) {
   HDIFF_CHECK_ARG(ws_bytes >= 0 && (ws != nullptr || ws_bytes == 0), "mha_flash_fwd_ws: workspace pointer / size mismatch");
-  return mha_flash_fwd_any(qkv, o, lse2, B, C, heads, L, ws, ws_bytes, (hipStream_t)stream);
+  return mha_flash_fwd_any(qkv, o, lse2, B, C, heads, L, ws, ws_bytes, MhaQkvMax{nullptr, nullptr}, (hipStream_t)stream);
+}
+
+extern "C" int hdiff_mha_flash_fwd_ws_max(const float* qkv, float* o, float* lse2, int B, int C, int heads, int L, void* ws,
+                                          int64_t ws_bytes, const uint32_t* qk_max, const uint32_t* v_max, hdiff_stream_t stream) {
+  HDIFF_CHECK_ARG(ws_bytes >= 0 && (ws != nullptr || ws_bytes == 0), "mha_flash_fwd_ws: workspace pointer / size mismatch");
+  HDIFF_CHECK_ARG(qk_max != nullptr && v_max != nullptr && (((uintptr_t)qk_max | (uintptr_t)v_max) & 3u) == 0,
+                  "mha_flash_fwd_ws_max: qk_max / v_max are null or not aligned to 32-bit words");
+  return mha_flash_fwd_any(qkv, o, lse2, B, C, heads, L, ws, ws_bytes, MhaQkvMax{qk_max, v_max}, (hipStream_t)stream);
 }
 
 extern "C" int hdiff_mha_flash_fwd_route(int B, int C, int heads, int L, int want_lse, int64_t ws_bytes, int* route_out,
diff --git a/hybrid-diffusion-underwater-atmopheric-image-enhancement_amd/csrc/attention_h2.hip b/hybrid-diffusion-underwater-atmopheric-image-enhancement_amd/csrc/attention_h2.hip
--- a/hybrid-diffusion-underwater-atmopheric-image-enhancement_amd/csrc/attention_h2.hip
+++ b/hybrid-diffusion-underwater-atmopheric-image-enhancement_amd/csrc/attention_h2.hip
@@ -110,6 +110,29 @@
 }
 
 template <int D>
+__device__ __forceinline__ void qk_split_position(const float* __restrict__ src, __bf16* __restrict__ pair, int which, int l, int L,
+                                                  float sc, float one) {
+  const size_t piece = (size_t)L * D;
+  const float up = (float)(1 << PAIR_SHIFT) * one;
+  unsigned h[4][D / 2];
+#pragma unroll
+  for (int j = 0; j < D / 2; ++j)
+    pair4(src[(size_t)(2 * j) * L + l] * sc, src[(size_t)(2 * j + 1) * L + l] * sc, up, h[0][j], h[1][j], h[2][j], h[3][j]);
+#pragma unroll
+  for (int p = 0; p < 4; ++p) {
+    if (which == 0 && (p == 1 || p == 3)) continue;
+    const int slot = which == 0 ? F_Q + (p == 0 ? 0 : 1) : F_K + p;
+    u32x4* o = reinterpret_cast<u32x4*>(pair + slot * piece + (size_t)l * D);
+#pragma unroll
+    for (int j = 0; j < D / 8; ++j) o[j] = u32x4{h[p][4 * j], h[p][4 * j + 1], h[p][4 * j + 2], h[p][4 * j + 3]};
+  }
+}
+__device__ __forceinline__ float qk_split_scale(unsigned mq_bits, unsigned mk_bits, int which, float qscale) {
+  const int a = balance_exp(mq_bits, mk_bits, qscale);
+  return which == 0 ? qscale * __builtin_bit_cast(float, (unsigned)(127 - a) << 23) : __builtin_bit_cast(float, (unsigned)(127 + a) << 23);
+}
+
+template <int D>
 __global__ __launch_bounds__(THREADS) void qk_split_h2_kernel(const float* __restrict__ qkv, const float* __restrict__ rowmax,
                                                               __bf16* __restrict__ ws, int C, int L, float qscale, float one) {
   const int heads = C / D;
@@ -121,25 +144,24 @@
     mq = fmaxf(mq, rowmax[(size_t)b * 2 * C + head * D + d]);
     mk = fmaxf(mk, rowmax[(size_t)b * 2 * C + C + head * D + d]);
   }
-  const int a = balance_exp(__builtin_bit_cast(unsigned, mq), __builtin_bit_cast(unsigned, mk), qscale);
-  const float sc = which == 0 ? qscale * __builtin_bit_cast(float, (unsigned)(127 - a) << 23) : __builtin_bit_cast(float, (unsigned)(127 + a) << 23);
+  const float sc = qk_split_scale(__builtin_bit_cast(unsigned, mq), __builtin_bit_cast(unsigned, mk), which, qscale);
   if (l >= L) return;
   const float* src = qkv + ((size_t)b * 3 * C + (size_t)which * C + (size_t)head * D) * L;
-  const size_t piece = (size_t)L * D;
-  __bf16* pair = ws + ((size_t)b * heads + head) * F_COUNT * piece;
-  const float up = (float)(1 << PAIR_SHIFT) * one;
-  unsigned h[4][D / 2];
-#pragma unroll
-  for (int j = 0; j < D / 2; ++j)
-    pair4(src[(size_t)(2 * j) * L + l] * sc, src[(size_t)(2 * j + 1) * L + l] * sc, up, h[0][j], h[1][j], h[2][j], h[3][j]);
-#pragma unroll
-  for (int p = 0; p < 4; ++p) {
-    if (which == 0 && (p == 1 || p == 3)) continue;
-    const int slot = which == 0 ? F_Q + (p == 0 ? 0 : 1) : F_K + p;
-    u32x4* o = reinterpret_cast<u32x4*>(pair + slot * piece + (size_t)l * D);
-#pragma unroll
-    for (int j = 0; j < D / 8; ++j) o[j] = u32x4{h[p][4 * j], h[p][4 * j + 1], h[p][4 * j + 2], h[p][4 * j + 3]};
-  }
+  qk_split_position<D>(src, ws + ((size_t)b * heads + head) * F_COUNT * (size_t)L * D, which, l, L, sc, one);
+}
+
+__device__ __forceinline__ int v_scale_exp(unsigned amax_bits) {
+  const int e = (int)((amax_bits >> 23) & 0xffu) - 127;
+  return e < -100 ? -100 : (e > 127 ? 127 : e);
+}
+__device__ __forceinline__ void v_split4(const float* __restrict__ src, _Float16* __restrict__ dst, size_t piece, int i, float scale,
+                                         float one) {
+  const f32x4 v = *reinterpret_cast<const f32x4*>(src + 4 * (size_t)i);
+  unsigned a0, a1, c0, c1;
+  split2(v[0] * scale, v[1] * scale, one, a0, a1);
+  split2(v[2] * scale, v[3] * scale, one, c0, c1);
+  *reinterpret_cast<u32x2*>(dst + 4 * (size_t)i) = u32x2{a0, c0};
+  *reinterpret_cast<u32x2*>(dst + piece + 4 * (size_t)i) = u32x2{a1, c1};
 }
 
 template <int D>
@@ -154,17 +176,38 @@
   _Float16* dst = reinterpret_cast<_Float16*>(pair + F_V * piece) + (size_t)d * L;
 
   const float amax = row_absmax(src, L, tid);
-  int e = (int)((__builtin_bit_cast(unsigned, amax) >> 23) & 0xffu) - 127;
-  e = e < -100 ? -100 : (e > 127 ? 127 : e);
+  const int e = v_scale_exp(__builtin_bit_cast(unsigned, amax));
   const float scale = __builtin_bit_cast(float, (unsigned)(14 - e + 127) << 23);
   if (tid == 0) reinterpret_cast<float*>(pair + F_VINV * piece)[d] = __builtin_bit_cast(float, (unsigned)(e - 14 + 127) << 23);
-  for (int i = tid; i < L / 4; i += THREADS) {
-    const f32x4 v = *reinterpret_cast<const f32x4*>(src + 4 * (size_t)i);
-    unsigned a0, a1, c0, c1;
-    split2(v[0] * scale, v[1] * scale, one, a0, a1);
-    split2(v[2] * scale, v[3] * scale, one, c0, c1);
-    *reinterpret_cast<u32x2*>(dst + 4 * (size_t)i) = u32x2{a0, c0};
-    *reinterpret_cast<u32x2*>(dst + piece + 4 * (size_t)i) = u32x2{a1, c1};
+  for (int i = tid; i < L / 4; i += THREADS) v_split4(src, dst, piece, i, scale, one);
+}
+
+template <int D>
+__global__ __launch_bounds__(THREADS) void qkv_split_h2_kernel(const float* __restrict__ qkv, const unsigned* __restrict__ qk_max,
+                                                               const unsigned* __restrict__ v_max, __bf16* __restrict__ ws, int C, int L,
+                                                               float qscale, float one) {
+  const int heads = C / D;
+  const int which = blockIdx.y / heads, head = blockIdx.y - which * heads, b = blockIdx.z;
+  const int tid = threadIdx.x;
+  const size_t piece = (size_t)L * D;
+  __bf16* pair = ws + ((size_t)b * heads + head) * F_COUNT * piece;
+  if (which < 2) {
+    const unsigned* m = qk_max + (size_t)b * 2 * heads + head;
+    const float sc = qk_split_scale(m[0], m[heads], which, qscale);
+    const int l = blockIdx.x * THREADS + tid;
+    if (l >= L) return;
+    qk_split_position<D>(qkv + ((size_t)b * 3 * C + (size_t)which * C + (size_t)head * D) * L, pair, which, l, L, sc, one);
+    return;
+  }
+  const unsigned* vm = v_max + (size_t)b * C + head * D;
+  if (blockIdx.x == 0 && tid < D)
+    reinterpret_cast<float*>(pair + F_VINV * piece)[tid] = __builtin_bit_cast(float, (unsigned)(v_scale_exp(vm[tid]) - 14 + 127) << 23);
+  const int i = blockIdx.x * (THREADS / 4) + (tid & 63);
+  if (4 * i >= L) return;
+  for (int d = tid >> 6; d < D; d += 4) {
+    const float scale = __builtin_bit_cast(float, (unsigned)(14 - v_scale_exp(vm[d]) + 127) << 23);
+    v_split4(qkv + ((size_t)b * 3 * C + 2 * (size_t)C + head * D + d) * L, reinterpret_cast<_Float16*>(pair + F_V * piece) + (size_t)d * L,
+             piece, i, scale, one);
   }
 }
 
@@ -466,10 +509,22 @@
   else hipLaunchKernelGGL((qk_split_h2_kernel<32>), grid, dim3(THREADS), 0, stream, qkv, rowmax, (__bf16*)ws, C, L, qscale, 1.0f);
 }
 
-void launch_mha_fwd_h2(const float* qkv, float* o, float* lse2, int B, int C, int heads, int L, float qscale, void* ws,
-                       hipStream_t stream) {
+void launch_qkv_split_h2(const float* qkv, void* ws, const unsigned* qk_max, const unsigned* v_max, int B, int C, int heads, int L,
+                         float qscale, hipStream_t stream) {
+  dim3 grid(L / 256, 3 * heads, B);
+  if (C / heads == 16) hipLaunchKernelGGL((qkv_split_h2_kernel<16>), grid, dim3(THREADS), 0, stream, qkv, qk_max, v_max, (__bf16*)ws, C, L, qscale, 1.0f);
+  else hipLaunchKernelGGL((qkv_split_h2_kernel<32>), grid, dim3(THREADS), 0, stream, qkv, qk_max, v_max, (__bf16*)ws, C, L, qscale, 1.0f);
+}
+
+void launch_split_h2(const float* qkv, void* ws, const MhaQkvMax& m, int B, int C, int heads, int L, float qscale, hipStream_t stream) {
+  if (m.qk_max != nullptr) return launch_qkv_split_h2(qkv, ws, m.qk_max, m.v_max, B, C, heads, L, qscale, stream);
   launch_qk_split_h2(qkv, ws, B, C, heads, L, qscale, stream);
   launch_v_split_h2(qkv, ws, B, C, heads, L, stream);
+}
+
+void launch_mha_fwd_h2(const float* qkv, float* o, float* lse2, int B, int C, int heads, int L, float qscale, void* ws,
+                       const MhaQkvMax& m, hipStream_t stream) {
+  launch_split_h2(qkv, ws, m, B, C, heads, L, qscale, stream);
   hipLaunchKernelGGL((mha_flash_fwd_h2_kernel<16, 4>), dim3(L / 256, heads, B), dim3(THREADS), 0, stream, (const __bf16*)ws, o, lse2,
                      C, L, 1.0f);
 }
diff --git a/hybrid-diffusion-underwater-atmopheric-image-enhancement_amd/csrc/attention_x3p.hip b/hybrid-diffusion-underwater-atmopheric-image-enhancement_amd/csrc/attention_x3p.hip
--- a/hybrid-diffusion-underwater-atmopheric-image-enhancement_amd/csrc/attention_x3p.hip
+++ b/hybrid-diffusion-underwater-atmopheric-image-enhancement_amd/csrc/attention_x3p.hip
@@ -268,9 +268,8 @@
 }
 
 void launch_mha_fwd_x3p(const float* qkv, float* o, float* lse2, int B, int C, int heads, int L, float qscale, void* ws,
-                        hipStream_t stream) {
-  launch_qk_split_h2(qkv, ws, B, C, heads, L, qscale, stream);
-  launch_v_split_h2(qkv, ws, B, C, heads, L, stream);
+                        const MhaQkvMax& m, hipStream_t stream) {
+  launch_split_h2(qkv, ws, m, B, C, heads, L, qscale, stream);
   hipLaunchKernelGGL(mha_flash_fwd_x3p_kernel, dim3(L / 256, heads, B), dim3(THREADS), 0, stream, (const __bf16*)ws, o, lse2, C, L, 1.0f);
 }
 
diff --git a/hybrid-diffusion-underwater-atmopheric-image-enhancement_amd/csrc/common.h b/hybrid-diffusion-underwater-atmopheric-image-enhancement_amd/csrc/common.h
--- a/hybrid-diffusion-underwater-atmopheric-image-enhancement_amd/csrc/common.h
+++ b/hybrid-diffusion-underwater-atmopheric-image-enhancement_amd/csrc/common.h
@@ -95,8 +95,10 @@
                        int C, int heads, int L, KeyRanges g, hipStream_t stream);
 int64_t mha_fwd_x3p_workspace(int B, int C, int heads, int L);
 int64_t mha_fwd_h2_tail_bytes(int B, int C);
-void launch_mha_fwd_x3p(const float* qkv, float* o, float* lse2, int B, int C, int heads, int L, float qscale, void* ws, hipStream_t stream);
-void launch_mha_fwd_h2(const float* qkv, float* o, float* lse2, int B, int C, int heads, int L, float qscale, void* ws, hipStream_t stream);
+struct MhaQkvMax { const unsigned* qk_max; const unsigned* v_max; };
+void launch_mha_fwd_x3p(const float* qkv, float* o, float* lse2, int B, int C, int heads, int L, float qscale, void* ws, const MhaQkvMax& m, hipStream_t stream);
+void launch_mha_fwd_h2(const float* qkv, float* o, float* lse2, int B, int C, int heads, int L, float qscale, void* ws, const MhaQkvMax& m, hipStream_t stream);
+void launch_split_h2(const float* qkv, void* ws, const MhaQkvMax& m, int B, int C, int heads, int L, float qscale, hipStream_t stream);
 void launch_qk_split_h2(const float* qkv, void* ws, int B, int C, int heads, int L, float qscale, hipStream_t stream);
 void launch_v_split_h2(const float* qkv, void* ws, int B, int C, int heads, int L, hipStream_t stream);
 void launch_mha_fwd_x3(const float* qkv, float* o, float* lse2, int B, int C, int heads, int L, float qscale, hipStream_t stream);
diff --git a/hybrid-diffusion-underwater-atmopheric-image-enhancement_amd/csrc/conv1x1_x3.hip b/hybrid-diffusion-underwater-atmopheric-image-enhancement_amd/csrc/conv1x1_x3.hip
--- a/hybrid-diffusion-underwater-atmopheric-image-enhancement_amd/csrc/conv1x1_x3.hip
+++ b/hybrid-diffusion-underwater-atmopheric-image-enhancement_amd/csrc/conv1x1_x3.hip
@@ -1,4 +1,6 @@
 #include <stdlib.h>
+
+#include <type_traits>
 
 #include "common.h"
 #include "conv_x3.h"
@@ -9,6 +11,21 @@
 namespace {
 
 constexpr int THREADS = 256;
+
+__device__ __forceinline__ unsigned row16_max(unsigned v) {
+  auto step = [&](auto ctrl) {
+    const unsigned o = (unsigned)__builtin_amdgcn_update_dpp(0, (int)v, decltype(ctrl)::value, 0xf, 0xf, true);
+    v = o > v ? o : v;
+  };
+  step(std::integral_constant<int, 0xB1>{});
+  step(std::integral_constant<int, 0x4E>{});
+  step(std::integral_constant<int, 0x141>{});
+  step(std::integral_constant<int, 0x140>{});
+  return v;
+}
+__device__ __forceinline__ void word_max(unsigned* w, unsigned m) {
+  if (m > __hip_atomic_load(w, __ATOMIC_RELAXED, __HIP_MEMORY_SCOPE_AGENT)) atomicMax(w, m);
+}
 
 __device__ constexpr int TERM_W[6] = {2, 1, 0, 1, 0, 0};
 __device__ constexpr int TERM_X[6] = {0, 1, 2, 0, 1, 0};
@@ -17,6 +34,7 @@
 __global__ __launch_bounds__(THREADS, 3) void conv1x1_x3_kernel(const Conv1x1X3K p) {
   constexpr int MT = 2, WN = 2;
   __shared__ __attribute__((aligned(16))) u32x4 sW[WLDS ? 2 : 1][WLDS ? 3 * 64 * 2 : 1];
+  __shared__ unsigned sMax[4][4][32];
   const int tid = threadIdx.x, lane = tid & 63, wave = tid >> 6;
   const int l31 = lane & 31, h = lane >> 5;
   int cob = blockIdx.x, tile_id = blockIdx.y;
@@ -146,6 +164,8 @@
   const bool full = co0 + 64 <= p.Cout;
   const bool track = p.absmax_out != nullptr;
   unsigned amax = 0u;
+  const bool qkv = p.qk_max != nullptr;
+  unsigned cmax[MT][16];
 #pragma unroll
   for (int mt = 0; mt < MT; ++mt) {
 #pragma unroll
@@ -173,10 +193,12 @@
         v += add[j];
         if (p.residual) v += res[j];
         if (ok[j]) *reinterpret_cast<f32x2*>(p.out + blk + (size_t)co * p.HW + 2u * l31) = v;
-        if (track && ok[j]) {
-          const unsigned v0 = __builtin_bit_cast(unsigned, v[0]) & 0x7fffffffu, v1 = __builtin_bit_cast(unsigned, v[1]) & 0x7fffffffu;
-          const unsigned vm = v0 > v1 ? v0 : v1;
+        if (track || qkv) {
+          const float e0 = v[0], e1 = v[1];
+          const unsigned v0 = __builtin_bit_cast(unsigned, e0) & 0x7fffffffu, v1 = __builtin_bit_cast(unsigned, e1) & 0x7fffffffu;
+          const unsigned vm = !ok[j] ? 0u : v0 > v1 ? v0 : v1;
           amax = vm > amax ? vm : amax;
+          if (qkv) cmax[mt][r] = vm;
         }
       }
     }
@@ -189,6 +211,46 @@
     }
     if (lane == 0) atomicMax(&p.absmax_out[b], amax);
   }
+  if (qkv) {
+#pragma unroll
+    for (int mt = 0; mt < MT; ++mt)
+#pragma unroll
+      for (int r = 0; r < 16; ++r) cmax[mt][r] = row16_max(cmax[mt][r]);
+    if ((lane & 15) == 0) {
+#pragma unroll
+      for (int mt = 0; mt < MT; ++mt)
+#pragma unroll
+        for (int r = 0; r < 16; ++r) sMax[wave][lane >> 4][mt * 16 + r] = cmax[mt][r];
+    }
+    __syncthreads();
+    if (tid < 64) {
+      const int u = tid & 31, hh = (u >> 2) & 1, reg = (tid >> 5) * 16 + (u & 3) + 4 * (u >> 3);
+      unsigned m = 0u;
+#pragma unroll
+      for (int w = 0; w < 4; ++w) {
+        const unsigned a = sMax[w][2 * hh][reg], c = sMax[w][2 * hh + 1][reg];
+        m = a > m ? a : m;
+        m = c > m ? c : m;
+      }
+      const int Cq = p.Cout / 3, D = Cq / p.heads, co = co0 + tid;
+      const bool runs = D == 16 || D == 32;
+      unsigned hm = m;
+      if (runs) {
+#pragma unroll
+        for (int o = 1; o < 16; o <<= 1) {
+          const unsigned other = (unsigned)__shfl_xor((int)hm, o, 64);
+          hm = other > hm ? other : hm;
+        }
+        const unsigned other = (unsigned)__shfl_xor((int)hm, 16, 64);
+        if (D == 32) hm = other > hm ? other : hm;
+      }
+      if (co < 2 * Cq) {
+        if (!runs || (tid & (D - 1)) == 0) word_max(&p.qk_max[(size_t)b * 2 * p.heads + co / D], hm);
+      } else if (co < p.Cout) {
+        word_max(&p.v_max[(size_t)b * Cq + (co - 2 * Cq)], m);
+      }
+    }
+  }
 }
 
 }
diff --git a/hybrid-diffusion-underwater-atmopheric-image-enhancement_amd/csrc/conv_igemm.hip b/hybrid-diffusion-underwater-atmopheric-image-enhancement_amd/csrc/conv_igemm.hip
--- a/hybrid-diffusion-underwater-atmopheric-image-enhancement_amd/csrc/conv_igemm.hip
+++ b/hybrid-diffusion-underwater-atmopheric-image-enhancement_amd/csrc/conv_igemm.hip
@@ -582,6 +582,8 @@
   const unsigned* pair_pack;
   int pair_taps;
   bool absmax_tail;
+  const hdiff_qkv_max* qkv;
+  bool qkv_tail;
 };
 
 bool s2_5x5_geometry(const hdiff_conv_desc* d, bool identity) {
@@ -618,12 +620,13 @@
          d->C0 % 2 == 0 && (long)(d->C0 + d->C1) * d->H * d->W < (1L << 30) && d->CinPad * d->CoutPad < (1 << 30);
 }
 
-ConvRoute conv_route(const hdiff_conv_desc* d, const hdiff_conv_range* r, bool dropout) {
+ConvRoute conv_route(const hdiff_conv_desc* d, const hdiff_conv_range* r, bool dropout, const hdiff_qkv_max* qkv = nullptr) {
   const bool split = hdiff::split_operands_on();
   if (!split || dropout) r = nullptr;
+  if (!split) qkv = nullptr;
   auto take = [&](int route, const void* pack = nullptr, int taps = 0) {
     const bool tail = r != nullptr && r->absmax_out != nullptr && (route == HDIFF_CONV_ROUTE_IGEMM || route == HDIFF_CONV_ROUTE_DIRECT_1X1);
-    return ConvRoute{route, r, (const unsigned*)pack, taps, tail};
+    return ConvRoute{route, r, (const unsigned*)pack, taps, tail, qkv, qkv != nullptr && route != HDIFF_CONV_ROUTE_X3_1X1};
   };
   const bool identity = d->out_sy == 1 && d->out_oy == 0 && d->out_sx == 1 && d->out_ox == 0;
   const bool same = identity && d->OH == d->H && d->OW == d->W;
@@ -716,7 +719,9 @@
     }
     case HDIFF_CONV_ROUTE_X3_1X1: {
       const hdiff::Conv1x1X3K q{d->x0, d->x1, d->C0, d->C0 + d->C1, (long)d->H * d->W, (const unsigned*)d->wp_x3, d->CoutPad, d->Cout,
-                                d->bias, d->addvec, d->residual, d->out, absmax_out};
+                                d->bias, d->addvec, d->residual, d->out, absmax_out,
+                                rt.qkv != nullptr ? rt.qkv->qk_max : nullptr, rt.qkv != nullptr ? rt.qkv->v_max : nullptr,
+                                rt.qkv != nullptr ? rt.qkv->heads : 0};
       hdiff::launch_conv1x1_x3(q, d->B, s);
       HDIFF_CHECK_LAUNCH("conv1x1_x3_kernel");
       return HDIFF_OK;
@@ -776,6 +781,29 @@
   }
   if ((threadIdx.x & 63) == 0) atomicMax(&q.words[b], m);
 }
+
+__global__ __launch_bounds__(256) void qkv_max_kernel(const float* __restrict__ out, unsigned* __restrict__ qk_max, unsigned* __restrict__ v_max,
+                                                      int C, int heads, long HW) {
+  const int row = blockIdx.x, b = blockIdx.y;
+  const float* src = out + ((size_t)b * 3 * C + row) * HW;
+  __shared__ unsigned red[4];
+  unsigned m = 0u;
+  for (long i = threadIdx.x; i < HW; i += 256) {
+    const unsigned vb = __builtin_bit_cast(unsigned, src[i]) & 0x7fffffffu;
+    m = vb > m ? vb : m;
+  }
+#pragma unroll
+  for (int o = 32; o > 0; o >>= 1) {
+    const unsigned other = (unsigned)__shfl_xor((int)m, o, 64);
+    m = other > m ? other : m;
+  }
+  if ((threadIdx.x & 63) == 0) red[threadIdx.x >> 6] = m;
+  __syncthreads();
+  if (threadIdx.x != 0) return;
+  for (int w = 0; w < 4; ++w) m = red[w] > m ? red[w] : m;
+  unsigned* word = row < 2 * C ? &qk_max[(size_t)b * 2 * heads + row / (C / heads)] : &v_max[(size_t)b * C + (row - 2 * C)];
+  if (m > __hip_atomic_load(word, __ATOMIC_RELAXED, __HIP_MEMORY_SCOPE_AGENT)) atomicMax(word, m);
+}
 }
 
 static int check_range(const hdiff_conv_desc* d, const hdiff_conv_range* r) {
@@ -810,19 +838,25 @@
 }
 
 static int conv2d_fwd(const hdiff_conv_desc* d, const hdiff_conv_range* r, const unsigned* keep_bits, float inv_keep,
-                      hdiff_stream_t stream) {
+                      hdiff_stream_t stream, const hdiff_qkv_max* qkv = nullptr) {
   ConvCfg c;
   int rc = configure(d, c);
   if (rc != HDIFF_OK) return rc;
-  const ConvRoute rt = conv_route(d, r, keep_bits != nullptr);
+  const ConvRoute rt = conv_route(d, r, keep_bits != nullptr, qkv);
   rc = conv2d_fwd_launch(d, c, rt, keep_bits, inv_keep, (hipStream_t)stream);
-  if (rc != HDIFF_OK || !rt.absmax_tail) return rc;
-  const OutAbsmaxK q{d->out, rt.range->absmax_out, d->Cout, d->VH, d->VW, d->OH, d->OW, d->out_sy, d->out_oy, d->out_sx, d->out_ox};
-  const long n = (long)d->Cout * d->VH * d->VW;
-  const int blocks = (int)((n + 1023) / 1024 < 256 ? (n + 1023) / 1024 : 256);
-  hipLaunchKernelGGL(conv_out_absmax_kernel, dim3(blocks, d->B), dim3(256), 0, (hipStream_t)stream, q);
-  HDIFF_CHECK_LAUNCH("conv_out_absmax_kernel");
-  return HDIFF_OK;
+  if (rc == HDIFF_OK && rt.absmax_tail) {
+    const OutAbsmaxK q{d->out, rt.range->absmax_out, d->Cout, d->VH, d->VW, d->OH, d->OW, d->out_sy, d->out_oy, d->out_sx, d->out_ox};
+    const long n = (long)d->Cout * d->VH * d->VW;
+    const int blocks = (int)((n + 1023) / 1024 < 256 ? (n + 1023) / 1024 : 256);
+    hipLaunchKernelGGL(conv_out_absmax_kernel, dim3(blocks, d->B), dim3(256), 0, (hipStream_t)stream, q);
+    HDIFF_CHECK_LAUNCH("conv_out_absmax_kernel");
+  }
+  if (rc == HDIFF_OK && rt.qkv_tail) {
+    hipLaunchKernelGGL(qkv_max_kernel, dim3(d->Cout, d->B), dim3(256), 0, (hipStream_t)stream, d->out, rt.qkv->qk_max, rt.qkv->v_max,
+                       d->Cout / 3, rt.qkv->heads, (long)d->OH * d->OW);
+    HDIFF_CHECK_LAUNCH("qkv_max_kernel");
+  }
+  return rc;
 }
 
 extern "C" int hdiff_conv2d_fwd(const hdiff_conv_desc* d, hdiff_stream_t stream) { return conv2d_fwd(d, nullptr, nullptr, 1.0f, stream); }
@@ -830,6 +864,17 @@
 extern "C" int hdiff_conv2d_fwd_range(const hdiff_conv_desc* d, const hdiff_conv_range* r, hdiff_stream_t stream) {
   const int rc = check_range(d, r);
   return rc != HDIFF_OK ? rc : conv2d_fwd(d, r, nullptr, 1.0f, stream);
+}
+
+extern "C" int hdiff_conv2d_fwd_qkv(const hdiff_conv_desc* d, const hdiff_conv_range* r, const hdiff_qkv_max* m, hdiff_stream_t stream) {
+  HDIFF_CHECK_ARG(d && m && m->qk_max && m->v_max, "conv2d_fwd_qkv: null pointer");
+  HDIFF_CHECK_ARG((((uintptr_t)m->qk_max | (uintptr_t)m->v_max) & 3u) == 0, "conv2d_fwd_qkv: qk_max / v_max are not aligned to 32-bit words");
+  HDIFF_CHECK_ARG(m->heads > 0 && d->Cout > 0 && d->Cout % (3 * m->heads) == 0, "conv2d_fwd_qkv: Cout = %d is not 3 x %d heads of equal size",
+                  d->Cout, m->heads);
+  HDIFF_CHECK_ARG(d->out_sy == 1 && d->out_oy == 0 && d->out_sx == 1 && d->out_ox == 0 && d->VH == d->OH && d->VW == d->OW,
+                  "conv2d_fwd_qkv: the output must be a dense [B][3 C][OH][OW] tensor written in full");
+  const int rc = r != nullptr ? check_range(d, r) : HDIFF_OK;
+  return rc != HDIFF_OK ? rc : conv2d_fwd(d, r, nullptr, 1.0f, stream, m);
 }
 
 extern "C" int hdiff_conv2d_fwd_dropout(const hdiff_conv_desc* d, const uint32_t* keep_bits, float inv_keep, hdiff_stream_t stream) {
diff --git a/hybrid-diffusion-underwater-atmopheric-image-enhancement_amd/csrc/conv_x3.h b/hybrid-diffusion-underwater-atmopheric-image-enhancement_amd/csrc/conv_x3.h
--- a/hybrid-diffusion-underwater-atmopheric-image-enhancement_amd/csrc/conv_x3.h
+++ b/hybrid-diffusion-underwater-atmopheric-image-enhancement_amd/csrc/conv_x3.h
@@ -44,6 +44,9 @@
   const float* residual;
   float* out;
   unsigned* absmax_out;
+  unsigned* qk_max;
+  unsigned* v_max;
+  int heads;
 };
 void launch_conv1x1_x3(const Conv1x1X3K& k, int B, hipStream_t stream);
 
diff --git a/hybrid-diffusion-underwater-atmopheric-image-enhancement_amd/engine.py b/hybrid-diffusion-underwater-atmopheric-image-enhancement_amd/engine.py
--- a/hybrid-diffusion-underwater-atmopheric-image-enhancement_amd/engine.py
+++ b/hybrid-diffusion-underwater-atmopheric-image-enhancement_amd/engine.py
@@ -229,17 +229,27 @@
         t._hdiff_base = base
         return t
 
-    RANGE_WORDS = 4096
-
-    def range_words(self, B: int) -> torch.Tensor:
+    RANGE_WORDS = 1 << 17
+
+    def range_words(self, B: int, optional: bool = False) -> Optional[torch.Tensor]:
         if self._words is None:
             self._words = torch.zeros(self.RANGE_WORDS, dtype=torch.int32, device=self.device)
             self.call("hdiff_range_words_zero", self._words.data_ptr(), self.RANGE_WORDS)
         if self._words_used + B > self.RANGE_WORDS:
+            if optional:
+                return None
             raise RuntimeError(f"hdiff: a plan holds at most {self.RANGE_WORDS} range words")
         w = self._words[self._words_used:self._words_used + B]
         self._words_used += B
         return w
+
+    def qkv_maxima(self, B: int, Cc: int, heads: int, L: int) -> Optional[Tuple[torch.Tensor, torch.Tensor, int]]:
+        need = C.c_int64(0)
+        _capi.check(self.lib.hdiff_mha_flash_fwd_workspace(B, Cc, heads, L, C.byref(need)), "mha_flash_fwd_workspace")
+        if not RESERVE_SPLIT_WORKSPACE or need.value == 0:
+            return None
+        words = self.range_words(B * (2 * heads + Cc), optional=True)
+        return None if words is None else (words[:B * 2 * heads], words[B * 2 * heads:], heads)
 
     def free(self, t: torch.Tensor) -> None:
         base = getattr(t, "_hdiff_base", None)
@@ -302,7 +312,8 @@
              addvec: Optional[torch.Tensor] = None, residual: Optional[torch.Tensor] = None,
              act_range: Optional[Tuple[torch.Tensor, torch.Tensor, int, float]] = None,
              dropout: Optional[Tuple[torch.Tensor, float]] = None,
-             absmax_out: Optional[torch.Tensor] = None, absmax_in: Optional[torch.Tensor] = None) -> None:
+             absmax_out: Optional[torch.Tensor] = None, absmax_in: Optional[torch.Tensor] = None,
+             qkv_max: Optional[Tuple[torch.Tensor, torch.Tensor, int]] = None) -> None:
         d = _capi.ConvDesc()
         C0 = int(x0.shape[1])
         C1 = int(x1.shape[1]) if x1 is not None else 0
@@ -335,7 +346,13 @@
             d.splitk_ws, d.splitk_floats = ws.data_ptr(), need.value
         self.keep((d, x0, x1, pk, bias, out, gn, addvec, residual, ws, dropout, r, absmax_out, absmax_in))
         self.flops += 2.0 * pk.ntaps * pk.cin * pk.cout * VH * VW * B
-        if dropout is not None:
+        if qkv_max is not None:
+            assert dropout is None
+            m = _capi.QkvMax()
+            m.qk_max, m.v_max, m.heads = qkv_max[0].data_ptr(), qkv_max[1].data_ptr(), qkv_max[2]
+            self.keep((m, qkv_max))
+            self.call("hdiff_conv2d_fwd_qkv", C.byref(d), None if r is None else C.byref(r), C.byref(m))
+        elif dropout is not None:
             self.call("hdiff_conv2d_fwd_dropout", C.byref(d), dropout[0].data_ptr(), C.c_float(dropout[1]))
         elif r is not None:
             self.call("hdiff_conv2d_fwd_range", C.byref(d), C.byref(r))
@@ -351,10 +368,15 @@
         _capi.check(self.lib.hdiff_mha_flash_fwd_workspace(B, Cc, heads, L, C.byref(need)), "mha_flash_fwd_workspace")
         return self.buf((need.value + 3) // 4) if need.value > 0 else None
 
-    def flash_attention(self, qkv: torch.Tensor, o: torch.Tensor, B: int, Cc: int, heads: int, L: int) -> None:
+    def flash_attention(self, qkv: torch.Tensor, o: torch.Tensor, B: int, Cc: int, heads: int, L: int,
+                        qkv_max: Optional[Tuple[torch.Tensor, torch.Tensor, int]] = None) -> None:
         ws = self.attention_workspace(B, Cc, heads, L)
-        self.call("hdiff_mha_flash_fwd_ws", qkv.data_ptr(), o.data_ptr(), None, B, Cc, heads, L, _ptr(ws),
-                  C.c_int64(0 if ws is None else ws.numel() * 4))
+        args = (qkv.data_ptr(), o.data_ptr(), None, B, Cc, heads, L, _ptr(ws), C.c_int64(0 if ws is None else ws.numel() * 4))
+        if qkv_max is not None:
+            self.ops.append(("hdiff_mha_flash_fwd_ws", self.lib.hdiff_mha_flash_fwd_ws_max,
+                             args + (qkv_max[0].data_ptr(), qkv_max[1].data_ptr())))
+        else:
+            self.call("hdiff_mha_flash_fwd_ws", *args)
         self.keep(ws)
         if ws is not None:
             self.free(ws)
@@ -460,9 +482,10 @@
     w_out = P[f"{p}.attn.out_proj.weight"].view(Cc, Cc, 1, 1)
     pk_in, pk_out = _std_pack(plan, w_in, 1, 0), _std_pack(plan, w_out, 1, 0)
     qkv = plan.buf(B, 3 * Cc, H, W)
-    plan.conv(h, None, pk_in, P[f"{p}.attn.in_proj_bias"], qkv, B=B, H=H, W=W, VH=H, VW=W)
+    qkv_max = plan.qkv_maxima(B, Cc, NUM_HEADS, H * W)
+    plan.conv(h, None, pk_in, P[f"{p}.attn.in_proj_bias"], qkv, B=B, H=H, W=W, VH=H, VW=W, qkv_max=qkv_max)
     o = plan.buf(B, Cc, H, W)
-    plan.flash_attention(qkv, o, B, Cc, NUM_HEADS, H * W)
+    plan.flash_attention(qkv, o, B, Cc, NUM_HEADS, H * W, qkv_max=qkv_max)
     plan.flops += 4.0 * (H * W) ** 2 * Cc * B
     plan.keep((qkv, o))
     plan.free(qkv)
diff --git a/include/hdiff.h b/include/hdiff.h
--- a/include/hdiff.h
+++ b/include/hdiff.h
@@ -83,6 +83,15 @@
 } hdiff_conv_range;
 int hdiff_conv2d_fwd_range(const hdiff_conv_desc* d, const hdiff_conv_range* r, hdiff_stream_t stream);
 int hdiff_range_words_zero(uint32_t* words, int n, hdiff_stream_t stream);
+
+typedef struct hdiff_qkv_max {
+  uint32_t* qk_max;
+  uint32_t* v_max;
+  int heads;
+} hdiff_qkv_max;
+int hdiff_conv2d_fwd_qkv(const hdiff_conv_desc* d, const hdiff_conv_range* r, const hdiff_qkv_max* m, hdiff_stream_t stream);
+int hdiff_mha_flash_fwd_ws_max(const float* qkv, float* o, float* lse2, int B, int C, int heads, int L, void* ws, int64_t ws_bytes,
+                               const uint32_t* qk_max, const uint32_t* v_max, hdiff_stream_t stream);
 
 enum {
   HDIFF_CONV_ROUTE_IGEMM = 0,
```
